# mjevans26/Satellite_ComputerVision

Hardware: AMD Instinct MI355X
Metric: tiles/sec (train) 256x256x4 U-Net (higher is better)
Workload: dtype bf16; 1 GPU; U-Net 256x256x4 bfloat16 training, batch 64 per GPU (BASELINE configs[1]); global_batch=64, parallelism=dp1, loss=weighted_categorical_crossentropy, optimizer=adam(9e-4)

## Files before the change

include/satcv.h:

```cpp
#ifndef SATCV_H
#define SATCV_H
#include <stdint.h>
#ifdef __cplusplus
extern "C" {
#endif

typedef double satcv_stat_t;

enum { SATCV_OK = 0, SATCV_ERR_INVALID = -1, SATCV_ERR_HIP = -2, SATCV_ERR_UNSUPPORTED = -3 };
enum { SATCV_F32 = 0, SATCV_BF16 = 1,
       SATCV_FP8 = 2 ,
       SATCV_FP8X = 3 ,
       SATCV_F64 = 4  };
#define SATCV_STAT_ROWS 32

const char* satcv_version(void);
const char* satcv_last_error(void);
int satcv_device_info(int32_t* out4);

int satcv_ingest_nhwc(const float* src, void* dst, int64_t npix, int32_t c, int32_t cpad,
                      int32_t dtype, void* stream);
int satcv_ingest_nhwc_scaled(const float* src, void* dst, int64_t npix, int32_t c, int32_t cpad, float mul, int32_t dtype, void* stream);
int satcv_ingest_chw(const void* src, int32_t src_kind, float scale, void* dst, int32_t n,
                     int32_t c, int32_t h, int32_t w, int32_t cpad, int32_t dtype, void* stream);
// ... 9 lines not shown
typedef struct satcv_conv_desc {
  const void* x0;
  const void* x1;
  int32_t c0, c1;
  const float* in_scale;
  const float* in_shift;
  int32_t in_relu;
  const void* w;
  const float* bias;
  void* y;
  int32_t ldy;
  satcv_stat_t* stats;
  int32_t stats_ld;
  int32_t n, h, w_;
  int32_t cout;
  int32_t cout_pad;
  int32_t kh, kw, dil;
  int32_t mode_in;
  int32_t mode_out;
  int32_t f;
  int32_t cstat;
  int32_t out_relu;
  int32_t dtype;
  int32_t accumulate;
  int32_t stride, hin, win;
  const float* out_scale;
  void* pool_y; int32_t pool_ld, pool_f;
  const void* bst_y; const void* bst_y1; int32_t bst_ld, bst_ld1, bst_split;
  const float* bst_scale; const float* bst_shift; const float* bst_mean; const float* bst_rstd; int32_t bst_relu;
  int32_t tile_policy;
} satcv_conv_desc;
int satcv_conv2d_igemm(const satcv_conv_desc* d, void* stream);
int satcv_conv2d_igemm_pipelined(const satcv_conv_desc* d);

typedef struct satcv_wgrad_desc {
  const void* x0; const void* x1; int32_t c0, c1;
  const float* in_scale; const float* in_shift; int32_t in_relu;
  const void* dy; int32_t lddy;
  float* dw;
  int32_t cin, cout;
  int32_t n, h, w_;
  int32_t kh, kw, dil;
  int32_t mode_dy;
  int32_t f;
  int32_t transposed;
  float* workspace; int64_t workspace_bytes;
  int32_t dtype;
  int32_t accumulate;
  int32_t whole_chip;
  int32_t defer_reduce;
} satcv_wgrad_desc;
int64_t satcv_conv2d_wgrad_workspace(const satcv_wgrad_desc* d);
int satcv_conv2d_wgrad(const satcv_wgrad_desc* d, void* stream);

typedef struct satcv_reduce_job {
  const float* ws; float* dw;
  int32_t nslab, taps, kpad, npad, cin, nvalid, transposed, accumulate, lanes, pad_;
} satcv_reduce_job;
int satcv_conv2d_wgrad_reduce_job(const satcv_wgrad_desc* d, satcv_reduce_job* job);
int64_t satcv_reduce_job_items(const satcv_reduce_job* job);
int satcv_reduce_slabs_batched(const satcv_reduce_job* jobs_dev, const int64_t* prefix_dev, int32_t njobs, int64_t total_items, void* stream);

typedef struct satcv_bwdf_desc {
  const void* g; const void* yraw; int32_t ldg;
  const float* bn_scale; const float* bn_shift; const float* bn_mean; const float* bn_rstd;
  const float* bn_coef;
  int32_t linear;
  const void* x0; const void* x1; int32_t c0, c1;
  const float* in_scale; const float* in_shift; int32_t in_relu;
  const void* w_dgrad;
  void* dx; int32_t lddx;
  float* dw; int32_t cin, cout;
  int32_t n, h, w_;
  int32_t kh, kw, dil;
  float* workspace; int64_t workspace_bytes;
  int32_t dtype;
  int32_t accumulate;
  satcv_stat_t* bst_sums; int32_t bst_sums_ld;
  const float* bst_mean; const float* bst_rstd;
  int32_t bst_act_form;
  const void* dpool; int32_t lddp; const void* amax;
  const float* hg_dlogits; const float* hg_w; int32_t hg_ncls;
  int32_t defer_reduce;
} satcv_bwdf_desc;
int64_t satcv_conv2d_bwd_fused_workspace(const satcv_bwdf_desc* d);
int satcv_conv2d_bwd_fused(const satcv_bwdf_desc* d, void* stream);
int satcv_conv2d_bwd_fused_reduce_job(const satcv_bwdf_desc* d, satcv_reduce_job* job);

typedef struct satcv_ctbf_desc {
  const void* g; int32_t ldg;
  const void* yup; int32_t ldy;
  const float* bn_scale; const float* bn_shift; const float* bn_mean; const float* bn_rstd;
  const float* bn_c1; const float* bn_c2; int32_t linear;
  const void* x; int32_t ldx;
  const float* in_scale; const float* in_shift; int32_t in_relu;
  const void* w_dgrad; int32_t w_npad;
  void* dx; int32_t lddx;
  float* dw; int32_t cin, cout;
  int32_t n, h, w_, f;
  float* workspace; int64_t workspace_bytes;
  int32_t dtype, accumulate, defer_reduce;
  satcv_stat_t* bst_sums; int32_t bst_sums_ld; const float* bst_mean; const float* bst_rstd;
} satcv_ctbf_desc;
int64_t satcv_convt_bwd_fused_workspace(const satcv_ctbf_desc* d);
int satcv_convt_bwd_fused(const satcv_ctbf_desc* d, void* stream);
int satcv_convt_bwd_fused_reduce_job(const satcv_ctbf_desc* d, satcv_reduce_job* job);

int satcv_bn_finalize_train(satcv_stat_t* stats, int32_t stats_ld, int32_t c, float count,
                            const float* gamma, const float* beta, float eps, float momentum,
                            int32_t updates, int32_t bessel, float* moving_mean, float* moving_var,
                            float* scale, float* shift, float* mean, float* rstd, void* stream);
int satcv_bn_affine_infer(const float* gamma, const float* beta, const float* moving_mean,
                          const float* moving_var, float eps, int32_t c, float* scale, float* shift,
                          void* stream);
typedef struct satcv_bn_affine_job {
  const float* gamma; const float* beta; const float* moving_mean; const float* moving_var;
  float* scale; float* shift; int64_t c;
  const float* conv_bias; float* bias_eff;
} satcv_bn_affine_job;
int satcv_bn_affine_infer_batched(const satcv_bn_affine_job* jobs_device, int32_t njobs, float eps, void* stream);

int satcv_bn_relu_pool(const void* yraw, const float* scale, const float* shift, void* act, int32_t act_ld,
                       void* pooled, satcv_stat_t* stats, int32_t stats_ld, int32_t n, int32_t h,
                       int32_t w_, int32_t c, int32_t f, int32_t dtype, void* stream);
int satcv_bn_relu_pool_amax(const void* yraw, const float* scale, const float* shift, void* act, int32_t act_ld,
                            void* pooled, void* amax, satcv_stat_t* stats, int32_t stats_ld, int32_t n, int32_t h,
                            int32_t w_, int32_t c, int32_t f, int32_t dtype, void* stream);

typedef struct satcv_bnbwd_desc {
  const void* da; int32_t ldda;
  const void* dpool; int32_t lddp;
  int32_t f;
  const void* yraw; int32_t ldy;
  const float* scale; const float* shift; const float* mean; const float* rstd;
  satcv_stat_t* sums; int32_t sums_ld;
  const float* coef;
  void* dy; int32_t lddy_out;
  float* dbias;
  int32_t n, h, w_, c;
  int32_t dtype;
  int32_t linear;
  const void* yraw1; int32_t ldy1;
  void* dy1; int32_t lddy1;
  int32_t c_split;
  satcv_stat_t* sk_sums; int32_t sk_sums_ld;
} satcv_bnbwd_desc;
int satcv_bn_bwd_reduce(const satcv_bnbwd_desc* d, void* stream);
int satcv_bn_bwd_finalize(satcv_stat_t* sums, int32_t sums_ld, int32_t c, float count, float* dgamma,
                          float* dbeta, float* coef, int32_t accumulate, void* stream);
int satcv_bn_bwd_apply(const satcv_bnbwd_desc* d, void* stream);
int satcv_bn_bwd_finalize2(satcv_stat_t* sums, int32_t sums_ld, satcv_stat_t* act_sums, int32_t act_sums_ld, int32_t c, float count,
                           const float* scale, const float* shift, const float* mean, const float* rstd, float* dgamma, float* dbeta,
                           float* coef, int32_t accumulate, void* stream);

int satcv_relu_bwd(const void* act, void* g, int64_t count, int32_t dtype, void* stream);
int64_t satcv_bias_grad_workspace(int64_t npix, int32_t c);
int satcv_bias_grad(const void* dy, int32_t lddy, int64_t npix, int32_t c, int32_t dtype, float* dbias, float* partials, void* stream);

int satcv_maxpool(const void* x, void* out, int32_t n, int32_t h, int32_t w_, int32_t c, int32_t k, int32_t s,
                  int32_t pad, int32_t dtype, void* stream);
int satcv_add_act(const void* y, const float* y_scale, const float* y_shift, const void* res,
                  const float* res_scale, const float* res_shift, int32_t relu, void* out, int64_t npix,
                  int32_t c, int32_t dtype, void* stream);
int satcv_affine_requant(const void* x, int32_t ldx, const float* scale, const float* shift, int32_t relu, void* out, int32_t ldo,
                         int64_t npix, int32_t c, int32_t dtype, int32_t dtype_out, void* stream);

int satcv_upsample_head(const float* logits, int32_t n, int32_t h, int32_t w_, int32_t ncls, int32_t factor,
                        int32_t activation, float thresh, float* probs, int32_t* classes, void* stream);

int satcv_dropout_mask(uint64_t seed, uint64_t offset, float rate, int64_t count, float* mask, void* stream);
int satcv_dropout_apply(const void* x, int32_t ldx, const float* scale, const float* shift, int32_t relu,
                        const float* mask, int32_t ldm, int32_t mask_mode, void* out, int32_t ldo, int32_t n,
                        int32_t hw, int32_t c, int32_t dtype, void* stream);

typedef struct satcv_head_desc {
  const void* x; int32_t ldx; int32_t cin;
  const float* in_scale; const float* in_shift;
  const float* w;
  const float* b;
  int32_t ncls; int32_t activation; float thresh;
  float* probs;
  int32_t* classes;
  const float* dlogits;
  void* dx; int32_t lddx;
  float* dw; float* db;
  const float* bnr_mean; const float* bnr_rstd; satcv_stat_t* bnr_sums; int32_t bnr_sums_ld;
  int64_t npix;
  int32_t dtype;
  float* partials;
} satcv_head_desc;
int satcv_head_fwd(const satcv_head_desc* d, void* stream);
int satcv_head_bwd(const satcv_head_desc* d, void* stream);
int64_t satcv_head_bwd_workspace(const satcv_head_desc* d);
int satcv_head_bwd_finalize(const satcv_head_desc* d, void* stream);

uint32_t satcv_crc32c(const void* data, uint64_t nbytes, uint32_t crc_in);

typedef struct {
  const void* src; int32_t src_kind;
  int32_t n, c, hin, win, h, w_;
  double rescale;
  int32_t nan_mask, replace;
  uint64_t seed;
  const double* ch_mean;
  double contra_mul, bright_mul;
  int32_t flip_v, flip_h, rot;
  float* dst; int32_t ldc, coff;
} satcv_tile_desc;
int satcv_tile_channel_mean(const satcv_tile_desc* d, double* mean_out , void* stream);
int satcv_tile_ingest(const satcv_tile_desc* d, void* stream);
int satcv_label_onehot(const void* lc, int32_t lc_kind, const int32_t* lut, const void* lu, int32_t lu_kind, const int32_t* lu_lut,
                       int32_t n, int32_t hin, int32_t win, int32_t h, int32_t w_, int32_t nclasses, int32_t flip_v, int32_t flip_h,
                       int32_t rot, float* dst, int32_t ldc, int32_t coff, void* stream);

int satcv_loss_fwd_bwd(int32_t kind, const float* probs, const float* y_true,
                       const float* weights, int32_t ncls, int32_t activation, int64_t npix,
                       float grad_scale, float* loss_out, float* dlogits, void* stream);

int satcv_loss_global_fwd_bwd(int32_t kind, const float* probs, const float* y_true,
                              const float* class_weights, int32_t ncls, int32_t activation,
                              int32_t nimg, int64_t pix_per_img, float eps, float grad_scale,
                              float* workspace, float* loss_out, float* dlogits, void* stream);

int satcv_confusion(const int32_t* classes, const float* y_true, int32_t ncls, int64_t npix,
                    int64_t* confusion, void* stream);

int satcv_adam_step(float* p, const float* g, float* m, float* v, int64_t n, float beta1,
                    float beta2, float eps, float* state, const float* lr_mul, void* stream);
int satcv_adam_step_part(float* p, const float* g, float* m, float* v, int64_t n, float beta1,
                         float beta2, float eps, float* state, const float* lr_mul, int32_t bump, void* stream);

int satcv_zero2(void* a, int64_t bytes_a, void* b, int64_t bytes_b, void* stream);

#define SATCV_COMM_ID_BYTES 128
typedef struct satcv_comm satcv_comm;
int satcv_comm_unique_id(void* id128);
// ... 57 lines not shown
```

satellite_computervision_amd/_lib.py:

```python
import ctypes as C
import os

import torch

_HERE = os.path.dirname(os.path.abspath(__file__))
LIB_PATH = os.environ.get('SATCV_LIB') or os.path.join(_HERE, 'libsatcv.so')

F32, BF16, FP8, FP8X, F64 = 0, 1, 2, 3, 4
STAT_ROWS = 32

c_i32, c_i64, c_f32, c_vp = C.c_int32, C.c_int64, C.c_float, C.c_void_p


class ConvDesc(C.Structure):
    _fields_ = [('x0', c_vp), ('x1', c_vp), ('c0', c_i32), ('c1', c_i32),
                ('in_scale', c_vp), ('in_shift', c_vp), ('in_relu', c_i32),
                ('w', c_vp), ('bias', c_vp), ('y', c_vp), ('ldy', c_i32),
                ('stats', c_vp), ('stats_ld', c_i32),
                ('n', c_i32), ('h', c_i32), ('w_', c_i32),
                ('cout', c_i32), ('cout_pad', c_i32),
                ('kh', c_i32), ('kw', c_i32), ('dil', c_i32),
                ('mode_in', c_i32), ('mode_out', c_i32), ('f', c_i32),
                ('cstat', c_i32), ('out_relu', c_i32), ('dtype', c_i32), ('accumulate', c_i32),
                ('stride', c_i32), ('hin', c_i32), ('win', c_i32), ('out_scale', c_vp), ('pool_y', c_vp), ('pool_ld', c_i32), ('pool_f', c_i32),
                ('bst_y', c_vp), ('bst_y1', c_vp), ('bst_ld', c_i32), ('bst_ld1', c_i32), ('bst_split', c_i32),
                ('bst_scale', c_vp), ('bst_shift', c_vp), ('bst_mean', c_vp), ('bst_rstd', c_vp), ('bst_relu', c_i32), ('tile_policy', c_i32)]


class PackJob(C.Structure):
    _fields_ = [('src', c_vp), ('dst', c_vp), ('mode', c_i32), ('taps', c_i32), ('cin', c_i32), ('cout', c_i32), ('kpad', c_i32), ('npad', c_i32)]


class TileDesc(C.Structure):
    _fields_ = [('src', c_vp), ('src_kind', c_i32), ('n', c_i32), ('c', c_i32), ('hin', c_i32), ('win', c_i32), ('h', c_i32), ('w_', c_i32),
                ('rescale', C.c_double), ('nan_mask', c_i32), ('replace', c_i32), ('seed', C.c_uint64), ('ch_mean', c_vp),
                ('contra_mul', C.c_double), ('bright_mul', C.c_double), ('flip_v', c_i32), ('flip_h', c_i32), ('rot', c_i32),
                ('dst', c_vp), ('ldc', c_i32), ('coff', c_i32)]


class WgradDesc(C.Structure):
    _fields_ = [('x0', c_vp), ('x1', c_vp), ('c0', c_i32), ('c1', c_i32),
                ('in_scale', c_vp), ('in_shift', c_vp), ('in_relu', c_i32),
                ('dy', c_vp), ('lddy', c_i32), ('dw', c_vp),
                ('cin', c_i32), ('cout', c_i32),
                ('n', c_i32), ('h', c_i32), ('w_', c_i32),
                ('kh', c_i32), ('kw', c_i32), ('dil', c_i32),
                ('mode_dy', c_i32), ('f', c_i32), ('transposed', c_i32),
                ('workspace', c_vp), ('workspace_bytes', c_i64), ('dtype', c_i32), ('accumulate', c_i32), ('whole_chip', c_i32), ('defer_reduce', c_i32)]


class BwdfDesc(C.Structure):
    _fields_ = [('g', c_vp), ('yraw', c_vp), ('ldg', c_i32),
                ('bn_scale', c_vp), ('bn_shift', c_vp), ('bn_mean', c_vp), ('bn_rstd', c_vp), ('bn_coef', c_vp), ('linear', c_i32),
                ('x0', c_vp), ('x1', c_vp), ('c0', c_i32), ('c1', c_i32),
                ('in_scale', c_vp), ('in_shift', c_vp), ('in_relu', c_i32),
                ('w_dgrad', c_vp), ('dx', c_vp), ('lddx', c_i32),
                ('dw', c_vp), ('cin', c_i32), ('cout', c_i32),
                ('n', c_i32), ('h', c_i32), ('w_', c_i32), ('kh', c_i32), ('kw', c_i32), ('dil', c_i32),
                ('workspace', c_vp), ('workspace_bytes', c_i64), ('dtype', c_i32), ('accumulate', c_i32),
                ('bst_sums', c_vp), ('bst_sums_ld', c_i32), ('bst_mean', c_vp), ('bst_rstd', c_vp), ('bst_act_form', c_i32),
                ('dpool', c_vp), ('lddp', c_i32), ('amax', c_vp),
                ('hg_dlogits', c_vp), ('hg_w', c_vp), ('hg_ncls', c_i32), ('defer_reduce', c_i32)]


class CtbfDesc(C.Structure):
    _fields_ = [('g', c_vp), ('ldg', c_i32), ('yup', c_vp), ('ldy', c_i32),
                ('bn_scale', c_vp), ('bn_shift', c_vp), ('bn_mean', c_vp), ('bn_rstd', c_vp), ('bn_c1', c_vp), ('bn_c2', c_vp), ('linear', c_i32),
                ('x', c_vp), ('ldx', c_i32), ('in_scale', c_vp), ('in_shift', c_vp), ('in_relu', c_i32),
                ('w_dgrad', c_vp), ('w_npad', c_i32), ('dx', c_vp), ('lddx', c_i32), ('dw', c_vp), ('cin', c_i32), ('cout', c_i32),
                ('n', c_i32), ('h', c_i32), ('w_', c_i32), ('f', c_i32), ('workspace', c_vp), ('workspace_bytes', c_i64),
                ('dtype', c_i32), ('accumulate', c_i32), ('defer_reduce', c_i32),
                ('bst_sums', c_vp), ('bst_sums_ld', c_i32), ('bst_mean', c_vp), ('bst_rstd', c_vp)]


class ReduceJob(C.Structure):
    _fields_ = [('ws', c_vp), ('dw', c_vp), ('nslab', c_i32), ('taps', c_i32), ('kpad', c_i32), ('npad', c_i32), ('cin', c_i32), ('nvalid', c_i32),
                ('transposed', c_i32), ('accumulate', c_i32), ('lanes', c_i32), ('pad_', c_i32)]


class BnBwdDesc(C.Structure):
    _fields_ = [('da', c_vp), ('ldda', c_i32), ('dpool', c_vp), ('lddp', c_i32), ('f', c_i32),
                ('yraw', c_vp), ('ldy', c_i32),
                ('scale', c_vp), ('shift', c_vp), ('mean', c_vp), ('rstd', c_vp),
                ('sums', c_vp), ('sums_ld', c_i32), ('coef', c_vp),
                ('dy', c_vp), ('lddy_out', c_i32), ('dbias', c_vp),
                ('n', c_i32), ('h', c_i32), ('w_', c_i32), ('c', c_i32), ('dtype', c_i32), ('linear', c_i32),
                ('yraw1', c_vp), ('ldy1', c_i32), ('dy1', c_vp), ('lddy1', c_i32), ('c_split', c_i32),
                ('sk_sums', c_vp), ('sk_sums_ld', c_i32)]


class HeadDesc(C.Structure):
    _fields_ = [('x', c_vp), ('ldx', c_i32), ('cin', c_i32),
                ('in_scale', c_vp), ('in_shift', c_vp), ('w', c_vp), ('b', c_vp),
                ('ncls', c_i32), ('activation', c_i32), ('thresh', c_f32),
                ('probs', c_vp), ('classes', c_vp), ('dlogits', c_vp),
                ('dx', c_vp), ('lddx', c_i32), ('dw', c_vp), ('db', c_vp),
                ('bnr_mean', c_vp), ('bnr_rstd', c_vp), ('bnr_sums', c_vp), ('bnr_sums_ld', c_i32),
                ('npix', c_i64), ('dtype', c_i32), ('partials', c_vp)]


class LstmGatesDesc(C.Structure):
    _fields_ = [('xg', c_vp), ('ldx', c_i32), ('hg', c_vp), ('ldh_g', c_i32), ('c_prev', c_vp),
                ('c_out', c_vp), ('h_out', c_vp), ('ldh', c_i32), ('gates_out', c_vp),
                ('stats', c_vp), ('stats_ld', c_i32),
                ('dh_a', c_vp), ('lddh_a', c_i32), ('dh_b', c_vp), ('lddh_b', c_i32), ('dc_next', c_vp),
                ('dz_out', c_vp), ('lddz', c_i32), ('dc_prev_out', c_vp),
                ('npix', c_i64), ('filters', c_i32), ('rec_act', c_i32), ('act', c_i32), ('dtype', c_i32)]


class DenseSrc(C.Structure):
    _fields_ = [('x', c_vp), ('ld', c_i32), ('cin', c_i32), ('dtype', c_i32),
                ('in_scale', c_vp), ('in_shift', c_vp), ('in_relu', c_i32),
                ('hs', c_i32), ('ws', c_i32),
                ('dx', c_vp), ('lddx', c_i32), ('dx_dtype', c_i32)]


class DenseDesc(C.Structure):
    _fields_ = [('src', DenseSrc * 2), ('nsrc', c_i32),
                ('w', c_vp), ('b', c_vp), ('cout', c_i32),
                ('activation', c_i32), ('max_value', c_f32),
                ('out', c_vp), ('classes', c_vp), ('z_out', c_vp),
                ('npix', c_i64), ('h', c_i32), ('w_', c_i32),
                ('dout', c_vp), ('dz_out', c_vp), ('dw', c_vp), ('db', c_vp)]


_SIGS = {
    'satcv_version': (C.c_char_p, []),
    'satcv_last_error': (C.c_char_p, []),
    'satcv_device_info': (C.c_int, [C.POINTER(c_i32)]),
    'satcv_ingest_nhwc': (C.c_int, [c_vp, c_vp, c_i64, c_i32, c_i32, c_i32, c_vp]),
    'satcv_ingest_nhwc_scaled': (C.c_int, [c_vp, c_vp, c_i64, c_i32, c_i32, c_f32, c_i32, c_vp]),
    'satcv_ingest_chw': (C.c_int, [c_vp, c_i32, c_f32, c_vp, c_i32, c_i32, c_i32, c_i32, c_i32, c_i32, c_vp]),
    'satcv_pack_weights': (C.c_int, [c_vp, c_vp, c_vp, c_i32, c_i32, c_i32, c_i32, c_i32, c_i32, c_i32, c_vp]),
    'satcv_pack_job_items': (c_i64, [C.POINTER(PackJob)]),
    'satcv_pack_weights_batched': (C.c_int, [c_vp, c_vp, c_i32, c_i64, c_i32, c_vp]),
    'satcv_conv2d_igemm': (C.c_int, [C.POINTER(ConvDesc), c_vp]),
    'satcv_conv2d_igemm_pipelined': (C.c_int, [C.POINTER(ConvDesc)]),
    'satcv_conv2d_wgrad_workspace': (c_i64, [C.POINTER(WgradDesc)]),
    'satcv_conv2d_wgrad': (C.c_int, [C.POINTER(WgradDesc), c_vp]),
    'satcv_conv2d_wgrad_reduce_job': (C.c_int, [C.POINTER(WgradDesc), C.POINTER(ReduceJob)]),
    'satcv_reduce_job_items': (c_i64, [C.POINTER(ReduceJob)]),
    'satcv_reduce_slabs_batched': (C.c_int, [c_vp, c_vp, c_i32, c_i64, c_vp]),
    'satcv_conv2d_bwd_fused_workspace': (c_i64, [C.POINTER(BwdfDesc)]),
    'satcv_conv2d_bwd_fused': (C.c_int, [C.POINTER(BwdfDesc), c_vp]),
    'satcv_conv2d_bwd_fused_reduce_job': (C.c_int, [C.POINTER(BwdfDesc), C.POINTER(ReduceJob)]),
    'satcv_convt_bwd_fused_workspace': (c_i64, [C.POINTER(CtbfDesc)]),
    'satcv_convt_bwd_fused': (C.c_int, [C.POINTER(CtbfDesc), c_vp]),
    'satcv_convt_bwd_fused_reduce_job': (C.c_int, [C.POINTER(CtbfDesc), C.POINTER(ReduceJob)]),
    'satcv_bn_finalize_train': (C.c_int, [c_vp, c_i32, c_i32, c_f32, c_vp, c_vp, c_f32, c_f32, c_i32, c_i32,
                                          c_vp, c_vp, c_vp, c_vp, c_vp, c_vp, c_vp]),
    'satcv_bn_affine_infer': (C.c_int, [c_vp, c_vp, c_vp, c_vp, c_f32, c_i32, c_vp, c_vp, c_vp]),
    'satcv_bn_affine_infer_batched': (C.c_int, [c_vp, c_i32, c_f32, c_vp]),
    'satcv_bn_relu_pool': (C.c_int, [c_vp, c_vp, c_vp, c_vp, c_i32, c_vp, c_vp, c_i32, c_i32, c_i32, c_i32, c_i32, c_i32, c_i32, c_vp]),
    'satcv_bn_relu_pool_amax': (C.c_int, [c_vp, c_vp, c_vp, c_vp, c_i32, c_vp, c_vp, c_vp, c_i32, c_i32, c_i32, c_i32, c_i32, c_i32, c_i32, c_vp]),
    'satcv_bn_bwd_reduce': (C.c_int, [C.POINTER(BnBwdDesc), c_vp]),
    'satcv_bn_bwd_finalize': (C.c_int, [c_vp, c_i32, c_i32, c_f32, c_vp, c_vp, c_vp, c_i32, c_vp]),
    'satcv_bn_bwd_apply': (C.c_int, [C.POINTER(BnBwdDesc), c_vp]),
    'satcv_bn_bwd_finalize2': (C.c_int, [c_vp, c_i32, c_vp, c_i32, c_i32, c_f32, c_vp, c_vp, c_vp, c_vp, c_vp, c_vp, c_vp, c_i32, c_vp]),
    'satcv_maxpool': (C.c_int, [c_vp, c_vp, c_i32, c_i32, c_i32, c_i32, c_i32, c_i32, c_i32, c_i32, c_vp]),
    'satcv_affine_requant': (C.c_int, [c_vp, c_i32, c_vp, c_vp, c_i32, c_vp, c_i32, c_i64, c_i32, c_i32, c_i32, c_vp]),
    'satcv_add_act': (C.c_int, [c_vp, c_vp, c_vp, c_vp, c_vp, c_vp, c_i32, c_vp, c_i64, c_i32, c_i32, c_vp]),
    'satcv_relu_bwd': (C.c_int, [c_vp, c_vp, c_i64, c_i32, c_vp]),
    'satcv_bias_grad_workspace': (c_i64, [c_i64, c_i32]),
    'satcv_bias_grad': (C.c_int, [c_vp, c_i32, c_i64, c_i32, c_i32, c_vp, c_vp, c_vp]),
    'satcv_upsample_head': (C.c_int, [c_vp, c_i32, c_i32, c_i32, c_i32, c_i32, c_i32, c_f32, c_vp, c_vp, c_vp]),
    'satcv_dropout_mask': (C.c_int, [C.c_uint64, C.c_uint64, c_f32, c_i64, c_vp, c_vp]),
    'satcv_dropout_apply': (C.c_int, [c_vp, c_i32, c_vp, c_vp, c_i32, c_vp, c_i32, c_i32, c_vp, c_i32, c_i32, c_i32, c_i32, c_i32, c_vp]),
    'satcv_tile_channel_mean': (C.c_int, [C.POINTER(TileDesc), c_vp, c_vp]),
    'satcv_tile_ingest': (C.c_int, [C.POINTER(TileDesc), c_vp]),
    'satcv_label_onehot': (C.c_int, [c_vp, c_i32, c_vp, c_vp, c_i32, c_vp, c_i32, c_i32, c_i32, c_i32, c_i32, c_i32, c_i32, c_i32, c_i32, c_vp, c_i32, c_i32, c_vp]),
    'satcv_crc32c': (C.c_uint32, [c_vp, C.c_uint64, C.c_uint32]),
    'satcv_head_fwd': (C.c_int, [C.POINTER(HeadDesc), c_vp]),
    'satcv_head_bwd': (C.c_int, [C.POINTER(HeadDesc), c_vp]),
    'satcv_head_bwd_workspace': (c_i64, [C.POINTER(HeadDesc)]),
    'satcv_head_bwd_finalize': (C.c_int, [C.POINTER(HeadDesc), c_vp]),
    'satcv_loss_fwd_bwd': (C.c_int, [c_i32, c_vp, c_vp, c_vp, c_i32, c_i32, c_i64, c_f32, c_vp, c_vp, c_vp]),
    'satcv_loss_global_fwd_bwd': (C.c_int, [c_i32, c_vp, c_vp, c_vp, c_i32, c_i32, c_i32, c_i64, c_f32, c_f32, c_vp, c_vp, c_vp, c_vp]),
    'satcv_confusion': (C.c_int, [c_vp, c_vp, c_i32, c_i64, c_vp, c_vp]),
    'satcv_adam_step': (C.c_int, [c_vp, c_vp, c_vp, c_vp, c_i64, c_f32, c_f32, c_f32, c_vp, c_vp, c_vp]),
    'satcv_adam_step_part': (C.c_int, [c_vp, c_vp, c_vp, c_vp, c_i64, c_f32, c_f32, c_f32, c_vp, c_vp, c_i32, c_vp]),
    'satcv_comm_unique_id': (C.c_int, [c_vp]),
    'satcv_comm_init': (C.c_int, [C.POINTER(c_vp), c_i32, c_i32, c_vp]),
    'satcv_comm_destroy': (C.c_int, [c_vp]),
    'satcv_comm_info': (C.c_int, [c_vp, C.POINTER(c_i32), C.POINTER(c_i32)]),
    'satcv_allreduce_grads': (C.c_int, [c_vp, c_vp, c_i64, c_i64, c_i64, c_i32, c_vp, c_vp]),
    'satcv_allreduce': (C.c_int, [c_vp, c_vp, c_i64, c_i32, c_i32, c_vp]),
    'satcv_ingest_seq': (C.c_int, [c_vp, c_vp, c_i32, c_i32, c_i32, c_i32, c_i32, c_i32, c_i32, c_vp]),
    'satcv_convlstm_gates_fwd': (C.c_int, [C.POINTER(LstmGatesDesc), c_vp]),
    'satcv_convlstm_gates_bwd': (C.c_int, [C.POINTER(LstmGatesDesc), c_vp]),
    'satcv_dense_small_fwd': (C.c_int, [C.POINTER(DenseDesc), c_vp]),
    'satcv_dense_small_bwd': (C.c_int, [C.POINTER(DenseDesc), c_vp]),
    'satcv_zero2': (C.c_int, [c_vp, c_i64, c_vp, c_i64, c_vp]),
    'satcv_graph_begin': (C.c_int, [c_vp]),
    'satcv_graph_end': (C.c_int, [c_vp, C.POINTER(c_vp)]),
    'satcv_graph_launch': (C.c_int, [c_vp, c_vp]),
    'satcv_graph_destroy': (C.c_int, [c_vp]),
    'satcv_prof_enable': (C.c_int, [c_i32]),
    'satcv_prof_collect': (C.c_int, [c_i32, C.POINTER(C.c_double), C.POINTER(c_i64), C.POINTER(C.c_double)]),
    'satcv_set_option': (C.c_int, [C.c_char_p, c_i32]),
    'satcv_get_option': (C.c_int, [C.c_char_p, C.POINTER(c_i32)]),
}

EXPORTED_SYMBOLS = tuple(_SIGS)


class SatcvError(RuntimeError):
    pass


def _load():
    if not os.path.exists(LIB_PATH):
        raise ImportError(
            f'{LIB_PATH} not found: the HIP extension is required (no CPU fallback). '
            'Build it with `python -m satellite_computervision_amd.build` or __graft_entry__.build().')
    hip = os.path.join(os.path.dirname(torch.__file__), 'lib', 'libamdhip64.so')
    if os.path.exists(hip):
        C.CDLL(hip, mode=C.RTLD_GLOBAL)
    lib = C.CDLL(LIB_PATH)
    for name, (res, args) in _SIGS.items():
        fn = getattr(lib, name)
        fn.restype = res
        fn.argtypes = args
    return lib


lib = _load()


def check(rc):
    if rc != 0:
        raise SatcvError(f'satcv error {rc}: {lib.satcv_last_error().decode()}')


def call(name, *args):
    check(getattr(lib, name)(*args))
```

satellite_computervision_amd/csrc/conv_bwd_fused.hip:

```cpp
#include "igemm_common.hpp"
#include <cstdlib>
#include <cstring>

#ifndef BWDF_ABL
#define BWDF_ABL 0
#endif
#define FABL(bit) ((BWDF_ABL & (bit)) != 0)

int wgrad_reduce_slabs(const float* ws, float* dw, int nslab, int taps, int kpad, int npad, int cin, int nvalid, int accumulate, hipStream_t st);
void reduce_job_fill(satcv_reduce_job* job, const float* ws, float* dw, int nslab, int taps, int kpad, int npad, int cin, int nvalid, int transposed, int accumulate);
void satcv_prof_begin(int kind, double flops, hipStream_t st);
void satcv_prof_end(int kind, hipStream_t st);

struct BwdfArgs {
  IgemmArgs e;
  const void* g; const void* yraw; int ldg;
  const float* bn_scale; const float* bn_shift; const float* bn_mean; const float* bn_rstd; const float* bn_coef; int bn_c, linear;
  const void* x0; const void* x1; int c0, c1;
  const float* in_scale; const float* in_shift; int in_relu;
  const void* w;
  float* ws;
  int tiles_x, tiles_y;
  satcv_stat_t* bst_sums; int bst_ld; const float* bst_mean; const float* bst_rstd;
  int bst_act_form;
  const void* dp; int lddp; const unsigned char* amax;
  const float* hg_dl; const float* hg_w;
};

__device__ __forceinline__ bf16x4 tr_read4(const bf16* p) {
  short4v v = __builtin_amdgcn_ds_read_tr16_b64_v4i16((__attribute__((address_space(3))) short4v*)(p));
  return __builtin_bit_cast(bf16x4, v);
}

template <int CIN, int COUT, int NW, int WPS, bool POOL = false, bool NODG = false, int CINS = CIN, bool HG = false>
__global__ __launch_bounds__(NW * 64, WPS) void bwd_fused_kernel(const BwdfArgs a, const int total_tiles) {
  static_assert(!HG || !POOL, "the head feeds a decoder block");
  typedef bf16 T;
  constexpr int TW = 32, TH = 8, BM = 256, RL = TH + 2, CL = TW + 2, PITCH = CL, EL = 8, NTHREADS = NW * 64;
  constexpr int SD = COUT / 8, SX = CIN / 8, SXR = CINS / 8;
  constexpr int DSTRIDE = RL * PITCH * EL;
  constexpr int XSTRIDE = BM * EL + 32;
  static_assert((DSTRIDE * 2) % 256 == 64 && (XSTRIDE * 2) % 256 == 64, "plane strides must be 64 B modulo 256 B");
  constexpr int D_ITEMS = RL * CL * SD, DI = (D_ITEMS + NTHREADS - 1) / NTHREADS;
  constexpr int X_ITEMS = BM * SXR, XI = X_ITEMS / NTHREADS;
  static_assert(X_ITEMS % NTHREADS == 0 && NTHREADS % SD == 0 && NTHREADS % SXR == 0, "item -> thread mapping");
  constexpr int XPIX_STEP = NTHREADS / SXR;
  static_assert(XPIX_STEP % 32 == 0, "x items of a thread must share a column");
  constexpr int MT = 8 / NW, NT = CIN / 32;
#ifdef BWDF_NOBAL
  constexpr int NTILE = (CIN / 32) * (COUT / 32) * 9, FULL = (NTILE + NW - 1) / NW, REM = 0, WT = FULL;
#else
  constexpr int NTILE = (CIN / 32) * (COUT / 32) * 9, FULL = NTILE / NW, REM = NTILE % NW, WT = FULL + (REM ? 1 : 0);
#endif
  constexpr bool GUARD = FULL * NW > NTILE;
  constexpr int WPP = REM ? NW / REM : 1, KPW = REM ? 16 / WPP : 0;
  static_assert(REM == 0 || (NW % REM == 0 && 16 % WPP == 0 && KPW % 2 == 0), "left-over products must split evenly along K");
  constexpr int W_ITEMS = NODG ? 0 : 9 * SD * CIN;
  constexpr size_t R0_BYTES = ((size_t)(SD * DSTRIDE + SX * XSTRIDE) * sizeof(T) + 127) / 128 * 128;
  constexpr size_t W_BYTES = (size_t)W_ITEMS * EL * sizeof(T);
  constexpr size_t O_BYTES = (size_t)BM * (CIN + 8) * sizeof(T);
  constexpr bool O_ALIAS = O_BYTES <= (size_t)SD * DSTRIDE * sizeof(T);
  constexpr size_t TAB_BYTES = (size_t)(SD * 32 + SX * 16 + (HG ? 2 * COUT : 0)) * sizeof(float);
  static_assert(!NODG || O_ALIAS || true, "");
  constexpr size_t O_OFF = O_ALIAS ? 0 : (R0_BYTES + W_BYTES + TAB_BYTES + 127) / 128 * 128;
  extern __shared__ __attribute__((aligned(16))) unsigned char smem_raw[];
  T* ldsD = reinterpret_cast<T*>(smem_raw);
  T* ldsX = ldsD + SD * DSTRIDE;
  T* ldsW = reinterpret_cast<T*>(smem_raw + R0_BYTES);
  float* tabD = reinterpret_cast<float*>(smem_raw + R0_BYTES + W_BYTES);
  float* tabX = tabD + SD * 32;
  float* tabH = tabX + SX * 16;

  const int tid = threadIdx.x, lane = tid & 63, wave = tid >> 6;
  const int r = lane & 31, hh = lane >> 5;
  const T* wp = reinterpret_cast<const T*>(a.w);

  for (int it = tid; it < W_ITEMS; it += NTHREADS) lstore8<T>(ldsW + (size_t)it * EL, gload8<T>(wp + (size_t)it * EL));
  if constexpr (SXR < SX) {
    for (int it = tid; it < (SX - SXR) * BM; it += NTHREADS) lstore8<T>(ldsX + (SXR + it / BM) * XSTRIDE + (it % BM) * EL, zero8<T>());
  }
  for (int ch = tid; ch < COUT; ch += NTHREADS) {
    const float sc = a.bn_scale[ch], sh = a.bn_shift[ch], mu = a.bn_mean[ch], rs = a.bn_rstd[ch], c1 = a.bn_coef[ch], c2 = a.bn_coef[a.bn_c + ch];
    float* t = tabD + (ch >> 3) * 32 + (ch & 7);
    t[0] = sc; t[8] = sh; t[16] = -sc * c2 * rs; t[24] = sc * (c2 * rs * mu - c1);
  }
  if constexpr (HG) {
    for (int ch = tid; ch < COUT; ch += NTHREADS) {
      float* t = tabH + (ch >> 3) * 16 + (ch & 7);
      t[0] = a.hg_w[ch * 2]; t[8] = a.hg_w[ch * 2 + 1];
    }
  }
  for (int ch = tid; ch < CINS; ch += NTHREADS) {
    float* t = tabX + (ch >> 3) * 16 + (ch & 7);
    t[0] = a.in_scale ? a.in_scale[ch] : 1.f; t[8] = a.in_scale ? a.in_shift[ch] : 0.f;
  }
  const float lin_lo = a.linear ? -INFINITY : 0.f;
  const bool xaff = a.in_scale != nullptr;
  const unsigned xrelu_lim = a.in_relu != 0 ? 0u : 0x80008000u;

  const int slot_d = tid % SD, slot_x = tid % SXR;
  constexpr int DPK = (DI + 2) / 3;
  unsigned d_pk[DPK];
#pragma unroll
  for (int k = 0; k < DPK; ++k) d_pk[k] = 0;
#pragma unroll
  for (int j = 0; j < DI; ++j) {
    const int it = tid + j * NTHREADS;
    const int p = it / SD, c = p % CL, L = p / CL;
    d_pk[j / 3] |= (unsigned)(it < D_ITEMS ? (L << 6) | c : 0x3ff) << (10 * (j % 3));
  }
  auto d_item = [&](int j) -> int { return (int)((d_pk[j / 3] >> (10 * (j % 3))) & 0x3ffu); };
  const int g_rowstride = a.e.w_ * a.ldg;
  const unsigned gy_lane = (unsigned)slot_d * EL;
  const int xch0 = slot_x * EL;
  const bool xsecond = xch0 >= a.c0;
  const T* xsrc = xsecond ? reinterpret_cast<const T*>(a.x1) + (xch0 - a.c0) : reinterpret_cast<const T*>(a.x0) + xch0;
  const int xcs = xsecond ? a.c1 : a.c0;
  const int xq0 = tid / SXR;
  const int x_l0 = slot_x * XSTRIDE + xq0 * EL;
  const int x_eoff0 = ((xq0 / TW) * a.e.w_ + (xq0 % TW)) * xcs, x_estep = (XPIX_STEP / TW) * a.e.w_ * xcs;

  int a_off[MT];
#pragma unroll
  for (int m = 0; m < MT; ++m) {
    const int q = (wave * MT + m) * 32 + r;
    a_off[m] = ((q / TW) * PITCH + (q % TW)) * EL;
  }
  const int gi = lane >> 4, i16 = lane & 15;
  const int chb = 16 * (gi & 1) + 4 * (i16 & 3);
  const int pk = 8 * (gi >> 1) + (i16 >> 2);
  const int tr_x = (chb >> 3) * XSTRIDE + pk * EL + (chb & 7);
  const int tr_d = (chb >> 3) * DSTRIDE + pk * EL + (chb & 7);

  auto tile_origin = [&](int v, int& n0, int& y0, int& x0) {
    const int tx = v % a.tiles_x; v /= a.tiles_x;
    const int ty = v % a.tiles_y;
    n0 = v / a.tiles_y; y0 = ty * TH; x0 = tx * TW;
  };
  auto next_origin = [&](int& n0, int& y0, int& x0) {
    x0 += TW;
    if (x0 >= a.e.w_) { x0 = 0; y0 += TH; if (y0 >= a.e.h) { y0 = 0; ++n0; } }
  };
  Raw8<T> rg[HG ? 1 : DI], ry[DI], rx[XI];
  float2 rdl[HG ? DI : 1];
  Raw8<T> rp[POOL ? DI : 1];
  uint2 ra[POOL ? DI : 1];
  const int hp = a.e.h >> 1, wpool = a.e.w_ >> 1;
  unsigned valid = 0;
  auto issue_loads = [&](int n0, int y0, int x0) -> unsigned {
    unsigned vm = 0;
    const int ylo = 1 - y0, yhi = a.e.h - y0 + 1, xlo = 1 - x0, xhi = a.e.w_ - x0 + 1;
    const long long pb = (long long)(n0 * a.e.h + y0 - 1) * a.e.w_ + (x0 - 1);
    const long long bp = pb * a.ldg;
    const T* gb = reinterpret_cast<const T*>(a.g) + bp;
    const T* yb = reinterpret_cast<const T*>(a.yraw) + bp;
    const unsigned centre = (unsigned)(g_rowstride + a.ldg) + gy_lane;
#pragma unroll
    for (int j = 0; j < DI; ++j) {
      const int pk_ = d_item(j), L = pk_ >> 6, c = pk_ & 63;
      const bool ok = pk_ != 0x3ff && L >= ylo && L < yhi && c >= xlo && c < xhi;
      vm |= (ok ? 1u : 0u) << j;
      unsigned off = ok ? (unsigned)(__mul24(L, g_rowstride) + __mul24(c, a.ldg)) + gy_lane : centre;
      asm volatile("" : "+v"(off));
      if constexpr (HG) {
        int poff = ok ? __mul24(L, a.e.w_) + c : a.e.w_ + 1;
        asm volatile("" : "+v"(poff));
        rdl[j] = reinterpret_cast<const float2*>(a.hg_dl)[pb + poff];
        ry[j] = gload8<T>(yb + off);
      } else if (!FABL(32)) { rg[j] = gload8<T>(gb + off); ry[j] = gload8<T>(yb + off); }
      else { rg[j] = zero8<T>(); ry[j] = zero8<T>(); rg[j].q[0].x = off; }
    }
    return vm;
  };
  auto issue_pool = [&](int n0, int y0, int x0) {
    if constexpr (POOL) {
      const int ylo = 1 - y0, yhi = a.e.h - y0 + 1, xlo = 1 - x0, xhi = a.e.w_ - x0 + 1;
      const size_t pb = (size_t)(n0 * hp + (y0 >> 1)) * wpool + (x0 >> 1);
#pragma unroll
      for (int j = 0; j < DI; ++j) {
        const int pk_ = d_item(j), L = pk_ >> 6, c = pk_ & 63;
        const bool ok = pk_ != 0x3ff && L >= ylo && L < yhi && c >= xlo && c < xhi;
        int po = ok ? __mul24((L - 1) >> 1, wpool) + ((c - 1) >> 1) : 0;
        asm volatile("" : "+v"(po));
        rp[j] = gload8<T>(reinterpret_cast<const T*>(a.dp) + (pb + po) * a.lddp + gy_lane);
        ra[j] = *reinterpret_cast<const uint2*>(a.amax + (pb + po) * COUT + gy_lane);
      }
    }
  };
  auto issue_x = [&](int n0, int y0, int x0) {
    const size_t bp = (size_t)(n0 * a.e.h + y0) * a.e.w_ + x0;
    const T* xb = xsrc + bp * xcs + x_eoff0;
#pragma unroll
    for (int j = 0; j < XI; ++j) { if (!FABL(32)) rx[j] = gload8<T>(xb + (size_t)j * x_estep); else { rx[j] = zero8<T>(); rx[j].q[0].x = (unsigned)(size_t)xb; } }
  };

  const int G = gridDim.x;
  const int xcd = blockIdx.x & 7, nx = G >> 3, remx = G & 7;
  const int bid = (xcd < remx ? xcd * (nx + 1) : remx * (nx + 1) + (xcd - remx) * nx) + (blockIdx.x >> 3);
  const int per = total_tiles / G, extra = total_tiles % G;
  const int t_lo = bid * per + (bid < extra ? bid : extra), t_hi = t_lo + per + (bid < extra ? 1 : 0);

  f32x16 wacc[WT];
  int w_xo[WT], w_do[WT];
#pragma unroll
  for (int t = 0; t < WT; ++t) {
#pragma unroll
    for (int i = 0; i < 16; ++i) wacc[t][i] = 0.f;
    const int wv = __builtin_amdgcn_readfirstlane(wave);
    const int id = t < FULL ? wv + t * NW : FULL * NW + wv / WPP;
    const int tap = id % 9, pair = id / 9;
    const int ci_t = pair % (CIN / 32), co_t = pair / (CIN / 32);
    w_xo[t] = ci_t * 4 * XSTRIDE;
    w_do[t] = co_t * 4 * DSTRIDE + ((2 - tap / 3) * PITCH + (2 - tap % 3)) * EL;
    if (t >= FULL) {
      const int k0 = (wv % WPP) * KPW;
      w_xo[t] += k0 * 16 * EL;
      w_do[t] += (k0 >> 1) * PITCH * EL;
    }
  }

  constexpr bool BST = !NODG && (WPS != 1 || POOL);
  float bs1[8], bs2[8];
#pragma unroll
  for (int e = 0; e < 8; ++e) { bs1[e] = 0.f; bs2[e] = 0.f; }
  int n0, y0, x0;
  if (t_lo < t_hi) { tile_origin(t_lo, n0, y0, x0); valid = issue_loads(n0, y0, x0); issue_x(n0, y0, x0); issue_pool(n0, y0, x0); }
  __syncthreads();
  for (int t = t_lo; t < t_hi; ++t) {
    {
      int toff = slot_d * 32;
      asm volatile("" : "+v"(toff));
      const float4* tp = reinterpret_cast<const float4*>(tabD + toff);
      float prm[32];
#pragma unroll
      for (int k = 0; k < 8; ++k) { const float4 v4 = tp[k]; prm[4 * k] = v4.x; prm[4 * k + 1] = v4.y; prm[4 * k + 2] = v4.z; prm[4 * k + 3] = v4.w; }
#pragma unroll
      for (int j = 0; j < DI; ++j) {
        float gv[8], yv[8];
        if constexpr (HG) {
          int hoff = slot_d * 16;
          asm volatile("" : "+v"(hoff));
          const float4* hp = reinterpret_cast<const float4*>(tabH + hoff);
          const float4 w00 = hp[0], w01 = hp[1], w10 = hp[2], w11 = hp[3];
          const float w0[8] = {w00.x, w00.y, w00.z, w00.w, w01.x, w01.y, w01.z, w01.w};
          const float w1[8] = {w10.x, w10.y, w10.z, w10.w, w11.x, w11.y, w11.z, w11.w};
#pragma unroll
          for (int e = 0; e < 8; ++e) gv[e] = (float)(T)fmaf(rdl[j].y, w1[e], rdl[j].x * w0[e]);
        } else {
          unpack8<T>(rg[j], gv);
        }
        unpack8<T>(ry[j], yv);
        if constexpr (POOL) {
          float pv[8];
          unpack8<T>(rp[j], pv);
          const int pk2 = d_item(j);
          const unsigned sub = ((((pk2 >> 6) + 1) & 1) << 1) | (((pk2 & 63) + 1) & 1);
#pragma unroll
          for (int e = 0; e < 8; ++e) {
            const unsigned am = ((e < 4 ? ra[j].x : ra[j].y) >> (8 * (e & 3))) & 0xffu;
            gv[e] += am == sub ? pv[e] : 0.f;
          }
        }
        Raw8<T> v;
        if constexpr (FABL(2) && !HG) { v = rg[j]; v.q[0].x ^= ry[j].q[0].x; }
        else {
          bf16x8 o;
#pragma unroll
          for (int e = 0; e < 8; ++e) {
            const float act = yv[e] * prm[e] + prm[8 + e];
            const float gm = act > lin_lo ? gv[e] : 0.f;
            o[e] = (bf16)(prm[e] * gm + (prm[16 + e] * yv[e] + prm[24 + e]));
          }
          v.q[0] = __builtin_bit_cast(uint4, o);
        }
        v = select8<T>((valid >> j) & 1u, v);
        const int pk_ = d_item(j);
        if (pk_ != 0x3ff) lstore8<T>(ldsD + slot_d * DSTRIDE + __mul24((pk_ >> 6) * CL + (pk_ & 63), EL), v);
        __builtin_amdgcn_sched_barrier(0);
      }
    }
    {
      float sc[8], sh[8];
      if (xaff) {
        int toff = slot_x * 16;
        asm volatile("" : "+v"(toff));
        const float4* tp = reinterpret_cast<const float4*>(tabX + toff);
        const float4 s0 = tp[0], s1 = tp[1], h0 = tp[2], h1 = tp[3];
        sc[0] = s0.x; sc[1] = s0.y; sc[2] = s0.z; sc[3] = s0.w; sc[4] = s1.x; sc[5] = s1.y; sc[6] = s1.z; sc[7] = s1.w;
        sh[0] = h0.x; sh[1] = h0.y; sh[2] = h0.z; sh[3] = h0.w; sh[4] = h1.x; sh[5] = h1.y; sh[6] = h1.z; sh[7] = h1.w;
      }
#pragma unroll
      for (int j = 0; j < XI; ++j) {
        Raw8<T> v = rx[j];
        if (xaff) v = affine8_lim(v, sc, sh, xrelu_lim);
        lstore8<T>(ldsX + x_l0 + j * (XPIX_STEP * EL), v);
      }
    }
    __syncthreads();
    const int tn0 = n0, ty0 = y0, tx0 = x0;
    if (t + 1 < t_hi) { next_origin(n0, y0, x0); valid = issue_loads(n0, y0, x0); }

#pragma unroll
    for (int tt = 0; tt < FULL; ++tt) {
      if (!FABL(8) && (!GUARD || tt < FULL - 1 || __builtin_amdgcn_readfirstlane(wave) + (FULL - 1) * NW < NTILE)) {
        const T* xa = ldsX + w_xo[tt] + tr_x;
        const T* da = ldsD + w_do[tt] + tr_d;
        bf16x4 fa[2][2], fb[2][2];
        auto read_k = [&](const T* xp, const T* dp, int u, int buf) {
          const int xq = u * 16 * EL, dq = ((u >> 1) * PITCH + (u & 1) * 16) * EL;
          fa[buf][0] = tr_read4(xp + xq); fa[buf][1] = tr_read4(xp + xq + 4 * EL);
          fb[buf][0] = tr_read4(dp + dq); fb[buf][1] = tr_read4(dp + dq + 4 * EL);
        };
        read_k(xa, da, 0, 0);
#pragma unroll 1
        for (int grp = 0; grp < TH / 2; ++grp) {
          const T* xp = xa + grp * (64 * EL);
          const T* dp = da + grp * (2 * PITCH * EL);
          const int wrap = grp + 1 < TH / 2 ? 1 : 1 - TH / 2;
#pragma unroll
          for (int u = 0; u < 4; ++u) {
            asm volatile("" ::: "memory");
            if (u < 3) read_k(xp, dp, u + 1, (u + 1) & 1);
            else read_k(xp + wrap * (64 * EL), dp + wrap * (2 * PITCH * EL), 0, 0);
            __builtin_amdgcn_sched_barrier(0);
            const bf16x8 afr = __builtin_shufflevector(fa[u & 1][0], fa[u & 1][1], 0, 1, 2, 3, 4, 5, 6, 7);
            const bf16x8 bfr = __builtin_shufflevector(fb[u & 1][0], fb[u & 1][1], 0, 1, 2, 3, 4, 5, 6, 7);
            if constexpr (!FABL(1)) wacc[tt] = __builtin_amdgcn_mfma_f32_32x32x16_bf16(afr, bfr, wacc[tt], 0, 0, 0);
            else asm volatile("" :: "v"(afr), "v"(bfr));
          }
        }
      }
    }
    if constexpr (REM > 0) {
      if (!FABL(8)) {
        const T* xa = ldsX + w_xo[FULL] + tr_x;
        const T* da = ldsD + w_do[FULL] + tr_d;
        bf16x4 fa[2][2], fb[2][2];
        auto read_k = [&](int u, int buf) {
          const int xq = u * 16 * EL, dq = ((u >> 1) * PITCH + (u & 1) * 16) * EL;
          fa[buf][0] = tr_read4(xa + xq); fa[buf][1] = tr_read4(xa + xq + 4 * EL);
          fb[buf][0] = tr_read4(da + dq); fb[buf][1] = tr_read4(da + dq + 4 * EL);
        };
        read_k(0, 0);
#pragma unroll
        for (int u = 0; u < KPW; ++u) {
          asm volatile("" ::: "memory");
          if (u + 1 < KPW) read_k(u + 1, (u + 1) & 1);
          __builtin_amdgcn_sched_barrier(0);
          const bf16x8 afr = __builtin_shufflevector(fa[u & 1][0], fa[u & 1][1], 0, 1, 2, 3, 4, 5, 6, 7);
          const bf16x8 bfr = __builtin_shufflevector(fb[u & 1][0], fb[u & 1][1], 0, 1, 2, 3, 4, 5, 6, 7);
          if constexpr (!FABL(1)) wacc[FULL] = __builtin_amdgcn_mfma_f32_32x32x16_bf16(afr, bfr, wacc[FULL], 0, 0, 0);
          else asm volatile("" :: "v"(afr), "v"(bfr));
        }
      }
    }
    if (t + 1 < t_hi) issue_x(n0, y0, x0);
    if (POOL && NODG && t + 1 < t_hi) issue_pool(n0, y0, x0);
    if constexpr (!NODG) {
    f32x16 acc[MT][NT];
#pragma unroll
    for (int m = 0; m < MT; ++m)
#pragma unroll
      for (int n = 0; n < NT; ++n)
#pragma unroll
        for (int i = 0; i < 16; ++i) acc[m][n][i] = 0.f;
    {
      constexpr int KS = COUT / 16, STEPS = 9 * KS;
      FragT<T> af[2][MT], bf[2][NT];
      auto read_step = [&](int st, int buf) {
        const int tap = st / KS, ks = st % KS;
        const int tap_off = ((tap / 3) * PITCH + (tap % 3)) * EL;
        const int slot = ks * 2 + hh;
#pragma unroll
        for (int m = 0; m < MT; ++m) af[buf][m] = lds_frag<T>(ldsD + slot * DSTRIDE + a_off[m] + tap_off);
#pragma unroll
        for (int n = 0; n < NT; ++n) bf[buf][n] = lds_frag<T>(ldsW + ((tap * SD + slot) * CIN + n * 32 + r) * EL);
      };
      if constexpr (!FABL(8)) {
      read_step(0, 0);
#pragma unroll
      for (int st = 0; st < STEPS; ++st) {
        asm volatile("" ::: "memory");
        if (st + 1 < STEPS) read_step(st + 1, (st + 1) & 1);
        __builtin_amdgcn_sched_barrier(0);
#pragma unroll
        for (int m = 0; m < MT; ++m)
#pragma unroll
          for (int n = 0; n < NT; ++n) {
            if constexpr (!FABL(1)) mma32<T>(acc[m][n], af[st & 1][m], bf[st & 1][n]);
            else asm volatile("" :: "v"(af[st & 1][m].v), "v"(bf[st & 1][n].v));
          }
      }
      }
    }
    if (POOL && t + 1 < t_hi) issue_pool(n0, y0, x0);
    __syncthreads();
    {
      constexpr int OPITCH = CIN + 8, VPR = CIN / 8;
      T* ldsO = reinterpret_cast<T*>(smem_raw + O_OFF);
      T* op = ldsO + ((wave * MT) * 32 + 4 * hh) * OPITCH + r;
#pragma unroll
      for (int m = 0; m < MT; ++m)
#pragma unroll
        for (int n = 0; n < NT; ++n)
#pragma unroll
          for (int i = 0; i < 16; ++i) op[(m * 32 + (i & 3) + 8 * (i >> 2)) * OPITCH + n * 32] = (T)acc[m][n][i];
      __syncthreads();
      const int vq = tid % VPR;
      T* yp = reinterpret_cast<T*>(a.e.y) + ((size_t)(tn0 * a.e.h + ty0) * a.e.w_ + tx0) * a.e.ldy + vq * 8;
      const unsigned row_pitch = (unsigned)a.e.w_ * a.e.ldy;
      const T* xact = ldsX + vq * XSTRIDE;
#pragma unroll 2
      for (int it = tid; it < BM * VPR; it += NTHREADS) {
        const int q = it / VPR;
        const uint4 dv = *reinterpret_cast<const uint4*>(ldsO + q * OPITCH + vq * 8);
        if constexpr (!FABL(4)) *reinterpret_cast<uint4*>(yp + (size_t)((q / TW) * row_pitch + (q % TW) * (unsigned)a.e.ldy)) = dv;
        else asm volatile("" :: "v"(dv.x));
        if (BST && a.bst_sums) {
          const bf16x8 d8 = __builtin_bit_cast(bf16x8, dv);
          const bf16x8 a8 = *reinterpret_cast<const bf16x8*>(xact + q * EL);
#pragma unroll
          for (int e = 0; e < 8; ++e) {
            const float df = (float)d8[e], af = (float)a8[e];
            bs1[e] += af > 0.f ? df : 0.f;
            bs2[e] += df * af;
          }
        }
      }
    }
    }
    __syncthreads();
  }
  if constexpr (REM > 0) {
    float* red = reinterpret_cast<float*>(smem_raw);
#pragma unroll
    for (int i = 0; i < 16; ++i) red[(wave * 16 + i) * 64 + lane] = wacc[FULL][i];
    __syncthreads();
    if (wave % WPP == 0) {
#pragma unroll 1
      for (int k = 1; k < WPP; ++k)
#pragma unroll
        for (int i = 0; i < 16; ++i) wacc[FULL][i] += red[((wave + k) * 16 + i) * 64 + lane];
    }
  }
#pragma unroll
  for (int tt = 0; tt < WT; ++tt) {
    const int wv = __builtin_amdgcn_readfirstlane(wave);
    const int id = tt < FULL ? wv + tt * NW : FULL * NW + wv / WPP;
    if ((tt < FULL && (!GUARD || id < NTILE)) || (tt >= FULL && wv % WPP == 0)) {
      const int tap = id % 9, pair = id / 9;
      const int ci_t = pair % (CIN / 32), co_t = pair / (CIN / 32);
      float* dst = a.ws + ((size_t)(blockIdx.x * 9 + tap) * CIN + ci_t * 32) * COUT + co_t * 32 + r;
#pragma unroll
      for (int i = 0; i < 16; ++i) dst[(size_t)((i & 3) + 8 * (i >> 2) + 4 * hh) * COUT] = wacc[tt][i];
    }
  }
  if (BST && a.bst_sums && t_lo < t_hi) {
    constexpr int VPR = CIN / 8, NPER = NTHREADS / VPR;
    float* red = reinterpret_cast<float*>(smem_raw);
    __syncthreads();
#pragma unroll
    for (int e = 0; e < 8; ++e) { red[e * NTHREADS + tid] = bs1[e]; red[(8 + e) * NTHREADS + tid] = bs2[e]; }
    __syncthreads();
    if (tid < CIN) {
      const int vq = tid >> 3, e = tid & 7;
      double t1 = 0.0, t2 = 0.0;
      for (int k = 0; k < NPER; ++k) { t1 += (double)red[e * NTHREADS + k * VPR + vq]; t2 += (double)red[(8 + e) * NTHREADS + k * VPR + vq]; }
      double s2 = t2;
      if (!a.bst_act_form) {
        const double sc = (double)a.in_scale[tid], sh = (double)a.in_shift[tid], mu = (double)a.bst_mean[tid], rs = (double)a.bst_rstd[tid];
        s2 = sc != 0.0 ? (t2 - (sh + sc * mu) * t1) * (rs / sc) : 0.0;
      }
      satcv_stat_t* rowp = a.bst_sums + (size_t)(blockIdx.x % SATCV_STAT_ROWS) * 2 * a.bst_ld;
      atomicAdd(rowp + tid, (satcv_stat_t)t1);
      atomicAdd(rowp + a.bst_ld + tid, (satcv_stat_t)s2);
    }
  }
}

template <int CIN, int COUT, int NW, bool NODG = false>
struct BwdfGeom {
  static constexpr int SD = COUT / 8, SX = CIN / 8;
  static constexpr size_t R0 = ((size_t)(SD * (10 * 34 * 8) + SX * (256 * 8 + 32)) * 2 + 127) / 128 * 128;
  static constexpr size_t O_BYTES = (size_t)256 * (CIN + 8) * 2;
  static constexpr bool O_ALIAS = O_BYTES <= (size_t)SD * (10 * 34 * 8) * 2;
  static constexpr size_t BASE = R0 + (NODG ? 0 : (size_t)9 * SD * CIN * 16) + (size_t)(SD * 32 + SX * 16 + 2 * COUT) * 4;
  static constexpr size_t LDS0 = O_ALIAS ? BASE : (BASE + 127) / 128 * 128 + O_BYTES;
  static constexpr size_t RED = (size_t)16 * NW * 64 * 4;
  static constexpr size_t LDS = LDS0 > RED ? LDS0 : RED;
};

static int g_ncu = 0;
static int bwdf_grid(size_t lds, int waves, int wps, long long total) {
  if (!g_ncu) {
    int dev = 0; hipDeviceProp_t p;
    if (hipGetDevice(&dev) != hipSuccess || hipGetDeviceProperties(&p, dev) != hipSuccess) return -1;
    g_ncu = p.multiProcessorCount;
  }
  int per_cu = (int)((160 * 1024) / lds);
  const int by_waves = 4 * wps / waves;
  if (per_cu > by_waves) per_cu = by_waves;
  if (per_cu < 1) per_cu = 1;
  long long grid = (long long)g_ncu * per_cu;
  if (grid > total) grid = total;
  return (int)grid;
}

static bool bwdf_shape_ok(const satcv_bwdf_desc* d, int& cin_s) {
  cin_s = d->c0 + d->c1;
  if (d->dtype != SATCV_BF16 || d->kh != 3 || d->kw != 3 || d->dil != 1) return false;
  if (d->x1 && d->c0 % 8 != 0) return false;
  if (d->h % 8 != 0 || d->w_ % 32 != 0) return false;
  if (d->ldg % 8 != 0 || ((uintptr_t)d->g % 16) != 0 || ((uintptr_t)d->yraw % 16) != 0) return false;
  if (d->hg_dlogits && (!d->hg_w || d->hg_ncls != 2 || d->dpool || ((uintptr_t)d->hg_dlogits % 8) != 0)) return false;
  if (d->dx && (d->lddx % 8 != 0 || ((uintptr_t)d->dx % 16) != 0)) return false;
  if ((long long)d->w_ * d->ldg >= (1 << 23)) return false;
  if (d->dpool) {
    if (!d->amax || d->lddp % 8 != 0 || ((uintptr_t)d->dpool % 16) != 0 || ((uintptr_t)d->amax % 8) != 0 || d->x1) return false;
    if (d->dx) return cin_s == 32 && d->cin == 32 && d->cout == 64;
    return cin_s == 16 && d->cin <= 16 && d->cout == 32 && !d->bst_sums;
  }
  if (!d->dx) return false;
  if (d->bst_sums && cin_s == 64 && d->cout == 64) return false;
  if (!((cin_s == 32 && d->cout == 32) || (cin_s == 64 && d->cout == 32) || (cin_s == 64 && d->cout == 64))) return false;
  if (d->cin != cin_s) return false;
  return true;
}

template <int CIN, int COUT, int NW, int WPS, bool POOL = false, bool NODG = false, int CINS = CIN, bool HG = false>
static int bwdf_launch(const satcv_bwdf_desc* d, hipStream_t st, bool query, int64_t* ws_bytes, satcv_reduce_job* job = nullptr) {
  using G = BwdfGeom<CIN, COUT, NW, NODG>;
  static_assert(G::LDS <= 160 * 1024, "tile + weights exceed the LDS");
  const long long total = (long long)d->n * (d->h / 8) * (d->w_ / 32);
  const int grid = bwdf_grid(G::LDS, NW, WPS, total);
  if (grid <= 0) { satcv_set_error("bwd_fused: device query failed"); return SATCV_ERR_HIP; }
  const size_t need = (size_t)grid * 9 * CIN * COUT * sizeof(float);
  if (job) { reduce_job_fill(job, d->workspace, d->dw, grid, 9, CIN, COUT, d->cin, COUT, 0, d->accumulate); return SATCV_OK; }
  if (query) { *ws_bytes = (int64_t)need; return SATCV_OK; }
  SATCV_CHECK((size_t)d->workspace_bytes >= need, "bwd_fused: workspace %lld < %zu", (long long)d->workspace_bytes, need);
  BwdfArgs a;
  memset(&a, 0, sizeof(a));
  a.e.y = d->dx; a.e.ldy = d->lddx; a.e.n = d->n; a.e.h = d->h; a.e.w_ = d->w_; a.e.cout = CIN; a.e.cout_pad = CIN; a.e.cstat = CIN;
  a.e.imgs = 1; a.e.rpi = 8; a.e.tiles_x = d->w_ / 32; a.e.tiles_y = d->h / 8; a.e.n_tiles = 1;
  a.g = d->g; a.yraw = d->yraw; a.ldg = d->ldg;
  a.bn_scale = d->bn_scale; a.bn_shift = d->bn_shift; a.bn_mean = d->bn_mean; a.bn_rstd = d->bn_rstd; a.bn_coef = d->bn_coef; a.bn_c = d->cout; a.linear = d->linear;
  a.x0 = d->x0; a.x1 = d->x1; a.c0 = d->c0; a.c1 = d->c1; a.in_scale = d->in_scale; a.in_shift = d->in_shift; a.in_relu = d->in_relu;
  a.w = d->w_dgrad; a.ws = d->workspace; a.tiles_x = d->w_ / 32; a.tiles_y = d->h / 8;
  a.bst_sums = d->bst_sums; a.bst_ld = d->bst_sums_ld; a.bst_mean = d->bst_mean; a.bst_rstd = d->bst_rstd; a.bst_act_form = d->bst_act_form;
  a.dp = d->dpool; a.lddp = d->lddp; a.amax = reinterpret_cast<const unsigned char*>(d->amax);
  a.hg_dl = d->hg_dlogits; a.hg_w = d->hg_w;
  auto kern = bwd_fused_kernel<CIN, COUT, NW, WPS, POOL, NODG, CINS, HG>;
  { const int rc = satcv_ensure_dynamic_lds(reinterpret_cast<const void*>(kern), G::LDS); if (rc) return rc; }
  const double flops = (NODG ? 2.0 : 4.0) * d->n * d->h * d->w_ * (double)CINS * COUT * 9;
  satcv_prof_begin(3, flops, st);
  hipLaunchKernelGGL(kern, dim3(grid), dim3(NW * 64), G::LDS, st, a, (int)total);
  satcv_prof_end(3, st);
  hipError_t e = hipGetLastError();
  if (e != hipSuccess) { satcv_set_error("bwd_fused launch: %s", hipGetErrorString(e)); return SATCV_ERR_HIP; }
  if (d->defer_reduce) return SATCV_OK;
  return wgrad_reduce_slabs(d->workspace, d->dw, grid, 9, CIN, COUT, d->cin, COUT, d->accumulate, st);
}

static int bwdf_dispatch(const satcv_bwdf_desc* d, hipStream_t st, bool query, int64_t* ws_bytes, satcv_reduce_job* job = nullptr) {
  int cin_s;
  if (!bwdf_shape_ok(d, cin_s)) return SATCV_ERR_UNSUPPORTED;
  if (d->dpool) {
    if (d->dx) return bwdf_launch<32, 64, 4, 1, true, false>(d, st, query, ws_bytes, job);
    return bwdf_launch<32, 32, 8, 2, true, true, 16>(d, st, query, ws_bytes, job);
  }
  if (cin_s == 32 && d->hg_dlogits) return bwdf_launch<32, 32, 8, 2, false, false, 32, true>(d, st, query, ws_bytes, job);
  if (d->hg_dlogits) return SATCV_ERR_UNSUPPORTED;
  if (cin_s == 32) return bwdf_launch<32, 32, 8, 2>(d, st, query, ws_bytes, job);
  if (d->cout == 32) return bwdf_launch<64, 32, 8, 2>(d, st, query, ws_bytes, job);
  return bwdf_launch<64, 64, 4, 1>(d, st, query, ws_bytes, job);
}

extern "C" int satcv_conv2d_bwd_fused_reduce_job(const satcv_bwdf_desc* d, satcv_reduce_job* job) {
  SATCV_CHECK(d && job && d->dw && d->workspace, "bwd_fused_reduce_job: null pointer");
  return bwdf_dispatch(d, nullptr, false, nullptr, job);
}

extern "C" int64_t satcv_conv2d_bwd_fused_workspace(const satcv_bwdf_desc* d) {
  int64_t nb = -1;
  if (!d || bwdf_dispatch(d, nullptr, true, &nb) != SATCV_OK) return -1;
  return nb;
}

extern "C" int satcv_conv2d_bwd_fused(const satcv_bwdf_desc* d, void* stream) {
  SATCV_CHECK(d && (d->g || d->hg_dlogits) && d->yraw && d->x0 && d->dw && d->workspace && (d->dx == nullptr || d->w_dgrad), "bwd_fused: null pointer");
  SATCV_CHECK(d->bn_scale && d->bn_shift && d->bn_mean && d->bn_rstd && d->bn_coef, "bwd_fused: BatchNorm coefficients missing");
  SATCV_CHECK((d->c1 == 0) == (d->x1 == nullptr) && d->n > 0 && d->h > 0 && d->w_ > 0, "bwd_fused: bad dims");
  SATCV_CHECK(!d->bst_sums || (d->bst_sums_ld >= d->c0 + d->c1 && (d->bst_act_form ? d->in_scale == nullptr
                               : (d->in_scale && d->in_shift && d->in_relu && d->bst_mean && d->bst_rstd))),
              "bwd_fused: the fused sums need the input's BatchNorm (in_scale / in_shift with ReLU, bst_mean / bst_rstd), or an activated input with bst_act_form");
  const int rc = bwdf_dispatch(d, reinterpret_cast<hipStream_t>(stream), false, nullptr);
  if (rc == SATCV_ERR_UNSUPPORTED) satcv_set_error("bwd_fused: shape outside the kernel's limits (ask satcv_conv2d_bwd_fused_workspace first)");
  return rc;
}
```

satellite_computervision_amd/csrc/elementwise.hip:

```cpp
#include "common.hpp"
#include <cstdlib>

#define EW_BLOCK 256
static inline int ew_grid(long long items, int cap = 0) {
  static const int dflt = [] { const char* e = getenv("SATCV_EW_PER_CU"); const int v = e ? atoi(e) : 6; return 256 * (v >= 1 ? v : 6); }();
  if (cap <= 0) cap = dflt;
  long long b = (items + EW_BLOCK - 1) / EW_BLOCK;
  if (b < 1) b = 1;
  if (b > cap) b = cap;
  return (int)b;
}
#define LAUNCH_OK(name)                                                          \
  do {                                                                           \
    hipError_t e__ = hipGetLastError();                                          \
    if (e__ != hipSuccess) {                                                     \
      satcv_set_error(name " launch: %s", hipGetErrorString(e__));               \
      return SATCV_ERR_HIP;                                                      \
    }                                                                            \
  } while (0)
#define DISPATCH_T(dtype, ...)                                                   \
  do {                                                                           \
    if ((dtype) == SATCV_BF16) { using T = bf16; __VA_ARGS__; }                  \
    else if ((dtype) == SATCV_F32) { using T = float; __VA_ARGS__; }             \
    else { satcv_set_error("bad dtype %d", (int)(dtype)); return SATCV_ERR_INVALID; } \
// ... 416 lines not shown
            float v[8];
            unpack8<T>(v4[q], v);
#pragma unroll
            for (int e = 0; e < 8; ++e) {
              const float a = round_to<T>(fmaxf(v[e] * sc[e] + sh[e], 0.f));
              if (a > mx[e]) { mx[e] = a; am[e] = q; }
            }
          }
        }
#pragma unroll
        for (int q = 0; q < 4; ++q) {
          float v[8], gr[8], o[8];
          unpack8<T>(v4[q], v);
          unpack8<T>(g4[q], gr);
#pragma unroll
          for (int e = 0; e < 8; ++e) {
            float gg = gr[e];
            if (am[e] == q) gg += gp[e];
            const float a = v[e] * sc[e] + sh[e];
            gg = (a > 0.f || d.linear) ? gg : 0.f;
            const float xh = (v[e] - mu[e]) * rs[e];
            if (APPLY) { const float t = sc[e] * (gg - c1[e] - xh * c2[e]); o[e] = round_to<T>(t); s1[e] += o[e]; }
            else { s1[e] += gg; s2[e] += gg * xh; }
          }
          if (APPLY) store8<T>(dy + pixs[q] * d.lddy_out + g * 8, o);
        }
        continue;
      }
      if (full) {
        float mx[8];
#pragma unroll
        for (int e = 0; e < 8; ++e) { mx[e] = -INFINITY; am[e] = 0; }
        for (int i = 0; i < f; ++i) for (int j = 0; j < f; ++j) {
          float v[8];
          load8<T>(yr + ((size_t)(img * h + py * f + i) * w + px * f + j) * d.ldy + g * 8, v);
#pragma unroll
          for (int e = 0; e < 8; ++e) {
            const float a = round_to<T>(fmaxf(v[e] * sc[e] + sh[e], 0.f));
            if (a > mx[e]) { mx[e] = a; am[e] = i * f + j; }
          }
        }
        load8<T>(dp + ((size_t)(img * hp + py) * wp + px) * d.lddp + g * 8, gp);
      }
      for (int i = 0; i < f; ++i) {
        const int y = py * f + i; if (y >= h) break;
        for (int j = 0; j < f; ++j) {
          const int x = px * f + j; if (x >= w) break;
          const size_t pix = (size_t)(img * h + y) * w + x;
          float v[8], gr[8];
          load8<T>(yr + pix * d.ldy + g * 8, v);
          if (da) load8<T>(da + pix * d.ldda + g * 8, gr);
          else {
#pragma unroll
            for (int e = 0; e < 8; ++e) gr[e] = 0.f;
          }
          float o[8];
#pragma unroll
          for (int e = 0; e < 8; ++e) {
            float gg = gr[e];
            if (full && am[e] == i * f + j) gg += gp[e];
            const float a = v[e] * sc[e] + sh[e];
            gg = (a > 0.f || d.linear) ? gg : 0.f;
            const float xh = (v[e] - mu[e]) * rs[e];
            if (APPLY) { const float t = sc[e] * (gg - c1[e] - xh * c2[e]); o[e] = round_to<T>(t); s1[e] += o[e]; }
            else { s1[e] += gg; s2[e] += gg * xh; }
          }
          if (APPLY) store8<T>(dy + pix * d.lddy_out + g * 8, o);
        }
      }
    }
  }
  if (!APPLY) block_channel_reduce(lds, s1, s2, g, active, c, d.sums, d.sums_ld);
  else if (d.dbias) {
    for (int i = threadIdx.x; i < c; i += blockDim.x) lds[i] = 0.f;
    __syncthreads();
    if (active) {
#pragma unroll
      for (int e = 0; e < 8; ++e) atomicAdd(&lds[g * 8 + e], s1[e]);
    }
    __syncthreads();
    for (int i = threadIdx.x; i < c; i += blockDim.x) atomicAdd(d.dbias + i, lds[i]);
  }
}
template <typename T, bool APPLY>
__global__ __launch_bounds__(EW_BLOCK) void bn_bwd_dense_kernel(const satcv_bnbwd_desc d, const int rev, const int cld) {
  extern __shared__ float lds[];
  const int c = d.c, G = c / 8;
  const unsigned npix = (unsigned)d.n * d.h * d.w_;
  const unsigned nthreads = gridDim.x * blockDim.x;
  const unsigned per = nthreads / G;
  const unsigned gid = blockIdx.x * blockDim.x + threadIdx.x;
  const bool active = gid < per * G;
  const int g = gid % G;
  const bool second = d.c_split > 0 && g * 8 >= d.c_split;
  const T* da = (const T*)d.da + g * 8;
  const T* yr = second ? (const T*)d.yraw1 + (g * 8 - d.c_split) : (const T*)d.yraw + g * 8;
  T* dy = second ? (T*)d.dy1 + (g * 8 - d.c_split) : (T*)d.dy + g * 8;
  const int ldy = second ? d.ldy1 : d.ldy, lddy = second ? d.lddy1 : d.lddy_out;
  const bool sk = APPLY && d.sk_sums != nullptr && !second;
  float sc[8], sh[8], mu[8], rs[8], c1[8], c2[8], s1[8], s2[8];
#pragma unroll
  for (int e = 0; e < 8; ++e) {
    const int ch = g * 8 + e;
    sc[e] = d.scale[ch]; sh[e] = d.shift[ch]; mu[e] = d.mean[ch]; rs[e] = d.rstd[ch];
    c1[e] = APPLY ? d.coef[ch] : 0.f; c2[e] = APPLY ? d.coef[cld + ch] : 0.f;
    s1[e] = 0.f; s2[e] = 0.f;
  }
  if (active) {
    const unsigned pfirst = gid / G;
    const long long step = rev ? -(long long)per : (long long)per;
    const long long pstart = rev ? (long long)npix - 1 - pfirst : (long long)pfirst;
    const T* yq = yr + pstart * ldy;
    const T* dq = da + pstart * d.ldda;
    T* oq = dy + pstart * lddy;
    const long long ystep = step * ldy, dstep = step * d.ldda, ostep = step * lddy;
    const float lin_lo = d.linear ? -INFINITY : 0.f;
#pragma unroll 4
    for (unsigned p0 = pfirst; p0 < npix; p0 += per) {
      float v[8], gr[8], o[8];
      load8<T>(yq, v);
      load8<T>(dq, gr);
#pragma unroll
      for (int e = 0; e < 8; ++e) {
        const float a = v[e] * sc[e] + sh[e];
        const float gg = (a > lin_lo) ? gr[e] : 0.f;
        const float xh = (v[e] - mu[e]) * rs[e];
        if (APPLY) {
          const float t = sc[e] * (gg - c1[e] - xh * c2[e]); o[e] = round_to<T>(t);
          if (sk) { s1[e] += v[e] > 0.f ? o[e] : 0.f; s2[e] += o[e] * v[e]; }
          else s1[e] += o[e];
        }
        else { s1[e] += gg; s2[e] += gg * xh; }
      }
      if (APPLY) store8<T>(oq, o);
      yq += ystep; dq += dstep; oq += ostep;
    }
  }
  if (!APPLY) block_channel_reduce(lds, s1, s2, g, active, c, d.sums, d.sums_ld);
  else if (d.sk_sums) block_channel_reduce(lds, s1, s2, g, active && !second, c, d.sk_sums, d.sk_sums_ld, d.c_split > 0 ? d.c_split : -1);
  else if (d.dbias) {
    for (int i = threadIdx.x; i < c; i += blockDim.x) lds[i] = 0.f;
    __syncthreads();
    if (active) {
#pragma unroll
      for (int e = 0; e < 8; ++e) atomicAdd(&lds[g * 8 + e], s1[e]);
    }
    __syncthreads();
    for (int i = threadIdx.x; i < c; i += blockDim.x) atomicAdd(d.dbias + i, lds[i]);
  }
}

template <typename T, bool SK, bool DB, int U>
__global__ __launch_bounds__(EW_BLOCK) void bn_bwd_apply_dense_kernel(const satcv_bnbwd_desc d, const int rev, const int cld) {
  extern __shared__ float lds[];
  const int c = d.c, G = c / 8;
  const unsigned npix = (unsigned)d.n * d.h * d.w_;
  const unsigned nthreads = gridDim.x * blockDim.x;
  const unsigned per = nthreads / G;
  const unsigned gid = blockIdx.x * blockDim.x + threadIdx.x;
  const bool active = gid < per * G;
  const int g = gid % G;
  const bool second = d.c_split > 0 && g * 8 >= d.c_split;
  const T* da = (const T*)d.da + g * 8;
  const T* yr = second ? (const T*)d.yraw1 + (g * 8 - d.c_split) : (const T*)d.yraw + g * 8;
  T* dy = second ? (T*)d.dy1 + (g * 8 - d.c_split) : (T*)d.dy + g * 8;
  const int ldy = second ? d.ldy1 : d.ldy, lddy = second ? d.lddy1 : d.lddy_out;
  float sc[8], sh[8], mu[8], k1[8], k2[8], s1[8], s2[8];
#pragma unroll
  for (int e = 0; e < 8; ++e) {
    const int ch = g * 8 + e;
    sc[e] = d.scale[ch]; sh[e] = d.shift[ch]; mu[e] = d.mean[ch];
    k1[e] = sc[e] * d.coef[ch]; k2[e] = sc[e] * d.rstd[ch] * d.coef[cld + ch];
    s1[e] = 0.f; s2[e] = 0.f;
  }
  const float lin_lo = d.linear ? -INFINITY : 0.f;
  const unsigned pfirst = gid / G;
  const unsigned nit = (npix + per - 1) / per;
  auto body = [&](unsigned i0, auto FULLC) __attribute__((always_inline)) {
    constexpr bool FULL = decltype(FULLC)::value;
    Raw8<T> rv[U], rg[U];
    unsigned pp[U];
    bool ok[U];
#pragma unroll
    for (int u = 0; u < U; ++u) {
      const unsigned long long q = (unsigned long long)pfirst + (unsigned long long)(i0 + u) * per;
      ok[u] = FULL ? active : (active && q < npix);
      const unsigned pq = (FULL || q < npix) ? (unsigned)q : npix - 1;
      pp[u] = rev ? npix - 1 - pq : pq;
      rv[u] = gload8<T>(yr + (size_t)pp[u] * ldy);
      rg[u] = gload8<T>(da + (size_t)pp[u] * d.ldda);
    }
#pragma unroll
    for (int u = 0; u < U; ++u) {
      float v[8], gr[8], o[8];
      unpack8<T>(rv[u], v);
      unpack8<T>(rg[u], gr);
#pragma unroll
      for (int e = 0; e < 8; ++e) {
        const float gm = (fmaf(v[e], sc[e], sh[e]) > lin_lo) ? gr[e] : 0.f;
        const float t = fmaf(-k2[e], v[e] - mu[e], fmaf(sc[e], gm, -k1[e]));
        if constexpr (SK || DB) {
          o[e] = round_to<T>(t);
          const float om = (FULL || ok[u]) ? o[e] : 0.f;
          if constexpr (SK) { s1[e] += v[e] > 0.f ? om : 0.f; s2[e] = fmaf(om, v[e], s2[e]); }
          else s1[e] += om;
        } else {
          o[e] = t;
        }
      }
      if (ok[u]) store8<T>(dy + (size_t)pp[u] * lddy, o);
    }
  };
  unsigned i0 = 0;
  for (; (unsigned long long)(i0 + U) * per < npix; i0 += U) body(i0, std::true_type{});
  for (; i0 < nit; i0 += U) body(i0, std::false_type{});
  if constexpr (SK) block_channel_reduce(lds, s1, s2, g, active && !second, c, d.sk_sums, d.sk_sums_ld, d.c_split > 0 ? d.c_split : -1);
  else if constexpr (DB) {
    for (int i = threadIdx.x; i < c; i += blockDim.x) lds[i] = 0.f;
    __syncthreads();
    if (active) {
#pragma unroll
      for (int e = 0; e < 8; ++e) atomicAdd(&lds[g * 8 + e], s1[e]);
    }
    __syncthreads();
    for (int i = threadIdx.x; i < c; i += blockDim.x) atomicAdd(d.dbias + i, lds[i]);
  }
}
template <typename T>
static void bn_bwd_apply_dense_launch(const satcv_bnbwd_desc& e, long long items, size_t lds_bytes, int rev, int cld, hipStream_t st) {
  static const int mode = getenv("SATCV_BN_APPLY") ? atoi(getenv("SATCV_BN_APPLY")) : 1;
  const dim3 grid(ew_grid(items)), block(EW_BLOCK);
  if (mode == 0) { hipLaunchKernelGGL((bn_bwd_dense_kernel<T, true>), grid, block, lds_bytes, st, e, rev, cld); return; }
  if (e.sk_sums) hipLaunchKernelGGL((bn_bwd_apply_dense_kernel<T, true, false, 4>), grid, block, lds_bytes, st, e, rev, cld);
  else if (e.dbias) hipLaunchKernelGGL((bn_bwd_apply_dense_kernel<T, false, true, 4>), grid, block, lds_bytes, st, e, rev, cld);
  else hipLaunchKernelGGL((bn_bwd_apply_dense_kernel<T, false, false, 4>), grid, block, lds_bytes, st, e, rev, cld);
}
static int bnbwd_check(const satcv_bnbwd_desc* d, bool apply) {
  SATCV_CHECK(d && d->yraw && d->scale && d->shift && d->mean && d->rstd, "bn_bwd: null pointer");
  SATCV_CHECK(d->da || d->dpool, "bn_bwd: no incoming gradient");
  SATCV_CHECK(d->c > 0 && d->c % 8 == 0 && d->c <= 2048 && d->n > 0 && d->h > 0 && d->w_ > 0, "bn_bwd: bad dims");
  SATCV_CHECK(!d->dpool || d->f >= 1, "bn_bwd: pool factor");
  SATCV_CHECK(!apply || !d->sk_sums || (d->c_split > 0 && !d->dbias && d->sk_sums_ld >= d->c_split), "bn_bwd_apply: sk_sums needs the two-source form");
  if (apply) SATCV_CHECK(d->coef && d->dy, "bn_bwd_apply: coef/dy missing");
  else SATCV_CHECK(d->sums && d->sums_ld >= d->c, "bn_bwd_reduce: sums missing");
  if (d->c_split > 0) {
    SATCV_CHECK(d->c_split % 8 == 0 && d->c_split < d->c && d->yraw1 && d->ldy1 >= d->c - d->c_split && !d->dpool && d->da && !d->dbias &&
                (long long)d->n * d->h * d->w_ < 0x7fffffffLL, "bn_bwd: second source needs the dense form (da, no dpool / dbias), c_split %% 8 == 0");
    if (apply) SATCV_CHECK(!d->dy1 || d->lddy1 >= d->c - d->c_split, "bn_bwd_apply: dy1 channel stride");
  }
  return SATCV_OK;
}
extern "C" int satcv_bn_bwd_reduce(const satcv_bnbwd_desc* d, void* stream) {
  int rc = bnbwd_check(d, false); if (rc) return rc;
  const int f = d->dpool ? d->f : 1;
  const long long items = (long long)d->n * cdiv(d->h, f) * cdiv(d->w_, f) * (d->c / 8);
  const int grid = ew_grid((items + 7) / 8);
  if (!d->dpool && d->da && (long long)d->n * d->h * d->w_ < 0x7fffffffLL) {
    DISPATCH_T(d->dtype, hipLaunchKernelGGL((bn_bwd_dense_kernel<T, false>), dim3(grid), dim3(EW_BLOCK), (EW_BLOCK + 8) * 16 * sizeof(float), (hipStream_t)stream, *d, 0, d->c));
  } else {
    DISPATCH_T(d->dtype, hipLaunchKernelGGL((bn_bwd_kernel<T, false>), dim3(grid), dim3(EW_BLOCK), (EW_BLOCK + 8) * 16 * sizeof(float), (hipStream_t)stream, *d));
  }
  LAUNCH_OK("bn_bwd_reduce");
  return SATCV_OK;
}
extern "C" int satcv_bn_bwd_apply(const satcv_bnbwd_desc* d, void* stream) {
  static const int rev = getenv("SATCV_BN_REV") ? atoi(getenv("SATCV_BN_REV")) : 1;
  int rc = bnbwd_check(d, true); if (rc) return rc;
  const int f = d->dpool ? d->f : 1;
  if (d->c_split > 0 && !d->dy1) {
    satcv_bnbwd_desc e = *d;
    e.c = d->c_split; e.c_split = 0; e.yraw1 = nullptr;
    const long long it1 = (long long)d->n * d->h * d->w_ * (e.c / 8);
    const size_t lds_1 = d->sk_sums ? (EW_BLOCK + 8) * 16 * sizeof(float) : e.c * sizeof(float);
    DISPATCH_T(d->dtype, bn_bwd_apply_dense_launch<T>(e, it1, lds_1, rev, d->c, (hipStream_t)stream));
    LAUNCH_OK("bn_bwd_apply");
    return SATCV_OK;
  }
  const long long items = (long long)d->n * cdiv(d->h, f) * cdiv(d->w_, f) * (d->c / 8);
  if (!d->dpool && d->da && (long long)d->n * d->h * d->w_ < 0x7fffffffLL) {
    const size_t lds_b = d->sk_sums ? (EW_BLOCK + 8) * 16 * sizeof(float) : d->c * sizeof(float);
    DISPATCH_T(d->dtype, bn_bwd_apply_dense_launch<T>(*d, items, lds_b, rev, d->c, (hipStream_t)stream));
  } else {
    DISPATCH_T(d->dtype, hipLaunchKernelGGL((bn_bwd_kernel<T, true>), dim3(ew_grid(items)), dim3(EW_BLOCK), d->c * sizeof(float), (hipStream_t)stream, *d));
  }
  LAUNCH_OK("bn_bwd_apply");
  return SATCV_OK;
}
__global__ void bn_bwd_finalize_kernel(satcv_stat_t* sums, int ld, int c, float count, float* dgamma, float* dbeta, float* coef, int accumulate) {
  const int ch = blockIdx.x * (blockDim.x / 32) + threadIdx.x / 32, r = threadIdx.x & 31;
  double d1 = 0.0, d2 = 0.0;
  if (ch < c) {
    satcv_stat_t* row = sums + (size_t)r * 2 * ld;
    d1 = row[ch]; d2 = row[ld + ch];
    row[ch] = 0.0; row[ld + ch] = 0.0;
  }
#pragma unroll
  for (int o = 16; o > 0; o >>= 1) { d1 += __shfl_xor(d1, o, 64); d2 += __shfl_xor(d2, o, 64); }
  if (ch >= c || r != 0) return;
  const float s1 = (float)d1, s2 = (float)d2;
  if (dbeta) dbeta[ch] = accumulate ? dbeta[ch] + s1 : s1;
  if (dgamma) dgamma[ch] = accumulate ? dgamma[ch] + s2 : s2;
  coef[ch] = s1 / count; coef[c + ch] = s2 / count;
}
__global__ void bn_bwd_finalize2_kernel(satcv_stat_t* sums, int ld, satcv_stat_t* asums, int ald, int c, float count, const float* scale, const float* shift,
                                        const float* mean, const float* rstd, float* dgamma, float* dbeta, float* coef, int accumulate) {
  const int ch = blockIdx.x * (blockDim.x / 32) + threadIdx.x / 32, r = threadIdx.x & 31;
  double d1 = 0.0, d2 = 0.0, a1 = 0.0, a2 = 0.0;
  if (ch < c) {
    if (sums) { satcv_stat_t* row = sums + (size_t)r * 2 * ld; d1 = row[ch]; d2 = row[ld + ch]; row[ch] = 0.0; row[ld + ch] = 0.0; }
    satcv_stat_t* arow = asums + (size_t)r * 2 * ald;
    a1 = arow[ch]; a2 = arow[ald + ch]; arow[ch] = 0.0; arow[ald + ch] = 0.0;
  }
#pragma unroll
  for (int o = 16; o > 0; o >>= 1) {
    d1 += __shfl_xor(d1, o, 64); d2 += __shfl_xor(d2, o, 64); a1 += __shfl_xor(a1, o, 64); a2 += __shfl_xor(a2, o, 64);
  }
  if (ch >= c || r != 0) return;
  const double sc = (double)scale[ch], sh = (double)shift[ch], mu = (double)mean[ch], rs = (double)rstd[ch];
  const double a2x = sc != 0.0 ? (a2 - (sh + sc * mu) * a1) * (rs / sc) : 0.0;
  const float s1 = (float)(d1 + a1), s2 = (float)(d2 + a2x);
  if (dbeta) dbeta[ch] = accumulate ? dbeta[ch] + s1 : s1;
  if (dgamma) dgamma[ch] = accumulate ? dgamma[ch] + s2 : s2;
  coef[ch] = s1 / count; coef[c + ch] = s2 / count;
}
extern "C" int satcv_bn_bwd_finalize2(satcv_stat_t* sums, int32_t sums_ld, satcv_stat_t* act_sums, int32_t act_sums_ld, int32_t c, float count,
                                      const float* scale, const float* shift, const float* mean, const float* rstd, float* dgamma, float* dbeta,
                                      float* coef, int32_t accumulate, void* stream) {
  SATCV_CHECK(act_sums && coef && scale && shift && mean && rstd && c > 0 && act_sums_ld >= c && (!sums || sums_ld >= c) && count > 0, "bn_bwd_finalize2: bad args");
  hipLaunchKernelGGL(bn_bwd_finalize2_kernel, dim3(cdiv(c, 8)), dim3(256), 0, (hipStream_t)stream, sums, sums_ld, act_sums, act_sums_ld, c, count, scale, shift,
                     mean, rstd, dgamma, dbeta, coef, accumulate);
  LAUNCH_OK("bn_bwd_finalize2");
  return SATCV_OK;
}
extern "C" int satcv_bn_bwd_finalize(satcv_stat_t* sums, int32_t sums_ld, int32_t c, float count, float* dgamma, float* dbeta, float* coef, int32_t accumulate,
                                     void* stream) {
  SATCV_CHECK(sums && coef && c > 0 && sums_ld >= c && count > 0, "bn_bwd_finalize: bad args");
  hipLaunchKernelGGL(bn_bwd_finalize_kernel, dim3(cdiv(c, 8)), dim3(256), 0, (hipStream_t)stream, sums, sums_ld, c, count, dgamma, dbeta, coef, accumulate);
  LAUNCH_OK("bn_bwd_finalize");
  return SATCV_OK;
}

#define HEAD_NCMAX 8
template <typename T>
__global__ void head_fwd_kernel(const satcv_head_desc d) {
  extern __shared__ float lds[];
  const int cin = d.cin, nc = d.ncls;
  float* lw = lds; float* lb = lw + cin * nc; float* lsc = lb + nc; float* lsh = lsc + cin;
  for (int i = threadIdx.x; i < cin * nc; i += blockDim.x) lw[i] = d.w[i];
  for (int i = threadIdx.x; i < nc; i += blockDim.x) lb[i] = d.b[i];
  for (int i = threadIdx.x; i < cin; i += blockDim.x) { lsc[i] = d.in_scale ? d.in_scale[i] : 1.f; lsh[i] = d.in_shift ? d.in_shift[i] : 0.f; }
  __syncthreads();
  const T* x = (const T*)d.x;
  const bool tr = d.in_scale != nullptr;
  for (long long p = blockIdx.x * (long long)blockDim.x + threadIdx.x; p < d.npix; p += (long long)gridDim.x * blockDim.x) {
    float z[HEAD_NCMAX];
#pragma unroll
    for (int k = 0; k < HEAD_NCMAX; ++k) z[k] = k < nc ? lb[k] : -INFINITY;
    for (int g = 0; g < cin / 8; ++g) {
      float v[8];
      load8<T>(x + p * d.ldx + g * 8, v);
#pragma unroll
      for (int e = 0; e < 8; ++e) {
        const int ch = g * 8 + e;
        const float a = tr ? fmaxf(v[e] * lsc[ch] + lsh[ch], 0.f) : v[e];
#pragma unroll
        for (int k = 0; k < HEAD_NCMAX; ++k) if (k < nc) z[k] += a * lw[ch * nc + k];
      }
    }
    if (d.activation == 2) {
#pragma unroll
      for (int k = 0; k < HEAD_NCMAX; ++k) if (k < nc) d.probs[p * nc + k] = z[k];
    } else if (d.activation == 0) {
      float mx = z[0]; int am = 0;
#pragma unroll
      for (int k = 1; k < HEAD_NCMAX; ++k) if (k < nc && z[k] > mx) { mx = z[k]; }
      float s = 0.f, ex[HEAD_NCMAX];
#pragma unroll
      for (int k = 0; k < HEAD_NCMAX; ++k) { ex[k] = k < nc ? expf(z[k] - mx) : 0.f; s += ex[k]; }
      const float inv = 1.f / s;
      float best = -1.f;
#pragma unroll
      for (int k = 0; k < HEAD_NCMAX; ++k) if (k < nc) {
        const float pr = ex[k] * inv;
        d.probs[p * nc + k] = pr;
        if (pr > best) { best = pr; am = k; }
      }
      if (d.classes) d.classes[p] = am;
    } else {
#pragma unroll
      for (int k = 0; k < HEAD_NCMAX; ++k) if (k < nc) {
        const float pr = 1.f / (1.f + expf(-z[k]));
        d.probs[p * nc + k] = pr;
        if (d.classes) d.classes[p * nc + k] = pr > d.thresh ? 1 : 0;
      }
    }
  }
}

template <typename T, int NC, int CIN>
__global__ __launch_bounds__(EW_BLOCK) void head_fwd_fast_kernel(const satcv_head_desc d) {
  float w[CIN][NC], b[NC], sc[CIN], sh[CIN];
  const bool tr = d.in_scale != nullptr;
#pragma unroll
  for (int c = 0; c < CIN; ++c) {
    sc[c] = tr ? d.in_scale[c] : 1.f; sh[c] = tr ? d.in_shift[c] : 0.f;
#pragma unroll
    for (int k = 0; k < NC; ++k) w[c][k] = d.w[c * NC + k];
  }
#pragma unroll
  for (int k = 0; k < NC; ++k) b[k] = d.b[k];
  const T* x = (const T*)d.x;
  for (long long p = blockIdx.x * (long long)blockDim.x + threadIdx.x; p < d.npix; p += (long long)gridDim.x * blockDim.x) {
    float z[NC];
#pragma unroll
// ... 846 lines not shown
```

satellite_computervision_amd/engine.py:

```python
import ctypes as C
import os
import itertools
from collections import defaultdict
from fractions import Fraction

import numpy as np
import torch

from . import ops, parallel
from ._lib import lib, check, F32, BF16, STAT_ROWS

_M16_DEFAULT = int(os.environ.get('SATCV_M16', '1'))

BN_EPS = 1e-3
BN_MOMENTUM = 0.99


class KTensor:
    _ids = itertools.count()

    def __init__(self, node, channels, down=Fraction(1), name=None):
        self.id = next(KTensor._ids)
        self.node, self.channels, self.down, self.name = node, channels, down, name

    @property
    def shape(self):
        return (None, None, None, self.channels)


class Node:
    def __init__(self, op, inputs, layer=None, **attrs):
        self.op, self.inputs, self.layer, self.attrs = op, list(inputs), layer, attrs
        self.outputs = []

    def out(self, channels, down, name=None):
        t = KTensor(self, channels, down, name)
        self.outputs.append(t)
        return t


class ParamSpec:
    def __init__(self, name, shape, kind, init):
        self.name, self.shape, self.kind, self.init = name, tuple(shape), kind, init

    @property
    def size(self):
        return int(np.prod(self.shape))


BIAS_NOISE = os.environ.get('SATCV_BN_BIAS_NOISE', '0') == '1'
WGRAD_LATE = os.environ.get('SATCV_WGRAD_LATE', '0') == '1'
CTBF = os.environ.get('SATCV_CTBF', '1') != '0'
CTBF_COUTS = tuple(int(v) for v in os.environ.get('SATCV_CTBF_COUTS', '32,64').split(',') if v)
FUSE_RESIDUAL = os.environ.get('SATCV_FUSE_RESIDUAL', '1') == '1'
EARLY_OPT = os.environ.get('SATCV_EARLY_OPT', '0') == '1'
EARLY_OPT_FRAC = 0.05
FUSE_DGRAD_ALL = os.environ.get('SATCV_FUSE_DGRAD_BN_BWD', '1') == '2'


def rup(a, b):
    return (a + b - 1) // b * b


def topo_nodes(outputs):
    seen, order = set(), []

    def visit(node):
        if id(node) in seen:
            return
        seen.add(id(node))
        for t in node.inputs:
            visit(t.node)
        order.append(node)
    for t in outputs:
        visit(t.node)
    return order


class TRef:

    def __init__(self, srcs, n, h, w, affine=None, relu=False):
        self.srcs, self.n, self.h, self.w = srcs, n, h, w
        self.affine, self.relu = affine, relu

    @property
    def c(self):
        return sum(c for _, c in self.srcs)


def _fp(t, off=0):
    return None if t is None else t.data_ptr() + t.element_size() * off


class Runtime:

    def __init__(self, model, dtype):
        if not torch.cuda.is_available():
            raise RuntimeError('satellite_computervision_amd needs a ROCm GPU (no CPU fallback)')
        self.model, self.dtype = model, dtype
        self.tdtype = ops.TORCH_DTYPE[dtype]
        self.esize = 2 if dtype == BF16 else 4
        self.dev = torch.device('cuda', torch.cuda.current_device())
        self.offsets = {}
        off = 0
        for p in model.param_specs:
            if p.kind in ('moving_mean', 'moving_var'):
                continue
            self.offsets[p.name] = off
            off += rup(p.size, 4)
        self.n_train = off
        soff = 0
        self.soffsets = {}
        for p in model.param_specs:
            if p.kind in ('moving_mean', 'moving_var'):
                self.soffsets[p.name] = soff
                soff += rup(p.size, 4)
        self.pflat = torch.zeros(max(off, 4), dtype=torch.float32, device=self.dev)
        self.gflat = torch.zeros_like(self.pflat)
        self.sflat = torch.zeros(max(soff, 4), dtype=torch.float32, device=self.dev)
        self.adam_m = self.adam_v = None
        self.adam_state = torch.tensor([1e-3, 0.0, 1.0, 0.0], dtype=torch.float32, device=self.dev)
        self.lr_mul = None
        self.dropout_seed = 0x5A7C0FFEE
        host = np.zeros(self.pflat.numel(), np.float32)
        hs = np.zeros(self.sflat.numel(), np.float32)
        self.zero_gamma = set()
        for p in model.param_specs:
            v = np.asarray(p.init(), np.float32).reshape(-1)
            self._note_gamma(p.name, v)
            if p.name in self.offsets:
                host[self.offsets[p.name]:self.offsets[p.name] + p.size] = v
            else:
                hs[self.soffsets[p.name]:self.soffsets[p.name] + p.size] = v
        self.pflat.copy_(torch.from_numpy(host))
        self.sflat.copy_(torch.from_numpy(hs))
        self.specs = {p.name: p for p in model.param_specs}
        self.packed = {}
        for node in model.nodes:
            if node.op in ('cba', 'convT'):
                lay = node.layer
# ... 481 lines not shown
                spatial = node.attrs['spatial']
                hw = r.h * r.w
                mask = self._z(*((n, ctot) if spatial else (n * hw, ctot)), dtype=torch.float32)
                out = self._z(n, r.h, r.w, ctot)
                rate = float(node.attrs['rate'])
                slot = len(self.dropouts)
                self.dropouts.append(dict(mask=mask, node=node))
                cnt = mask.numel()

                def gen(st, mask=mask, rate=rate, cnt=cnt, slot=slot):
                    check(lib.satcv_dropout_mask(self.rt.dropout_seed, (self.step_count << 8) + slot, rate, cnt, mask.data_ptr(), st))
                self.fwd.append(gen)
                off = 0
                mode = 0 if spatial else 1
                for (src, cs) in r.srcs:
                    a = r.affine
                    self.fwd.append(lambda st, src=src, cs=cs, off=off, a=a, rl=1 if r.relu else 0, mask=mask, ctot=ctot, mode=mode, out=out,
                                    hw=hw: check(lib.satcv_dropout_apply(
                        src.data_ptr(), cs, _fp(a['scale'], off) if a else None, _fp(a['shift'], off) if a else None, rl,
                        _fp(mask, off), ctot, mode, out.data_ptr() + off * es, ctot, n, hw, cs, dt, st)))
                    off += cs
                vals[tout.id] = TRef([(out, ctot)], n, r.h, r.w)
                ctx[id(node)] = dict(mask=mask, spatial=spatial, ctot=ctot, hw=hw, r=r)
            elif op == 'head':
                tin, tout = node.inputs[0], node.outputs[0]
                r = vals[tin.id]
                if len(r.srcs) != 1:
                    raise NotImplementedError('head on concatenated input')
                lay = node.layer
                ncls = tout.channels
                act = {'softmax': 0, 'sigmoid': 1, 'linear': 2}[node.attrs['activation']]
                (y, c) = r.srcs[0]
                npix = n * r.h * r.w
                probs = self._z(n, r.h, r.w, ncls, dtype=torch.float32)
                classes = self._z(*((n, r.h, r.w) if act != 1 else (n, r.h, r.w, ncls)), dtype=torch.int32)
                hd = ops.make_head_desc(x=y.data_ptr(), ldx=c, cin=c, w=rt.pptr(lay.name + '/kernel'), b=rt.pptr(lay.name + '/bias'),
                                        ncls=ncls, activation=act, npix=npix, dtype=dt,
                                        in_scale=_fp(r.affine['scale']) if r.affine else None,
                                        in_shift=_fp(r.affine['shift']) if r.affine else None,
                                        thresh=node.attrs.get('thresh', 0.5), probs=probs.data_ptr(), classes=classes.data_ptr())
                self.keep.append(hd)
                self.fwd.append(lambda st, hd=hd: check(lib.satcv_head_fwd(C.byref(hd), st)))
                self.outputs[tout.id] = probs
                ctx[id(node)] = dict(r=r, probs=probs, classes=classes, act=act, ncls=ncls)
                self.head = ctx[id(node)]
                self.head_node = node
            elif op == 'classes':
                hctx = ctx[id(node.inputs[0].node)]
                if 'thresh' in node.attrs:
                    node.inputs[0].node.attrs['thresh'] = node.attrs['thresh']
                self.outputs[node.outputs[0].id] = hctx['classes']
            else:
                raise NotImplementedError(f'op {op}')
        self.vals = vals
        self.node_ctx = ctx
        if training:
            self._build_backward(consumers, vals, acts, ctx, cat_stats)

    def _build_backward(self, consumers, vals, acts, ctx, cat_stats):
        rt, m, n = self.rt, self.rt.model, self.n
        dt, es = rt.dtype, rt.esize
        gact, gpool, gpool_f, graw = {}, {}, {}, {}
        self.dbg = {}
        _cnt = defaultdict(int)
        for nd in m.nodes:
            if nd.layer is not None:
                _cnt[nd.layer.name] += 1
        shared_layers = {k for k, v in _cnt.items() if v > 1}
        ws_need = 0
        wdescs = []
        DEFER = int(os.environ.get('SATCV_DEFER_REDUCE', '0')) != 0
        RED3 = (not DEFER) and self.side is not None and os.environ.get('SATCV_REDUCE_STREAM', '0') == '1'
        self.rstream = torch.cuda.Stream() if RED3 else None
        self._last_red_ev = None
        rpending = []
        rgroups = []
        fused_ws_need = 0
        fdescs = []
        h = self.head
        self.dlogits = self._z(n * h['r'].h * h['r'].w, h['ncls'], dtype=torch.float32)
        self.loss_buf = self._z(1, dtype=torch.float32)

        def bn_bwd_steps(da, ldda, dp, lddp, f, yraw, ldy, aff, aoff, sums, sums_off, sums_ld, c, hh, ww, dy, lddy, dbias,
                         dgamma, dbeta, accum=0, linear=0, frozen=False, second=None, act=None):
            coef = self._z(2, c, dtype=torch.float32)
            common = dict(yraw=yraw, ldy=ldy, scale=_fp(aff['scale'], aoff), shift=_fp(aff['shift'], aoff),
                          mean=_fp(aff['mean'], aoff), rstd=_fp(aff['rstd'], aoff), n=n, h=hh, w_=ww, c=c, dtype=dt,
                          f=f, sums=_fp(sums, sums_off), sums_ld=sums_ld, coef=_fp(coef), dy=dy, lddy_out=lddy, dbias=dbias, linear=linear)
            d = ops.make_bnbwd_desc(da=da, ldda=ldda, dpool=dp, lddp=lddp, **common, **(second or {}))
            self.keep.append(d)
            parts = act['parts'] if (act and not frozen) else set()
            need_da, need_dp = da is not None and 'skip' not in parts, dp is not None and 'pool' not in parts
            dr = d
            if parts and (need_da or need_dp):
                dr = ops.make_bnbwd_desc(da=da if need_da else None, ldda=ldda if need_da else 0, dpool=dp if need_dp else None,
                                         lddp=lddp if need_dp else 0, **common)
                self.keep.append(dr)
            cnt = float(n * hh * ww)
            red = lambda st: check(lib.satcv_bn_bwd_reduce(C.byref(dr), st))
            red.label = f"bn_bwd_reduce n{n} {hh}x{ww} c{c} f{f}{' (part)' if dr is not d else ''}"
            red.work = dict(kind='bn_bwd_reduce', px=n * hh * ww, c=c, esize=es)
            if parts and not (need_da or need_dp):
                red = None
            if parts:
                abuf = act['buf']
                fin0 = lambda st: check(lib.satcv_bn_bwd_finalize2(_fp(sums, sums_off) if red is not None else None, sums_ld, _fp(abuf), c, c, cnt,
                                                                   _fp(aff['scale'], aoff), _fp(aff['shift'], aoff), _fp(aff['mean'], aoff),
                                                                   _fp(aff['rstd'], aoff), dgamma, dbeta, _fp(coef), accum, st))
            else:
                fin0 = lambda st: check(lib.satcv_bn_bwd_finalize(_fp(sums, sums_off), sums_ld, c, cnt, dgamma, dbeta, _fp(coef), accum, st))
            if self.sync_bn:
                def fin(st):
                    parallel.allreduce_mean_(sums)
                    if parts:
                        parallel.allreduce_mean_(act['buf'])
                    fin0(st)
            else:
                fin = fin0
            app = lambda st: check(lib.satcv_bn_bwd_apply(C.byref(d), st))
            app.label = f"bn_bwd_apply n{n} {hh}x{ww} c{c} f{f}"
            app.work = dict(kind='bn_bwd_apply', px=n * hh * ww, c=c, esize=es)
            app.coef = coef
            if frozen:
                def fin_frozen(st):
                    sums.zero_()
                    coef.zero_()
                    if act:
                        act['buf'].zero_()
                return None, fin_frozen, app
            return red, fin, app

        act_sums = {}
        POOL_SUMS = getattr(rt.model, 'fuse_pool_bn_sums', True) and dt == ops.BF16
        ident = {}

        def ident_vecs(c):
            if c not in ident:
                ident[c] = (torch.ones(c, dtype=torch.float32, device=rt.dev), torch.zeros(c, dtype=torch.float32, device=rt.dev))
                self.keep.append(ident[c])
            return ident[c]

        def act_sums_for(t):
            if not POOL_SUMS or t.node.op != 'cba' or not t.node.attrs.get('bn', True) or not t.node.attrs.get('relu', True):
                return None
            if t.node.layer.bn_name in self.frozen or t.node.layer.bn_name in self.raw_bn or t.node.layer.name in shared_layers:
                return None
            if t.id not in act_sums:
                act_sums[t.id] = dict(buf=self._z(STAT_ROWS, 2, t.channels, dtype=torch.float64), parts=set())
            return act_sums[t.id]

        seen_layers = set()
        fused = {}
        HEAD_FAST = {(1, 16), (2, 16), (1, 32), (2, 32), (3, 32), (4, 32), (1, 64), (2, 64)}

        def fuse_target(t):
            if not rt.model.fuse_head_bn_bwd or t.id in gact or len(consumers[t.id]) != 1:
                return None
            P, pc = t.node, ctx.get(id(t.node))
            if P.op != 'cba' or pc['yoff'] != 0 or pc['ldy'] != pc['cout']:
                return None
            c, aff = pc['cout'], pc['aff']
            sums = self._z(STAT_ROWS, 2, c, dtype=torch.float64)
            return dict(mean=_fp(aff['mean']), rstd=_fp(aff['rstd']), sums=_fp(sums), sums_ld=c), sums

        def bst_target(t):
            if not getattr(rt.model, 'fuse_dgrad_bn_bwd', True) or dt != ops.BF16 or t.id in gact or t.id in gpool or len(consumers[t.id]) != 1:
                return None
            P, pc = t.node, ctx.get(id(t.node))
            if P.op == 'cba' and P.attrs.get('bn', True) and P.layer.bn_name not in self.frozen:
                c, aff, aoff = pc['cout'], pc['aff'], pc['aoff']
                b = dict(y=pc['y'].data_ptr() + pc['yoff'] * es, ld=pc['ldy'], relu=1 if P.attrs.get('relu', True) else 0)
            elif P.op == 'concat_bn_relu' and P.layer.name not in self.frozen:
                ra, rb, aff, ca, cb = pc['ra'], pc['rb'], pc['aff'], pc['ca'], pc['cb']
                if (P.inputs[1].node.op == 'convT' and BIAS_NOISE) or ca % 8:
                    return None
                c, aoff = ca + cb, 0
                b = dict(y=ra.srcs[0][0].data_ptr(), ld=ca, y1=rb.srcs[0][0].data_ptr(), ld1=cb, split=ca, relu=1)
            else:
                return None
            b.update(scale=_fp(aff['scale'], aoff), shift=_fp(aff['shift'], aoff), mean=_fp(aff['mean'], aoff), rstd=_fp(aff['rstd'], aoff))
            return b, c

        def act_form_unfit(t):
            P = t.node
            return (P.op == 'cba' and P.layer.bn_name in self.raw_bn) or (P.op == 'concat_bn_relu' and P.layer.name in self.raw_bn)

        def dgrad_step(t, **kw):
            kw.setdefault('tile_policy', self.tile_policy)
            if (POOL_SUMS and not kw.get('accumulate') and t.node.op == 'pool' and len(consumers[t.id]) == 1 and t.id not in gact
                    and len(vals[t.id].srcs) == 1 and vals[t.id].affine is None):
                ent = act_sums_for(t.node.inputs[0])
                if ent is not None and vals[t.id].srcs[0][1] == kw['cout'] == t.node.inputs[0].channels:
                    one, zero = ident_vecs(kw['cout'])
                    kwp = dict(kw, bst=dict(y=vals[t.id].srcs[0][0].data_ptr(), ld=kw['cout'], scale=_fp(one), shift=_fp(zero), mean=_fp(zero),
                                            rstd=_fp(one), relu=1), stats=_fp(ent['buf']), stats_ld=kw['cout'])
                    probe = ops.make_conv_desc(**kwp)
                    if lib.satcv_conv2d_igemm_pipelined(C.byref(probe)) == 1:
                        ent['parts'].add('pool')
                        fn = self._conv_step(role='dgrad', **kwp)
                        fn.label += ' +poolsums'
                        return fn
            bt = None if kw.get('accumulate') else bst_target(t)
            kdepth = kw.get('kh', 1) * kw.get('kw', 1) * (kw.get('c0', 0) + (kw.get('c1', 0) or 0))
            pays = FUSE_DGRAD_ALL or kdepth >= 2304 or (kdepth >= 1152 and kw['cout'] <= kw.get('c0', 0)) or kw.get('kh', 1) == 1
            if bt is not None and bt[1] == kw['cout'] and pays:
                sums = self._z(STAT_ROWS, 2, bt[1], dtype=torch.float64)
                kw2 = dict(kw, bst=bt[0], stats=_fp(sums), stats_ld=bt[1])
                probe = ops.make_conv_desc(**kw2)
                if lib.satcv_conv2d_igemm_pipelined(C.byref(probe)) == 1:
                    fused[t.id] = sums
                    fn = self._conv_step(role='dgrad', **kw2)
                    fn.label += ' +bnred'
                    return fn
            return self._conv_step(role='dgrad', **kw)

        def wgrad_step(r, dy, lddy, lay, cin_real, cout, hh, ww, k, dil, f=0, accum=0, last=False):
            nonlocal ws_need
            sa = self._src_args(r)
            if sa['x1'] is not None and sa['c0'] % 8:
                raise NotImplementedError(f'{lay.name}: training a convolution over a concatenation needs a first part of a multiple of 8 channels '
                                          f'(got {sa["c0"]}); inference has no such limit')
            d = ops.make_wgrad_desc(dy=dy, lddy=lddy, dw=rt.gptr(lay.name + '/kernel'), cin=cin_real, cout=cout, n=n, h=hh, w_=ww,
                                    dtype=dt, kh=k, kw=k, dil=dil, mode_dy=1 if f else 0, f=f if f else 1, transposed=1 if f else 0, accumulate=accum,
                                    whole_chip=1 if last else 0, **sa)
            nb = lib.satcv_conv2d_wgrad_workspace(C.byref(d))
            if nb < 0:
                raise RuntimeError(lib.satcv_last_error().decode())
            nvalid = (f * f if f else 1) * cout
            grp = None
            if DEFER and not accum and lay.name not in shared_layers and nvalid % 4 == 0 and not (k == 3 and dil > 1):
                d.defer_reduce = 1
                d._own_ws = nb
# ... 120 lines not shown
                dx = self._z(n, r.h, r.w, c)
                lay = node.layer
                hb = None
                ft = fuse_target(node.inputs[0]) if (cx['ncls'], c) in HEAD_FAST and r.affine else None
                if ft is not None:
                    hb = dict(mean=ft[0]['mean'], rstd=ft[0]['rstd'], sums=ft[0]['sums'], sums_ld=ft[0]['sums_ld'])
                    fused[node.inputs[0].id] = ft[1]
                hd = ops.make_head_desc(x=y.data_ptr(), ldx=c, cin=c, w=rt.pptr(lay.name + '/kernel'), b=rt.pptr(lay.name + '/bias'),
                                        ncls=cx['ncls'], activation=cx['act'], npix=n * r.h * r.w, dtype=dt,
                                        in_scale=_fp(r.affine['scale']) if r.affine else None,
                                        in_shift=_fp(r.affine['shift']) if r.affine else None,
                                        dlogits=self.dlogits.data_ptr(), dx=dx.data_ptr(), lddx=c,
                                        dw=rt.gptr(lay.name + '/kernel'), db=rt.gptr(lay.name + '/bias'), bnr=hb)
                self.keep.append(hd)
                self.bwd.append(lambda st, hd=hd: check(lib.satcv_head_bwd(C.byref(hd), st)))
                nb = lib.satcv_head_bwd_workspace(C.byref(hd))
                if nb > 0:
                    part = self._z(nb // 4, dtype=torch.float32)
                    hd.partials = part.data_ptr()
                    self.bwd.append(lambda st, hd=hd: check(lib.satcv_head_bwd_finalize(C.byref(hd), st)))
                gact[node.inputs[0].id] = (dx, 0, c)
                head_feed[node.inputs[0].id] = dict(hd=hd, ncls=cx['ncls'], c=c, w=rt.pptr(lay.name + '/kernel'), wname=lay.name + '/kernel',
                                                    fused_reduce=ft is not None)
            elif op == 'add_relu':
                ty, tsc = node.inputs
                g = gact.get(node.outputs[0].id)
                if g is None or cx is None:
                    continue
                c, hh, ww, out = cx['c'], cx['h'], cx['w'], cx['out']
                if g[1] != 0 or g[2] != c:
                    raise NotImplementedError('residual-join gradient in a channel slice')
                gb, cnt = g[0], n * hh * ww * c
                self.bwd.append(lambda st, out=out, gb=gb, cnt=cnt: check(lib.satcv_relu_bwd(out.data_ptr(), gb.data_ptr(), cnt, dt, st)))
                for t in (ty, tsc):
                    prev = gact.get(t.id)
                    if prev is None:
                        gact[t.id] = (gb, 0, c)
                    else:
                        if prev[1] != 0 or prev[2] != c:
                            raise NotImplementedError('gradient fan-in into a channel slice')
                        self.bwd.append(lambda st, pb=prev[0], gb=gb, npx=n * hh * ww, c=c: check(lib.satcv_add_act(
                            pb.data_ptr(), None, None, gb.data_ptr(), None, None, 0, pb.data_ptr(), npx, c, dt, st)))
            elif op == 'cba' and not node.attrs.get('bn', True):
                tin, tout = node.inputs[0], node.outputs[0]
                da = gact.get(tout.id)
                if da is None:
                    continue
                lay, r, cout = node.layer, cx['r'], cx['cout']
                if da[1] != 0 or da[2] != cout:
                    raise NotImplementedError('plain-convolution gradient in a channel slice')
                hh, ww, dyb = r.h, r.w, da[0]
                accum = 1 if lay.name in seen_layers else 0
                seen_layers.add(lay.name)
                bpart = self._z(max(lib.satcv_bias_grad_workspace(n * hh * ww, cout) // 4, 1), dtype=torch.float32)
                self.bwd.append(lambda st, dyb=dyb, cout=cout, npx=n * hh * ww, db=rt.gptr(lay.name + '/bias'), bpart=bpart: check(lib.satcv_bias_grad(
                    dyb.data_ptr(), cout, npx, cout, dt, db, bpart.data_ptr(), st)))
                pk = rt.packed[lay.name]
                self.bwd.append(wgrad_step(r, dyb.data_ptr(), cout, lay, pk['cin'], cout, hh, ww, cx['k'], cx['dil'], accum=accum))
                if tin.node.op != 'input':
                    cinp = r.c
                    prev = gact.get(tin.id)
                    if prev is not None and (prev[1] != 0 or prev[2] != cinp):
                        raise NotImplementedError('gradient fan-in into a channel slice')
                    gin = prev[0] if prev is not None else self._z(n, hh, ww, cinp)
                    self.bwd.append(dgrad_step(tin, x0=dyb.data_ptr(), c0=cout, w=pk['dgrad'].data_ptr(), y=gin.data_ptr(), ldy=cinp,
                                               n=n, h=hh, w_=ww, cout=cinp, cout_pad=rup(cinp, 32), kh=cx['k'], kw=cx['k'],
                                               dil=cx['dil'], dtype=dt, accumulate=1 if prev is not None else 0))
                    gact[tin.id] = (gin, 0, cinp)
            elif op == 'cba':
                tin, tout = node.inputs[0], node.outputs[0]
                da, dp = gact.get(tout.id), gpool.get(tout.id)
                graws = [gact[cn.outputs[0].id] for cn in consumers.get(tout.id, []) if cn.op == 'raw' and cn.outputs[0].id in gact]
                if da is None and dp is None:
                    if graws:
                        raise NotImplementedError('a convolution consumed only through its un-normalised output')
                    continue
                lay, r, y, aff, cout = node.layer, cx['r'], cx['y'], cx['aff'], cx['cout']
                yoff, ldy, aoff = cx['yoff'], cx['ldy'], cx['aoff']
                hh, ww = r.h, r.w
                pre = fused.get(tout.id)
                sums = pre if pre is not None else self._z(STAT_ROWS, 2, cout, dtype=torch.float64)
                accum = 1 if lay.name in seen_layers else 0
                seen_layers.add(lay.name)
                da_ptr = da[0].data_ptr() + da[1] * es if da is not None else None
                fz = None
                if (getattr(rt.model, 'fuse_thin_bwd', True) and dt == ops.BF16 and da is not None and dp is None and not graws and not BIAS_NOISE
                        and tin.node.op != 'input' and gact.get(tin.id) is None and cx['k'] == 3 and cx['dil'] == 1 and da[2] == ldy
                        and lay.name not in shared_layers):
                    pk = rt.packed[lay.name]
                    cinp = r.c
                    sa = self._src_args(r)
                    coef = self._z(2, cout, dtype=torch.float32)
                    gin = self._z(n, hh, ww, cinp)
                    fz = ops.make_bwdf_desc(g=da_ptr, yraw=y.data_ptr() + yoff * es, ldg=ldy, bn_scale=_fp(aff['scale'], aoff), bn_shift=_fp(aff['shift'], aoff),
                                            bn_mean=_fp(aff['mean'], aoff), bn_rstd=_fp(aff['rstd'], aoff), bn_coef=_fp(coef),
                                            linear=0 if node.attrs.get('relu', True) else 1, w_dgrad=pk['dgrad'].data_ptr(), dx=gin.data_ptr(), lddx=cinp,
                                            dw=rt.gptr(lay.name + '/kernel'), cin=pk['cin'], cout=cout, n=n, h=hh, w_=ww, dtype=dt, accumulate=accum, **sa)
                    bt = bst_target(tin) if (sa['in_relu'] and sa['in_scale'] is not None and not act_form_unfit(tin)) else None
                    sums_below = None
                    if bt is not None and bt[1] == cinp and bt[0].get('relu', 0) == 1:
                        sums_below = self._z(STAT_ROWS, 2, cinp, dtype=torch.float64)
                        fz.bst_sums, fz.bst_sums_ld, fz.bst_mean, fz.bst_rstd = _fp(sums_below), cinp, bt[0]['mean'], bt[0]['rstd']
                    hf = head_feed.get(tout.id)
                    if (hf is not None and getattr(rt.model, 'fuse_head_grad', True) and hf['ncls'] == 2 and hf['c'] == cout == 32 and cinp == 32
                            and hf['fused_reduce'] and pre is not None and len(consumers.get(tout.id, [])) == 1):
                        fz.hg_dlogits, fz.hg_w, fz.hg_ncls = self.dlogits.data_ptr(), hf['w'], 2
                        if lib.satcv_conv2d_bwd_fused_workspace(C.byref(fz)) < 0:
                            fz.hg_dlogits, fz.hg_w, fz.hg_ncls = None, None, 0
                        else:
                            hf['hd'].dx = None
                    nbf = lib.satcv_conv2d_bwd_fused_workspace(C.byref(fz))
                    if nbf < 0 and sums_below is not None:
                        fz.bst_sums, fz.bst_sums_ld, fz.bst_mean, fz.bst_rstd = None, 0, None, None
                        sums_below = None
                        nbf = lib.satcv_conv2d_bwd_fused_workspace(C.byref(fz))
                    if nbf < 0:
                        fz = None
                    elif sums_below is not None:
                        fused[tin.id] = sums_below
                if fz is not None:
                    if DEFER and not accum and lay.name not in shared_layers:
                        fz.defer_reduce = 1
                        fz._own_ws = nbf
                        rpending.append((fz, 'f', 4 * 9 * pk['cin'] * cout))
                    else:
                        fused_ws_need = max(fused_ws_need, nbf)
                    fdescs.append(fz)
                    self.keep.append(fz)
                    cnt = float(n * hh * ww)
                    frozen_bn = lay.bn_name in self.frozen
                    dg_, db_ = rt.gptr(lay.bn_name + '/gamma'), rt.gptr(lay.bn_name + '/beta')
                    bd = ops.make_bnbwd_desc(yraw=y.data_ptr() + yoff * es, ldy=ldy, scale=_fp(aff['scale'], aoff), shift=_fp(aff['shift'], aoff),
                                             mean=_fp(aff['mean'], aoff), rstd=_fp(aff['rstd'], aoff), n=n, h=hh, w_=ww, c=cout, dtype=dt,
                                             da=da_ptr, ldda=da[2], sums=_fp(sums), sums_ld=cout, coef=_fp(coef), linear=fz.linear)
                    self.keep.append(bd)
                    if frozen_bn:
                        def fin(st, sums=sums, coef=coef):
                            sums.zero_(); coef.zero_()
                    else:
                        if pre is None:
                            red = lambda st, bd=bd: check(lib.satcv_bn_bwd_reduce(C.byref(bd), st))
                            red.label = f"bn_bwd_reduce n{n} {hh}x{ww} c{cout} f1"
                            red.work = dict(kind='bn_bwd_reduce', px=n * hh * ww, c=cout, esize=es)
                            self.bwd.append(red)
                        fin0 = lambda st, sums=sums, coef=coef, cnt=cnt, dg_=dg_, db_=db_, accum=accum, c_=cout: check(lib.satcv_bn_bwd_finalize(
                            _fp(sums), c_, c_, cnt, dg_, db_, _fp(coef), accum, st))
                        if self.sync_bn:
                            def fin(st, fin0=fin0, sums=sums):
                                parallel.allreduce_mean_(sums)
                                fin0(st)
                        else:
                            fin = fin0
                    self.bwd.append(fin)
                    fstep = lambda st, fz=fz: check(lib.satcv_conv2d_bwd_fused(C.byref(fz), st))
                    fstep.label = f"bwd_fused k3 n{n} {hh}x{ww} {sa['c0']}+{sa['c1']}->{cout}{' +bnred' if fz.bst_sums else ''}{' +headgrad' if fz.hg_dlogits else ''}"
                    fstep.work = dict(kind='bwd_fused', taps=9, px=n * hh * ww, cin=pk['cin'], cout=cout, esize=es)
                    self.bwd.append(fstep)
                    gact[tin.id] = (gin, 0, cinp)
                    self.dbg['dx:' + lay.name] = gin
                    self.dbg['dyparts:' + lay.name] = dict(g=da, y=y, yoff=yoff, ldy=ldy, aff=aff, aoff=aoff, cout=cout, coef=coef, linear=fz.linear)
                    if fz.hg_dlogits:
                        self.dbg['dyparts:' + lay.name]['head'] = (self.dlogits, head_feed[tout.id]['wname'])
                    self.dbg['_ctx:' + lay.name] = dict(da=da, dp=dp, y=y, yoff=yoff, ldy=ldy, aff=aff, aoff=aoff, cout=cout)
                    continue
                dy = self._z(n, hh, ww, cout)
                red, fin, app = bn_bwd_steps(da_ptr, da[2] if da is not None else 0, dp[0].data_ptr() if dp is not None else None,
                                             cout, gpool_f.get(tout.id, 1), y.data_ptr() + yoff * es, ldy, aff, aoff, sums, 0, cout, cout, hh, ww,
                                             dy.data_ptr(), cout, rt.gptr(lay.name + '/bias') if BIAS_NOISE else None,
                                             rt.gptr(lay.bn_name + '/gamma'), rt.gptr(lay.bn_name + '/beta'), accum,
                                             linear=0 if node.attrs.get('relu', True) else 1, frozen=lay.bn_name in self.frozen,
                                             act=act_sums.get(tout.id) if (act_sums.get(tout.id) or {}).get('parts') else None)
                fzp = None
                amax = self.amax_of.get(tout.id)
                if (amax is not None and getattr(rt.model, 'fuse_pool_bwd', True) and dt == ops.BF16 and da is not None and dp is not None
                        and gpool_f.get(tout.id, 1) == 2 and not graws and not BIAS_NOISE and cx['k'] == 3 and cx['dil'] == 1 and da[2] == ldy
                        and dp[1] == 0 and lay.bn_name not in self.frozen and gact.get(tin.id) is None and lay.name not in shared_layers):
                    pkp = rt.packed[lay.name]
                    sa = self._src_args(r)
                    want_dx = tin.node.op != 'input'
                    cinp = r.c
                    ginp = self._z(n, hh, ww, cinp) if want_dx else None
                    fzp = ops.make_bwdf_desc(g=da_ptr, yraw=y.data_ptr() + yoff * es, ldg=ldy, bn_scale=_fp(aff['scale'], aoff), bn_shift=_fp(aff['shift'], aoff),
                                             bn_mean=_fp(aff['mean'], aoff), bn_rstd=_fp(aff['rstd'], aoff), bn_coef=_fp(app.coef), linear=0,
                                             w_dgrad=pkp['dgrad'].data_ptr() if want_dx else None, dx=ginp.data_ptr() if want_dx else None,
                                             lddx=cinp if want_dx else 0, dw=rt.gptr(lay.name + '/kernel'), cin=pkp['cin'], cout=cout, n=n, h=hh, w_=ww,
                                             dtype=dt, accumulate=accum, dpool=dp[0].data_ptr(), lddp=dp[2], amax=amax.data_ptr(), **sa)
                    ent = None
                    if (want_dx and POOL_SUMS and tin.node.op == 'pool' and len(consumers[tin.id]) == 1 and sa['in_scale'] is None
                            and len(vals[tin.id].srcs) == 1 and tin.node.inputs[0].channels == cinp):
                        ent = act_sums_for(tin.node.inputs[0])
                    if ent is not None:
                        fzp.bst_sums, fzp.bst_sums_ld, fzp.bst_act_form = _fp(ent['buf']), cinp, 1
                    nbp = lib.satcv_conv2d_bwd_fused_workspace(C.byref(fzp))
                    if nbp < 0:
                        fzp = None
                    elif ent is not None:
                        ent['parts'].add('pool')
                if fzp is not None:
                    if DEFER and not accum and lay.name not in shared_layers:
                        fzp.defer_reduce = 1
                        fzp._own_ws = nbp
                        rpending.append((fzp, 'f', 4 * 9 * pkp['cin'] * cout))
                    else:
                        fused_ws_need = max(fused_ws_need, nbp)
                    fdescs.append(fzp)
                    self.keep.append(fzp)
                    self.bwd += [fin] if (pre is not None or red is None) else [red, fin]
                    fstep = lambda st, fzp=fzp: check(lib.satcv_conv2d_bwd_fused(C.byref(fzp), st))
                    fstep.label = f"bwd_fused k3 n{n} {hh}x{ww} {sa['c0']}+{sa['c1']}->{cout} pooled{'' if want_dx else ' nodx'}{' +poolsums' if fzp.bst_sums else ''}"
                    fstep.work = dict(kind='bwd_fused', taps=9, px=n * hh * ww, cin=pkp['cin'], cout=cout, esize=es, nodx=not want_dx, pooled=True)
                    self.bwd.append(fstep)
                    if want_dx:
                        gact[tin.id] = (ginp, 0, cinp)
                        self.dbg['dx:' + lay.name] = ginp
                    self.dbg['dyparts:' + lay.name] = dict(g=da, y=y, yoff=yoff, ldy=ldy, aff=aff, aoff=aoff, cout=cout, coef=app.coef, linear=0,
                                                           dp=dp, amax=amax)
                    self.dbg['_ctx:' + lay.name] = dict(da=da, dp=dp, y=y, yoff=yoff, ldy=ldy, aff=aff, aoff=aoff, cout=cout)
                    continue
                self.bwd += [fin, app] if (pre is not None or red is None) else [red, fin, app]
                for gr in graws:
                    if gr[1] != 0 or gr[2] != cout:
                        raise NotImplementedError('raw-output gradient in a channel slice')
                    bpart = self._z(max(lib.satcv_bias_grad_workspace(n * hh * ww, cout) // 4, 1), dtype=torch.float32)
                    self.bwd.append(lambda st, dy=dy, gb=gr[0], npx=n * hh * ww, cout=cout, db=rt.gptr(lay.name + '/bias'), bpart=bpart: (
                        check(lib.satcv_bias_grad(gb.data_ptr(), cout, npx, cout, dt, db, bpart.data_ptr(), st)),
                        check(lib.satcv_add_act(dy.data_ptr(), None, None, gb.data_ptr(), None, None, 0, dy.data_ptr(), npx, cout, dt, st))))
                self.dbg['dy:' + lay.name] = dy
                self.dbg['_ctx:' + lay.name] = dict(da=da, dp=dp, y=y, yoff=yoff, ldy=ldy, aff=aff, aoff=aoff, cout=cout)
                pk = rt.packed[lay.name]
                wstep = wgrad_step(r, dy.data_ptr(), cout, lay, pk['cin'], cout, hh, ww, cx['k'], cx['dil'], accum=accum,
                                   last=tin.node.op == 'input' and len(m.inputs) == 1 and os.environ.get('SATCV_WGRAD_LAST_FULL', '1') != '0')
                if not WGRAD_LATE:
                    self.bwd.append(wstep)
                if tin.node.op != 'input':
                    cinp = r.c
                    prev = gact.get(tin.id)
                    if prev is not None and (prev[1] != 0 or prev[2] != cinp):
                        raise NotImplementedError('gradient fan-in into a channel slice')
                    gin = prev[0] if prev is not None else self._z(n, hh, ww, cinp)
                    self.bwd.append(dgrad_step(tin, x0=dy.data_ptr(), c0=cout, w=pk['dgrad'].data_ptr(), y=gin.data_ptr(), ldy=cinp,
                                               n=n, h=hh, w_=ww, cout=cinp, cout_pad=rup(cinp, 32), kh=cx['k'], kw=cx['k'],
                                               dil=cx['dil'], dtype=dt, accumulate=1 if prev is not None else 0))
                    gact[tin.id] = (gin, 0, cinp)
                    self.dbg['dx:' + lay.name] = gin
                if WGRAD_LATE:
                    self.bwd.append(wstep)
            elif op == 'dropout':
                tin, tout = node.inputs[0], node.outputs[0]
                g = gact.get(tout.id)
                if g is None or cx is None:
                    continue
                if g[1] != 0 or g[2] != cx['ctot']:
                    raise NotImplementedError('dropout gradient in a channel slice')
                gt, mask, ctot, hw = g[0], cx['mask'], cx['ctot'], cx['hw']
                mode = 0 if cx['spatial'] else 1
                self.bwd.append(lambda st, gt=gt, mask=mask, ctot=ctot, hw=hw, mode=mode: check(lib.satcv_dropout_apply(
                    gt.data_ptr(), ctot, None, None, 0, _fp(mask), ctot, mode, gt.data_ptr(), ctot, n, hw, ctot, dt, st)))
                gact[tin.id] = (gt, 0, ctot)
            elif op == 'concat':
                g = gact.get(node.outputs[0].id)
                if g is None:
                    continue
                off = 0
                for t in node.inputs:
                    gact[t.id] = (g[0], g[1] + off, g[2])
                    off += t.channels
            elif op == 'pool':
                tin, tout = node.inputs[0], node.outputs[0]
                if tout.id in gact:
                    if gact[tout.id][1] != 0:
                        raise NotImplementedError('pooled gradient in a channel slice')
                    gpool[tin.id] = gact[tout.id]
                    gpool_f[tin.id] = cx['f']
            elif op == 'concat_bn_relu':
                ta, tb = node.inputs
                tout = node.outputs[0]
                g = gact.get(tout.id)
                if g is None:
                    continue
                ra, rb, aff, ca, cb = cx['ra'], cx['rb'], cx['aff'], cx['ca'], cx['cb']
                ctot = ca + cb
                hh, ww = ra.h, ra.w
                pre = fused.get(tout.id)
                sums = pre if pre is not None else self._z(STAT_ROWS, 2, ctot, dtype=torch.float64)
                dskip = self._z(n, hh, ww, ca)
                du = self._z(n, hh, ww, cb)
                bn = node.layer.name
                upl = tb.node.layer
                if g[2] != ctot:
                    raise NotImplementedError('decoder concat gradient in a channel slice')
                gptr_ = g[0].data_ptr() + g[1] * es
                if not (tb.node.op == 'convT' and BIAS_NOISE) and ca % 8 == 0:
                    sec = dict(yraw1=rb.srcs[0][0].data_ptr(), ldy1=cb, dy1=du.data_ptr(), lddy1=cb, c_split=ca)
                    ctbf = None
                    cxt = ctx.get(id(tb.node)) if tb.node.op == 'convT' else None
                    if (CTBF and dt == ops.BF16 and cxt is not None and bn not in self.frozen and upl.name not in shared_layers and cxt['f'] == 2
                            and cb in CTBF_COUTS and len(consumers.get(tb.id, [])) == 1):
                        rT = cxt['r']
                        saT = self._src_args(rT)
                        probe = ops.make_ctbf_desc(g=gptr_ + ca * es, ldg=ctot, yup=rb.srcs[0][0].data_ptr(), ldy=cb, bn_scale=None, bn_shift=None, bn_mean=None,
                                                   bn_rstd=None, bn_c1=None, bn_c2=None, x=saT['x0'], ldx=saT['c0'], w_dgrad=rt.packed[upl.name]['dgrad'].data_ptr(),
                                                   w_npad=rup(rT.c, 32), dx=saT['x0'], lddx=rT.c, dw=rt.gptr(upl.name + '/kernel'), cin=rT.c, cout=cb, n=n,
                                                   h=rT.h, w_=rT.w, dtype=dt)
                        if saT['x1'] is None and saT['c0'] == rT.c == rt.packed[upl.name]['cin'] and lib.satcv_convt_bwd_fused_workspace(C.byref(probe)) > 0:
                            ctbf = dict(g=gptr_ + ca * es, ldg=ctot, yup=rb.srcs[0][0].data_ptr(), ldy=cb, aff=aff, aoff=ca, ctot=ctot)
                            sec['dy1'] = None
                    ent = None
                    if (bn not in self.frozen and ta.id not in gact and any(cn.op == 'pool' for cn in consumers[ta.id])
                            and len([cn for cn in consumers[ta.id] if cn.op != 'pool']) == 1 and ta.channels == ca):
                        ent = act_sums_for(ta)
                    if ent is not None:
                        sec.update(sk_sums=_fp(ent['buf']), sk_sums_ld=ca)
                        ent['parts'].add('skip')
                    r_, f_, a_ = bn_bwd_steps(gptr_, ctot, None, 0, 1, ra.srcs[0][0].data_ptr(), ca, aff, 0, sums, 0, ctot, ctot, hh, ww,
                                              dskip.data_ptr(), ca, None, rt.gptr(bn + '/gamma'), rt.gptr(bn + '/beta'), frozen=bn in self.frozen,
                                              second=sec)
                    if ent is not None:
                        a_.label += ' +skipsums'
                    if ctbf is not None:
                        a_.label += ' (skip half)'
                        a_.work = dict(kind='bn_bwd_apply', px=n * hh * ww, c=ca, esize=es)
                        ctbf['coef'] = a_.coef
                    self.bwd += [f_, a_] if (pre is not None or r_ is None) else [r_, f_, a_]
                    gact[ta.id] = (dskip, 0, ca)
                    self.dbg['dskip:' + bn] = dskip
                    self.dbg['du:' + bn] = du
                    graw[tb.id] = ctbf if ctbf is not None else du
                    continue
                ra_, fa_, aa_ = bn_bwd_steps(gptr_, ctot, None, 0, 1, ra.srcs[0][0].data_ptr(), ca, aff, 0, sums, 0, ctot, ca, hh, ww,
                                             dskip.data_ptr(), ca, None, rt.gptr(bn + '/gamma'), rt.gptr(bn + '/beta'), frozen=bn in self.frozen)
                rb_, fb_, ab_ = bn_bwd_steps(gptr_ + ca * es, ctot, None, 0, 1, rb.srcs[0][0].data_ptr(), cb, aff, ca, sums, ca, ctot, cb,
                                             hh, ww, du.data_ptr(), cb, rt.gptr(upl.name + '/bias') if (tb.node.op == 'convT' and BIAS_NOISE) else None,
                                             rt.gptr(bn + '/gamma') + 4 * ca, rt.gptr(bn + '/beta') + 4 * ca, frozen=bn in self.frozen)
                self.bwd += [fa_, fb_, aa_, ab_] if (pre is not None or ra_ is None) else [ra_, rb_, fa_, fb_, aa_, ab_]
                gact[ta.id] = (dskip, 0, ca)
                self.dbg['dskip:' + bn] = dskip
                self.dbg['du:' + bn] = du
                graw[tb.id] = du
            elif op == 'convT':
                tin, tout = node.inputs[0], node.outputs[0]
                du = graw.get(tout.id)
                if du is None:
                    continue
                lay, r, cout, f = node.layer, cx['r'], cx['cout'], cx['f']
                pk = rt.packed[lay.name]
                if isinstance(du, dict):
                    cb_, sa = du, self._src_args(r)
                    cinp = r.c
                    gin = self._z(n, r.h, r.w, cinp)
                    af_, ao_, ct_ = cb_['aff'], cb_['aoff'], cb_['ctot']
                    fz = ops.make_ctbf_desc(g=cb_['g'], ldg=cb_['ldg'], yup=cb_['yup'], ldy=cb_['ldy'], bn_scale=_fp(af_['scale'], ao_), bn_shift=_fp(af_['shift'], ao_),
                                            bn_mean=_fp(af_['mean'], ao_), bn_rstd=_fp(af_['rstd'], ao_), bn_c1=_fp(cb_['coef'], ao_), bn_c2=_fp(cb_['coef'], ct_ + ao_),
                                            x=sa['x0'], ldx=sa['c0'], in_scale=sa['in_scale'], in_shift=sa['in_shift'], in_relu=sa['in_relu'],
                                            w_dgrad=pk['dgrad'].data_ptr(), w_npad=rup(cinp, 32), dx=gin.data_ptr(), lddx=cinp, dw=rt.gptr(lay.name + '/kernel'),
                                            cin=cinp, cout=cout, n=n, h=r.h, w_=r.w, dtype=dt)
                    bt = bst_target(tin) if (sa['in_relu'] and sa['in_scale'] is not None and not act_form_unfit(tin)) else None
                    if bt is not None and bt[1] == cinp and bt[0].get('relu', 0) == 1:
                        sums_below = self._z(STAT_ROWS, 2, cinp, dtype=torch.float64)
                        fz.bst_sums, fz.bst_sums_ld, fz.bst_mean, fz.bst_rstd = _fp(sums_below), cinp, bt[0]['mean'], bt[0]['rstd']
                        fused[tin.id] = sums_below
                    nbc = lib.satcv_convt_bwd_fused_workspace(C.byref(fz))
                    if nbc <= 0:
                        raise RuntimeError('convt_bwd_fused: the probe accepted this shape, the final descriptor did not')
                    wsc = self._z(max(nbc // 4, 1), dtype=torch.float32)
                    fz.workspace, fz.workspace_bytes = wsc.data_ptr(), nbc
                    self.keep.append(fz)
                    cstep = lambda st, fz=fz: check(lib.satcv_convt_bwd_fused(C.byref(fz), st))
                    cstep.label = f"convt_bwd_fused n{n} {r.h}x{r.w} {cinp}<-4x{cout}{' +bnred' if fz.bst_sums else ''}"
                    cstep.work = dict(kind='convt_bwd_fused', px=n * r.h * r.w, cin=cinp, cout=cout, esize=es)
                    self.bwd.append(cstep)
                    gact[tin.id] = (gin, 0, cinp)
                    self.dbg['dx:' + lay.name] = gin
                    continue
                wstep = wgrad_step(r, du.data_ptr(), cout, lay, pk['cin'], cout, r.h, r.w, 1, 1, f=f)
                if not WGRAD_LATE:
                    self.bwd.append(wstep)
                cinp = r.c
                gin = self._z(n, r.h, r.w, cinp)
                self.bwd.append(dgrad_step(tin, x0=du.data_ptr(), c0=cout, w=pk['dgrad'].data_ptr(), y=gin.data_ptr(), ldy=cinp, n=n, h=r.h,
                                           w_=r.w, cout=cinp, cout_pad=rup(cinp, 32), kh=1, kw=1, dil=1, mode_in=1, f=f, dtype=dt))
                if WGRAD_LATE:
                    self.bwd.append(wstep)
                gact[tin.id] = (gin, 0, cinp)
                self.dbg['dx:' + lay.name] = gin
        if prev_node is not None:
            grads_ready(prev_node)
        if ws_need:
            ws = self._z(max(ws_need // 4, 1), dtype=torch.float32)
            for d in wdescs:
                if not d.defer_reduce:
                    d.workspace, d.workspace_bytes = ws.data_ptr(), ws_need
        if fused_ws_need:
            wsf = self._z(max(fused_ws_need // 4, 1), dtype=torch.float32)
            for d in fdescs:
                if not d.defer_reduce:
                    d.workspace, d.workspace_bytes = wsf.data_ptr(), fused_ws_need
        flush_reduces(force=True)
        if rgroups:
            from ._lib import ReduceJob
            own = [d for g in rgroups for d, _ in g['items']]
            arena = self._z(max(sum((d._own_ws + 255) // 256 * 256 for d in own) // 4, 1), dtype=torch.float32)
            off = 0
            for d in own:
                d.workspace, d.workspace_bytes = arena.data_ptr() + off, d._own_ws
                off += (d._own_ws + 255) // 256 * 256
            for g in rgroups:
                jobs, prefix, tot = [], [], 0
                for d, kind in g['items']:
                    j = ReduceJob()
                    check((lib.satcv_conv2d_wgrad_reduce_job if kind == 'w' else lib.satcv_conv2d_bwd_fused_reduce_job)(C.byref(d), C.byref(j)))
                    prefix.append(tot)
# ... 29 lines not shown
```

satellite_computervision_amd/ops.py:

```python
import ctypes as C
import torch

from . import _lib
from ._lib import lib, check, ConvDesc, WgradDesc, BnBwdDesc, HeadDesc, F32, BF16, FP8, FP8X, STAT_ROWS

TORCH_DTYPE = {F32: torch.float32, BF16: torch.bfloat16, FP8: torch.float8_e4m3fn, FP8X: torch.float8_e4m3fn}
DTYPE_CODE = {torch.float32: F32, torch.bfloat16: BF16, torch.float8_e4m3fn: FP8}


def rup(a, b):
    return (a + b - 1) // b * b


def stream_ptr():
    return C.c_void_p(torch.cuda.current_stream().cuda_stream)


def ptr(t):
    if t is None:
        return None
    assert t.is_cuda, 'satcv ops need device tensors (no CPU fallback)'
    return C.c_void_p(t.data_ptr())


# ... 160 lines not shown
def conv_bwd_fused(g, yraw, scale, shift, mean, rstd, coef, x, w_dgrad, cin, cout, *, x1=None, in_scale=None, in_shift=None, in_relu=False,
                   linear=False, accumulate_into=None, bst=None, dpool=None, amax=None, want_dx=True, head=None):
    n, h, w_, c0 = x.shape
    c1 = x1.shape[-1] if x1 is not None else 0
    dx = torch.empty(n, h, w_, c0 + c1, dtype=x.dtype, device=x.device) if want_dx else None
    dw = accumulate_into if accumulate_into is not None else torch.empty(3, 3, cin, cout, dtype=torch.float32, device=x.device)
    d = make_bwdf_desc(g=_p(g), yraw=_p(yraw), ldg=g.shape[-1] if g is not None else yraw.shape[-1], bn_scale=_p(scale), bn_shift=_p(shift), bn_mean=_p(mean), bn_rstd=_p(rstd),
                       bn_coef=_p(coef), x0=_p(x), c0=c0, x1=_p(x1), c1=c1, in_scale=_p(in_scale), in_shift=_p(in_shift), in_relu=in_relu,
                       w_dgrad=_p(w_dgrad), dx=_p(dx), lddx=c0 + c1, dw=_p(dw), cin=cin, cout=cout, n=n, h=h, w_=w_, dtype=DTYPE_CODE[x.dtype],
                       linear=linear, accumulate=accumulate_into is not None, dpool=_p(dpool), lddp=dpool.shape[-1] if dpool is not None else 0,
                       amax=_p(amax), **(dict(hg_dlogits=_p(head[0]), hg_w=_p(head[1]), hg_ncls=head[0].shape[-1]) if head else {}),
                       **(dict(bst_sums=_p(bst['sums']), bst_sums_ld=bst['sums'].shape[-1], bst_mean=_p(bst.get('mean')), bst_rstd=_p(bst.get('rstd')),
                               bst_act_form=bst.get('act_form', 0)) if bst else {}))
    nb = lib.satcv_conv2d_bwd_fused_workspace(C.byref(d))
    if nb < 0:
        return None
    ws = torch.empty(max(nb // 4, 1), dtype=torch.float32, device=x.device)
    d.workspace, d.workspace_bytes = ws.data_ptr(), nb
    check(lib.satcv_conv2d_bwd_fused(C.byref(d), stream_ptr()))
    return dx, dw


def conv2d_wgrad(x, dy, cin, cout, *, kh=3, kw=3, dil=1, x1=None, in_scale=None, in_shift=None, in_relu=False,
                 transposed_f=0, dw=None):
    n, h, w_, c0 = x.shape
    dtype = DTYPE_CODE[x.dtype]
    c1 = x1.shape[-1] if x1 is not None else 0
    f = transposed_f
    if dw is None:
        shape = (f, f, cout, cin) if f else (kh, kw, cin, cout)
        dw = torch.empty(shape, dtype=torch.float32, device=x.device)
    d = make_wgrad_desc(x0=_p(x), c0=c0, x1=_p(x1), c1=c1, dy=_p(dy), lddy=dy.shape[-1], dw=_p(dw), cin=cin, cout=cout,
                        n=n, h=h, w_=w_, dtype=dtype, in_scale=_p(in_scale), in_shift=_p(in_shift), in_relu=in_relu,
                        kh=1 if f else kh, kw=1 if f else kw, dil=dil, mode_dy=1 if f else 0, f=f if f else 1,
                        transposed=1 if f else 0)
    nbytes = lib.satcv_conv2d_wgrad_workspace(C.byref(d))
    if nbytes < 0:
        raise _lib.SatcvError(lib.satcv_last_error().decode())
    ws = torch.empty(max(nbytes // 4, 1), dtype=torch.float32, device=x.device)
    d.workspace, d.workspace_bytes = ws.data_ptr(), nbytes
    check(lib.satcv_conv2d_wgrad(C.byref(d), stream_ptr()))
    return dw


def bn_finalize_train(stats, count, gamma, beta, moving_mean, moving_var, eps=1e-3, momentum=0.99, updates=1, bessel=False):
    c = gamma.numel()
    dev = gamma.device
    scale, shift, mean, rstd = (torch.empty(c, dtype=torch.float32, device=dev) for _ in range(4))
    check(lib.satcv_bn_finalize_train(ptr(stats), stats.shape[-1], c, float(count), ptr(gamma), ptr(beta), eps, momentum,
                                      updates, int(bessel), ptr(moving_mean), ptr(moving_var), ptr(scale), ptr(shift),
                                      ptr(mean), ptr(rstd), stream_ptr()))
    return scale, shift, mean, rstd


def bn_affine_infer(gamma, beta, moving_mean, moving_var, eps=1e-3):
    c = gamma.numel()
    scale = torch.empty(c, dtype=torch.float32, device=gamma.device)
    shift = torch.empty_like(scale)
    check(lib.satcv_bn_affine_infer(ptr(gamma), ptr(beta), ptr(moving_mean), ptr(moving_var), eps, c, ptr(scale), ptr(shift), stream_ptr()))
    return scale, shift


def bn_relu_pool(yraw, scale, shift, f, want_act=True, want_pool=True, stats=None):
    n, h, w_, c = yraw.shape
    act = torch.empty_like(yraw) if want_act else None
    pooled = torch.empty(n, h // f, w_ // f, c, dtype=yraw.dtype, device=yraw.device) if want_pool else None
    check(lib.satcv_bn_relu_pool(ptr(yraw), ptr(scale), ptr(shift), ptr(act), 0, ptr(pooled), ptr(stats),
                                 stats.shape[-1] if stats is not None else 0, n, h, w_, c, f, DTYPE_CODE[yraw.dtype], stream_ptr()))
    return act, pooled


def bn_relu_pool_amax(yraw, scale, shift, f):
    n, h, w_, c = yraw.shape
    act = torch.empty_like(yraw)
    pooled = torch.empty(n, h // f, w_ // f, c, dtype=yraw.dtype, device=yraw.device)
    amax = torch.empty(n, h // f, w_ // f, c, dtype=torch.uint8, device=yraw.device)
    check(lib.satcv_bn_relu_pool_amax(ptr(yraw), ptr(scale), ptr(shift), ptr(act), 0, ptr(pooled), ptr(amax), None, 0, n, h, w_, c, f,
                                      DTYPE_CODE[yraw.dtype], stream_ptr()))
    return act, pooled, amax


def make_bnbwd_desc(*, yraw, ldy, scale, shift, mean, rstd, n, h, w_, c, dtype, da=None, ldda=0, dpool=None, lddp=0, f=1,
                    sums=None, sums_ld=0, coef=None, dy=None, lddy_out=0, dbias=None, linear=0, yraw1=None, ldy1=0, dy1=None, lddy1=0,
                    c_split=0, sk_sums=None, sk_sums_ld=0):
    d = BnBwdDesc()
    d.sk_sums, d.sk_sums_ld = sk_sums, sk_sums_ld
    d.linear = linear
    d.yraw1, d.ldy1, d.dy1, d.lddy1, d.c_split = yraw1, ldy1, dy1, lddy1, c_split
    d.da, d.ldda, d.dpool, d.lddp, d.f = da, ldda, dpool, lddp, f
    d.yraw, d.ldy = yraw, ldy
    d.scale, d.shift, d.mean, d.rstd = scale, shift, mean, rstd
    d.sums, d.sums_ld, d.coef = sums, sums_ld, coef
    d.dy, d.lddy_out, d.dbias = dy, lddy_out, dbias
    d.n, d.h, d.w_, d.c, d.dtype = n, h, w_, c, dtype
    return d


def bn_relu_bwd(yraw, scale, shift, mean, rstd, da=None, dpool=None, f=1, want_dbias=False):
    n, h, w_, c = yraw.shape
    dev, dtype = yraw.device, DTYPE_CODE[yraw.dtype]
    sums = new_stats(c, dev)
    coef = torch.empty(2, c, dtype=torch.float32, device=dev)
    dgamma = torch.empty(c, dtype=torch.float32, device=dev)
    dbeta = torch.empty_like(dgamma)
    dy = torch.empty_like(yraw)
    dbias = torch.zeros(c, dtype=torch.float32, device=dev) if want_dbias else None
    d = make_bnbwd_desc(yraw=_p(yraw), ldy=c, scale=_p(scale), shift=_p(shift), mean=_p(mean), rstd=_p(rstd), n=n, h=h, w_=w_,
                        c=c, dtype=dtype, da=_p(da), ldda=da.shape[-1] if da is not None else 0, dpool=_p(dpool),
                        lddp=dpool.shape[-1] if dpool is not None else 0, f=f, sums=_p(sums), sums_ld=c, coef=_p(coef),
                        dy=_p(dy), lddy_out=c, dbias=_p(dbias))
    check(lib.satcv_bn_bwd_reduce(C.byref(d), stream_ptr()))
    check(lib.satcv_bn_bwd_finalize(ptr(sums), c, c, float(n * h * w_), ptr(dgamma), ptr(dbeta), ptr(coef), 0, stream_ptr()))
    check(lib.satcv_bn_bwd_apply(C.byref(d), stream_ptr()))
    return dy, dgamma, dbeta, dbias


def bn_relu_bwd_concat(y0, y1, scale, shift, mean, rstd, da):
    n, h, w_, c0 = y0.shape
    c1 = y1.shape[-1]
    c = c0 + c1
    dev, dtype = y0.device, DTYPE_CODE[y0.dtype]
    sums = new_stats(c, dev)
    coef = torch.empty(2, c, dtype=torch.float32, device=dev)
    dgamma = torch.empty(c, dtype=torch.float32, device=dev)
    dbeta = torch.empty_like(dgamma)
    dy0, dy1 = torch.empty_like(y0), torch.empty_like(y1)
    d = make_bnbwd_desc(yraw=_p(y0), ldy=c0, scale=_p(scale), shift=_p(shift), mean=_p(mean), rstd=_p(rstd), n=n, h=h, w_=w_, c=c, dtype=dtype,
                        da=_p(da), ldda=c, sums=_p(sums), sums_ld=c, coef=_p(coef), dy=_p(dy0), lddy_out=c0,
                        yraw1=_p(y1), ldy1=c1, dy1=_p(dy1), lddy1=c1, c_split=c0)
    check(lib.satcv_bn_bwd_reduce(C.byref(d), stream_ptr()))
    check(lib.satcv_bn_bwd_finalize(ptr(sums), c, c, float(n * h * w_), ptr(dgamma), ptr(dbeta), ptr(coef), 0, stream_ptr()))
    check(lib.satcv_bn_bwd_apply(C.byref(d), stream_ptr()))
    return dy0, dy1, dgamma, dbeta


def make_head_desc(*, x, ldx, cin, w, b, ncls, activation, npix, dtype, in_scale=None, in_shift=None, thresh=0.5,
                   probs=None, classes=None, dlogits=None, dx=None, lddx=0, dw=None, db=None, bnr=None, partials=None):
    d = HeadDesc()
    d.partials = partials
    d.x, d.ldx, d.cin = x, ldx, cin
    d.in_scale, d.in_shift, d.w, d.b = in_scale, in_shift, w, b
    d.ncls, d.activation, d.thresh = ncls, activation, thresh
    d.probs, d.classes, d.dlogits = probs, classes, dlogits
    d.dx, d.lddx, d.dw, d.db = dx, lddx, dw, db
    d.npix, d.dtype = npix, dtype
    if bnr:
        for k, v in bnr.items():
            setattr(d, 'bnr_' + k, v)
    return d


def head_fwd(x, w, b, activation='softmax', in_scale=None, in_shift=None, thresh=0.5):
    n, h, w_, c = x.shape
    cin, ncls = w.shape
    act = 0 if activation == 'softmax' else 1
    probs = torch.empty(n, h, w_, ncls, dtype=torch.float32, device=x.device)
    classes = torch.empty((n, h, w_) if act == 0 else (n, h, w_, ncls), dtype=torch.int32, device=x.device)
    d = make_head_desc(x=_p(x), ldx=c, cin=cin, w=_p(w), b=_p(b), ncls=ncls, activation=act, npix=n * h * w_,
                       dtype=DTYPE_CODE[x.dtype], in_scale=_p(in_scale), in_shift=_p(in_shift), thresh=thresh,
                       probs=_p(probs), classes=_p(classes))
    check(lib.satcv_head_fwd(C.byref(d), stream_ptr()))
    return probs, classes


def head_bwd(x, w, dlogits, in_scale=None, in_shift=None):
    n, h, w_, c = x.shape
    cin, ncls = w.shape
    dx = torch.empty(n, h, w_, c, dtype=x.dtype, device=x.device)
    if c > cin:
# ... 81 lines not shown
```

Measured before the change: 8387 tiles/s.

## Fold decoder concat skip-branch BN backward into pooled encoder fused backward

```diff
diff --git a/include/satcv.h b/include/satcv.h
--- a/include/satcv.h
+++ b/include/satcv.h
@@ -115,6 +115,9 @@
   const void* dpool; int32_t lddp; const void* amax;
   const float* hg_dlogits; const float* hg_w; int32_t hg_ncls;
   int32_t defer_reduce;
+  const void* cat_g; int32_t cat_ld;
+  const float* cat_scale; const float* cat_shift; const float* cat_mean; const float* cat_rstd; const float* cat_coef; int32_t cat_c;
+  satcv_stat_t* fold_sums; int32_t fold_sums_ld;
 } satcv_bwdf_desc;
 int64_t satcv_conv2d_bwd_fused_workspace(const satcv_bwdf_desc* d);
 int satcv_conv2d_bwd_fused(const satcv_bwdf_desc* d, void* stream);
@@ -177,6 +180,7 @@
   void* dy1; int32_t lddy1;
   int32_t c_split;
   satcv_stat_t* sk_sums; int32_t sk_sums_ld;
+  satcv_stat_t* fold_sums; int32_t fold_sums_ld;
 } satcv_bnbwd_desc;
 int satcv_bn_bwd_reduce(const satcv_bnbwd_desc* d, void* stream);
 int satcv_bn_bwd_finalize(satcv_stat_t* sums, int32_t sums_ld, int32_t c, float count, float* dgamma,
@@ -185,6 +189,10 @@
 int satcv_bn_bwd_finalize2(satcv_stat_t* sums, int32_t sums_ld, satcv_stat_t* act_sums, int32_t act_sums_ld, int32_t c, float count,
                            const float* scale, const float* shift, const float* mean, const float* rstd, float* dgamma, float* dbeta,
                            float* coef, int32_t accumulate, void* stream);
+int satcv_bn_bwd_finalize2_fold(satcv_stat_t* sums, int32_t sums_ld, satcv_stat_t* act_sums, int32_t act_sums_ld, satcv_stat_t* fold_sums,
+                                int32_t fold_sums_ld, int32_t c, float count, const float* scale, const float* shift, const float* mean,
+                                const float* rstd, const float* cat_scale, const float* cat_mean, const float* cat_rstd, const float* cat_coef,
+                                int32_t cat_c, float cat_eps, float* dgamma, float* dbeta, float* coef, int32_t accumulate, void* stream);
 
 int satcv_relu_bwd(const void* act, void* g, int64_t count, int32_t dtype, void* stream);
 int64_t satcv_bias_grad_workspace(int64_t npix, int32_t c);
diff --git a/satellite_computervision_amd/_lib.py b/satellite_computervision_amd/_lib.py
--- a/satellite_computervision_amd/_lib.py
+++ b/satellite_computervision_amd/_lib.py
@@ -60,7 +60,9 @@
                 ('workspace', c_vp), ('workspace_bytes', c_i64), ('dtype', c_i32), ('accumulate', c_i32),
                 ('bst_sums', c_vp), ('bst_sums_ld', c_i32), ('bst_mean', c_vp), ('bst_rstd', c_vp), ('bst_act_form', c_i32),
                 ('dpool', c_vp), ('lddp', c_i32), ('amax', c_vp),
-                ('hg_dlogits', c_vp), ('hg_w', c_vp), ('hg_ncls', c_i32), ('defer_reduce', c_i32)]
+                ('hg_dlogits', c_vp), ('hg_w', c_vp), ('hg_ncls', c_i32), ('defer_reduce', c_i32),
+                ('cat_g', c_vp), ('cat_ld', c_i32), ('cat_scale', c_vp), ('cat_shift', c_vp), ('cat_mean', c_vp), ('cat_rstd', c_vp),
+                ('cat_coef', c_vp), ('cat_c', c_i32), ('fold_sums', c_vp), ('fold_sums_ld', c_i32)]
 
 
 class CtbfDesc(C.Structure):
@@ -86,7 +88,7 @@
                 ('dy', c_vp), ('lddy_out', c_i32), ('dbias', c_vp),
                 ('n', c_i32), ('h', c_i32), ('w_', c_i32), ('c', c_i32), ('dtype', c_i32), ('linear', c_i32),
                 ('yraw1', c_vp), ('ldy1', c_i32), ('dy1', c_vp), ('lddy1', c_i32), ('c_split', c_i32),
-                ('sk_sums', c_vp), ('sk_sums_ld', c_i32)]
+                ('sk_sums', c_vp), ('sk_sums_ld', c_i32), ('fold_sums', c_vp), ('fold_sums_ld', c_i32)]
 
 
 class HeadDesc(C.Structure):
@@ -157,6 +159,8 @@
     'satcv_bn_bwd_finalize': (C.c_int, [c_vp, c_i32, c_i32, c_f32, c_vp, c_vp, c_vp, c_i32, c_vp]),
     'satcv_bn_bwd_apply': (C.c_int, [C.POINTER(BnBwdDesc), c_vp]),
     'satcv_bn_bwd_finalize2': (C.c_int, [c_vp, c_i32, c_vp, c_i32, c_i32, c_f32, c_vp, c_vp, c_vp, c_vp, c_vp, c_vp, c_vp, c_i32, c_vp]),
+    'satcv_bn_bwd_finalize2_fold': (C.c_int, [c_vp, c_i32, c_vp, c_i32, c_vp, c_i32, c_i32, c_f32, c_vp, c_vp, c_vp, c_vp,
+                                              c_vp, c_vp, c_vp, c_vp, c_i32, c_f32, c_vp, c_vp, c_vp, c_i32, c_vp]),
     'satcv_maxpool': (C.c_int, [c_vp, c_vp, c_i32, c_i32, c_i32, c_i32, c_i32, c_i32, c_i32, c_i32, c_vp]),
     'satcv_affine_requant': (C.c_int, [c_vp, c_i32, c_vp, c_vp, c_i32, c_vp, c_i32, c_i64, c_i32, c_i32, c_i32, c_vp]),
     'satcv_add_act': (C.c_int, [c_vp, c_vp, c_vp, c_vp, c_vp, c_vp, c_i32, c_vp, c_i64, c_i32, c_i32, c_vp]),
diff --git a/satellite_computervision_amd/csrc/conv_bwd_fused.hip b/satellite_computervision_amd/csrc/conv_bwd_fused.hip
--- a/satellite_computervision_amd/csrc/conv_bwd_fused.hip
+++ b/satellite_computervision_amd/csrc/conv_bwd_fused.hip
@@ -25,6 +25,9 @@
   int bst_act_form;
   const void* dp; int lddp; const unsigned char* amax;
   const float* hg_dl; const float* hg_w;
+  const void* cg; int ldc;
+  const float* c_scale; const float* c_shift; const float* c_mean; const float* c_rstd; const float* c_coef; int c_c;
+  satcv_stat_t* fold_sums; int fold_ld;
 };
 
 __device__ __forceinline__ bf16x4 tr_read4(const bf16* p) {
@@ -32,9 +35,10 @@
   return __builtin_bit_cast(bf16x4, v);
 }
 
-template <int CIN, int COUT, int NW, int WPS, bool POOL = false, bool NODG = false, int CINS = CIN, bool HG = false>
+template <int CIN, int COUT, int NW, int WPS, bool POOL = false, bool NODG = false, int CINS = CIN, bool HG = false, bool CAT = false, int FOLDG = 0>
 __global__ __launch_bounds__(NW * 64, WPS) void bwd_fused_kernel(const BwdfArgs a, const int total_tiles) {
   static_assert(!HG || !POOL, "the head feeds a decoder block");
+  static_assert(!CAT || POOL, "the concatenation's skip gradient feeds a pooled encoder block");
   typedef bf16 T;
   constexpr int TW = 32, TH = 8, BM = 256, RL = TH + 2, CL = TW + 2, PITCH = CL, EL = 8, NTHREADS = NW * 64;
   constexpr int SD = COUT / 8, SX = CIN / 8, SXR = CINS / 8;
@@ -60,7 +64,7 @@
   constexpr size_t W_BYTES = (size_t)W_ITEMS * EL * sizeof(T);
   constexpr size_t O_BYTES = (size_t)BM * (CIN + 8) * sizeof(T);
   constexpr bool O_ALIAS = O_BYTES <= (size_t)SD * DSTRIDE * sizeof(T);
-  constexpr size_t TAB_BYTES = (size_t)(SD * 32 + SX * 16 + (HG ? 2 * COUT : 0)) * sizeof(float);
+  constexpr size_t TAB_BYTES = (size_t)(SD * 32 + SX * 16 + (HG ? 2 * COUT : 0) + (CAT ? SD * 40 : 0)) * sizeof(float);
   static_assert(!NODG || O_ALIAS || true, "");
   constexpr size_t O_OFF = O_ALIAS ? 0 : (R0_BYTES + W_BYTES + TAB_BYTES + 127) / 128 * 128;
   extern __shared__ __attribute__((aligned(16))) unsigned char smem_raw[];
@@ -70,6 +74,11 @@
   float* tabD = reinterpret_cast<float*>(smem_raw + R0_BYTES + W_BYTES);
   float* tabX = tabD + SD * 32;
   float* tabH = tabX + SX * 16;
+  float* tabC = tabH + (HG ? 2 * COUT : 0);
+  constexpr int VPR_ = CIN / 8, NFT = FOLDG ? NTHREADS / VPR_ * FOLDG : 1;
+  constexpr size_t F_OFF = ((O_ALIAS ? R0_BYTES + W_BYTES + TAB_BYTES : O_OFF + O_BYTES) + 127) / 128 * 128;
+  T* ldsR = reinterpret_cast<T*>(smem_raw + F_OFF);
+  float* facc = reinterpret_cast<float*>(smem_raw + F_OFF + (size_t)FOLDG * XSTRIDE * sizeof(T));
 
   const int tid = threadIdx.x, lane = tid & 63, wave = tid >> 6;
   const int r = lane & 31, hh = lane >> 5;
@@ -90,6 +99,16 @@
       t[0] = a.hg_w[ch * 2]; t[8] = a.hg_w[ch * 2 + 1];
     }
   }
+  if constexpr (CAT) {
+    for (int ch = tid; ch < COUT; ch += NTHREADS) {
+      const float sc = a.c_scale[ch];
+      float* t = tabC + (ch >> 3) * 40 + (ch & 7);
+      t[0] = sc; t[8] = a.c_shift[ch]; t[16] = a.c_mean[ch]; t[24] = sc * a.c_coef[ch]; t[32] = sc * a.c_rstd[ch] * a.c_coef[a.c_c + ch];
+    }
+  }
+  if constexpr (FOLDG > 0) {
+    for (int i = tid; i < 16 * NFT; i += NTHREADS) facc[i] = 0.f;
+  }
   for (int ch = tid; ch < CINS; ch += NTHREADS) {
     float* t = tabX + (ch >> 3) * 16 + (ch & 7);
     t[0] = a.in_scale ? a.in_scale[ch] : 1.f; t[8] = a.in_scale ? a.in_shift[ch] : 0.f;
@@ -111,6 +130,7 @@
   }
   auto d_item = [&](int j) -> int { return (int)((d_pk[j / 3] >> (10 * (j % 3))) & 0x3ffu); };
   const int g_rowstride = a.e.w_ * a.ldg;
+  const int c_rowstride = a.e.w_ * a.ldc;
   const unsigned gy_lane = (unsigned)slot_d * EL;
   const int xch0 = slot_x * EL;
   const bool xsecond = xch0 >= a.c0;
@@ -167,6 +187,10 @@
         asm volatile("" : "+v"(poff));
         rdl[j] = reinterpret_cast<const float2*>(a.hg_dl)[pb + poff];
         ry[j] = gload8<T>(yb + off);
+      } else if constexpr (CAT) {
+        unsigned offc = ok ? (unsigned)(__mul24(L, c_rowstride) + __mul24(c, a.ldc)) + gy_lane : (unsigned)(c_rowstride + a.ldc) + gy_lane;
+        asm volatile("" : "+v"(offc));
+        rg[j] = gload8<T>(reinterpret_cast<const T*>(a.cg) + pb * a.ldc + offc); ry[j] = gload8<T>(yb + off);
       } else if (!FABL(32)) { rg[j] = gload8<T>(gb + off); ry[j] = gload8<T>(yb + off); }
       else { rg[j] = zero8<T>(); ry[j] = zero8<T>(); rg[j].q[0].x = off; }
     }
@@ -250,6 +274,17 @@
           unpack8<T>(rg[j], gv);
         }
         unpack8<T>(ry[j], yv);
+        if constexpr (CAT) {
+          int coff = slot_d * 40;
+          asm volatile("" : "+v"(coff));
+          const float* cp = tabC + coff;
+#pragma unroll
+          for (int e = 0; e < 8; ++e) {
+            const float av = round_to<T>(fmaxf(yv[e] * prm[e] + prm[8 + e], 0.f));
+            const float gmc = fmaf(av, cp[e], cp[8 + e]) > 0.f ? gv[e] : 0.f;
+            gv[e] = round_to<T>(fmaf(-cp[32 + e], av - cp[16 + e], fmaf(cp[e], gmc, -cp[24 + e])));
+          }
+        }
         if constexpr (POOL) {
           float pv[8];
           unpack8<T>(rp[j], pv);
@@ -292,6 +327,7 @@
 #pragma unroll
       for (int j = 0; j < XI; ++j) {
         Raw8<T> v = rx[j];
+        if constexpr (FOLDG > 0) { if (slot_x < FOLDG) lstore8<T>(ldsR + x_l0 + j * (XPIX_STEP * EL), v); }
         if (xaff) v = affine8_lim(v, sc, sh, xrelu_lim);
         lstore8<T>(ldsX + x_l0 + j * (XPIX_STEP * EL), v);
       }
@@ -410,6 +446,9 @@
       T* yp = reinterpret_cast<T*>(a.e.y) + ((size_t)(tn0 * a.e.h + ty0) * a.e.w_ + tx0) * a.e.ldy + vq * 8;
       const unsigned row_pitch = (unsigned)a.e.w_ * a.e.ldy;
       const T* xact = ldsX + vq * XSTRIDE;
+      float fz[FOLDG ? 8 : 1], fg[FOLDG ? 8 : 1];
+#pragma unroll
+      for (int e = 0; e < (FOLDG ? 8 : 1); ++e) { fz[e] = 0.f; fg[e] = 0.f; }
 #pragma unroll 2
       for (int it = tid; it < BM * VPR; it += NTHREADS) {
         const int q = it / VPR;
@@ -425,6 +464,24 @@
             bs1[e] += af > 0.f ? df : 0.f;
             bs2[e] += df * af;
           }
+          if constexpr (FOLDG > 0) {
+            if (vq < FOLDG) {
+              const bf16x8 r8 = *reinterpret_cast<const bf16x8*>(ldsR + vq * XSTRIDE + q * EL);
+#pragma unroll
+              for (int e = 0; e < 8; ++e) {
+                const bool z = (float)r8[e] == 0.f;
+                fz[e] += z ? 1.f : 0.f;
+                fg[e] += (z && (float)a8[e] > 0.f) ? (float)d8[e] : 0.f;
+              }
+            }
+          }
+        }
+      }
+      if constexpr (FOLDG > 0) {
+        if (BST && a.bst_sums && vq < FOLDG) {
+          const int k = (tid / VPR) * FOLDG + vq;
+#pragma unroll
+          for (int e = 0; e < 8; ++e) { facc[e * NFT + k] += fg[e]; facc[(8 + e) * NFT + k] += fz[e]; }
         }
       }
     }
@@ -475,17 +532,28 @@
       atomicAdd(rowp + tid, (satcv_stat_t)t1);
       atomicAdd(rowp + a.bst_ld + tid, (satcv_stat_t)s2);
     }
-  }
-}
-
-template <int CIN, int COUT, int NW, bool NODG = false>
+    if constexpr (FOLDG > 0) {
+      if (tid < FOLDG * 8) {
+        const int vq = tid >> 3, e = tid & 7;
+        double g1 = 0.0, z1 = 0.0;
+        for (int k = 0; k < NTHREADS / VPR; ++k) { g1 += (double)facc[e * NFT + k * FOLDG + vq]; z1 += (double)facc[(8 + e) * NFT + k * FOLDG + vq]; }
+        satcv_stat_t* rowf = a.fold_sums + (size_t)(blockIdx.x % SATCV_STAT_ROWS) * 2 * a.fold_ld;
+        atomicAdd(rowf + tid, (satcv_stat_t)g1);
+        atomicAdd(rowf + a.fold_ld + tid, (satcv_stat_t)z1);
+      }
+    }
+  }
+}
+
+template <int CIN, int COUT, int NW, bool NODG = false, bool CAT = false, int FOLDG = 0>
 struct BwdfGeom {
   static constexpr int SD = COUT / 8, SX = CIN / 8;
   static constexpr size_t R0 = ((size_t)(SD * (10 * 34 * 8) + SX * (256 * 8 + 32)) * 2 + 127) / 128 * 128;
   static constexpr size_t O_BYTES = (size_t)256 * (CIN + 8) * 2;
   static constexpr bool O_ALIAS = O_BYTES <= (size_t)SD * (10 * 34 * 8) * 2;
-  static constexpr size_t BASE = R0 + (NODG ? 0 : (size_t)9 * SD * CIN * 16) + (size_t)(SD * 32 + SX * 16 + 2 * COUT) * 4;
-  static constexpr size_t LDS0 = O_ALIAS ? BASE : (BASE + 127) / 128 * 128 + O_BYTES;
+  static constexpr size_t BASE = R0 + (NODG ? 0 : (size_t)9 * SD * CIN * 16) + (size_t)(SD * 32 + SX * 16 + 2 * COUT + (CAT ? SD * 40 : 0)) * 4;
+  static constexpr size_t LDS00 = O_ALIAS ? BASE : (BASE + 127) / 128 * 128 + O_BYTES;
+  static constexpr size_t LDS0 = FOLDG ? (LDS00 + 127) / 128 * 128 + (size_t)FOLDG * (256 * 8 + 32) * 2 + (size_t)16 * (NW * 64 / (CIN / 8) * FOLDG) * 4 : LDS00;
   static constexpr size_t RED = (size_t)16 * NW * 64 * 4;
   static constexpr size_t LDS = LDS0 > RED ? LDS0 : RED;
 };
@@ -513,6 +581,13 @@
   if (d->h % 8 != 0 || d->w_ % 32 != 0) return false;
   if (d->ldg % 8 != 0 || ((uintptr_t)d->g % 16) != 0 || ((uintptr_t)d->yraw % 16) != 0) return false;
   if (d->hg_dlogits && (!d->hg_w || d->hg_ncls != 2 || d->dpool || ((uintptr_t)d->hg_dlogits % 8) != 0)) return false;
+  if (d->cat_g) {
+    if (!d->dpool || d->cat_ld % 8 != 0 || d->cat_ld < d->cout || ((uintptr_t)d->cat_g % 16) != 0 || (long long)d->w_ * d->cat_ld >= (1 << 23)) return false;
+    if (!d->cat_scale || !d->cat_shift || !d->cat_mean || !d->cat_rstd || !d->cat_coef || d->cat_c < d->cout || d->linear) return false;
+  }
+  if (d->fold_sums) {
+    if (d->dpool || d->hg_dlogits || !d->bst_sums || d->bst_act_form || d->c0 != 32 || d->c1 != 32 || d->cout != 32 || d->fold_sums_ld < 32) return false;
+  }
   if (d->dx && (d->lddx % 8 != 0 || ((uintptr_t)d->dx % 16) != 0)) return false;
   if ((long long)d->w_ * d->ldg >= (1 << 23)) return false;
   if (d->dpool) {
@@ -527,9 +602,9 @@
   return true;
 }
 
-template <int CIN, int COUT, int NW, int WPS, bool POOL = false, bool NODG = false, int CINS = CIN, bool HG = false>
+template <int CIN, int COUT, int NW, int WPS, bool POOL = false, bool NODG = false, int CINS = CIN, bool HG = false, bool CAT = false, int FOLDG = 0>
 static int bwdf_launch(const satcv_bwdf_desc* d, hipStream_t st, bool query, int64_t* ws_bytes, satcv_reduce_job* job = nullptr) {
-  using G = BwdfGeom<CIN, COUT, NW, NODG>;
+  using G = BwdfGeom<CIN, COUT, NW, NODG, CAT, FOLDG>;
   static_assert(G::LDS <= 160 * 1024, "tile + weights exceed the LDS");
   const long long total = (long long)d->n * (d->h / 8) * (d->w_ / 32);
   const int grid = bwdf_grid(G::LDS, NW, WPS, total);
@@ -549,7 +624,9 @@
   a.bst_sums = d->bst_sums; a.bst_ld = d->bst_sums_ld; a.bst_mean = d->bst_mean; a.bst_rstd = d->bst_rstd; a.bst_act_form = d->bst_act_form;
   a.dp = d->dpool; a.lddp = d->lddp; a.amax = reinterpret_cast<const unsigned char*>(d->amax);
   a.hg_dl = d->hg_dlogits; a.hg_w = d->hg_w;
-  auto kern = bwd_fused_kernel<CIN, COUT, NW, WPS, POOL, NODG, CINS, HG>;
+  a.cg = d->cat_g; a.ldc = d->cat_ld; a.c_scale = d->cat_scale; a.c_shift = d->cat_shift; a.c_mean = d->cat_mean; a.c_rstd = d->cat_rstd;
+  a.c_coef = d->cat_coef; a.c_c = d->cat_c; a.fold_sums = d->fold_sums; a.fold_ld = d->fold_sums_ld;
+  auto kern = bwd_fused_kernel<CIN, COUT, NW, WPS, POOL, NODG, CINS, HG, CAT, FOLDG>;
   { const int rc = satcv_ensure_dynamic_lds(reinterpret_cast<const void*>(kern), G::LDS); if (rc) return rc; }
   const double flops = (NODG ? 2.0 : 4.0) * d->n * d->h * d->w_ * (double)CINS * COUT * 9;
   satcv_prof_begin(3, flops, st);
@@ -565,9 +642,14 @@
   int cin_s;
   if (!bwdf_shape_ok(d, cin_s)) return SATCV_ERR_UNSUPPORTED;
   if (d->dpool) {
+    if (d->cat_g) {
+      if (d->dx) return bwdf_launch<32, 64, 4, 1, true, false, 32, false, true>(d, st, query, ws_bytes, job);
+      return bwdf_launch<32, 32, 8, 2, true, true, 16, false, true>(d, st, query, ws_bytes, job);
+    }
     if (d->dx) return bwdf_launch<32, 64, 4, 1, true, false>(d, st, query, ws_bytes, job);
     return bwdf_launch<32, 32, 8, 2, true, true, 16>(d, st, query, ws_bytes, job);
   }
+  if (d->fold_sums) return bwdf_launch<64, 32, 8, 2, false, false, 64, false, false, 4>(d, st, query, ws_bytes, job);
   if (cin_s == 32 && d->hg_dlogits) return bwdf_launch<32, 32, 8, 2, false, false, 32, true>(d, st, query, ws_bytes, job);
   if (d->hg_dlogits) return SATCV_ERR_UNSUPPORTED;
   if (cin_s == 32) return bwdf_launch<32, 32, 8, 2>(d, st, query, ws_bytes, job);
@@ -587,7 +669,7 @@
 }
 
 extern "C" int satcv_conv2d_bwd_fused(const satcv_bwdf_desc* d, void* stream) {
-  SATCV_CHECK(d && (d->g || d->hg_dlogits) && d->yraw && d->x0 && d->dw && d->workspace && (d->dx == nullptr || d->w_dgrad), "bwd_fused: null pointer");
+  SATCV_CHECK(d && (d->g || d->hg_dlogits || d->cat_g) && d->yraw && d->x0 && d->dw && d->workspace && (d->dx == nullptr || d->w_dgrad), "bwd_fused: null pointer");
   SATCV_CHECK(d->bn_scale && d->bn_shift && d->bn_mean && d->bn_rstd && d->bn_coef, "bwd_fused: BatchNorm coefficients missing");
   SATCV_CHECK((d->c1 == 0) == (d->x1 == nullptr) && d->n > 0 && d->h > 0 && d->w_ > 0, "bwd_fused: bad dims");
   SATCV_CHECK(!d->bst_sums || (d->bst_sums_ld >= d->c0 + d->c1 && (d->bst_act_form ? d->in_scale == nullptr
diff --git a/satellite_computervision_amd/csrc/elementwise.hip b/satellite_computervision_amd/csrc/elementwise.hip
--- a/satellite_computervision_amd/csrc/elementwise.hip
+++ b/satellite_computervision_amd/csrc/elementwise.hip
@@ -522,7 +522,7 @@
     for (int i = threadIdx.x; i < c; i += blockDim.x) atomicAdd(d.dbias + i, lds[i]);
   }
 }
-template <typename T, bool APPLY>
+template <typename T, bool APPLY, bool FD = false>
 __global__ __launch_bounds__(EW_BLOCK) void bn_bwd_dense_kernel(const satcv_bnbwd_desc d, const int rev, const int cld) {
   extern __shared__ float lds[];
   const int c = d.c, G = c / 8;
@@ -538,13 +538,13 @@
   T* dy = second ? (T*)d.dy1 + (g * 8 - d.c_split) : (T*)d.dy + g * 8;
   const int ldy = second ? d.ldy1 : d.ldy, lddy = second ? d.lddy1 : d.lddy_out;
   const bool sk = APPLY && d.sk_sums != nullptr && !second;
-  float sc[8], sh[8], mu[8], rs[8], c1[8], c2[8], s1[8], s2[8];
+  float sc[8], sh[8], mu[8], rs[8], c1[8], c2[8], s1[8], s2[8], f1[8], f2[8];
 #pragma unroll
   for (int e = 0; e < 8; ++e) {
     const int ch = g * 8 + e;
     sc[e] = d.scale[ch]; sh[e] = d.shift[ch]; mu[e] = d.mean[ch]; rs[e] = d.rstd[ch];
     c1[e] = APPLY ? d.coef[ch] : 0.f; c2[e] = APPLY ? d.coef[cld + ch] : 0.f;
-    s1[e] = 0.f; s2[e] = 0.f;
+    s1[e] = 0.f; s2[e] = 0.f; f1[e] = 0.f; f2[e] = 0.f;
   }
   if (active) {
     const unsigned pfirst = gid / G;
@@ -570,13 +570,22 @@
           if (sk) { s1[e] += v[e] > 0.f ? o[e] : 0.f; s2[e] += o[e] * v[e]; }
           else s1[e] += o[e];
         }
-        else { s1[e] += gg; s2[e] += gg * xh; }
+        else {
+          s1[e] += gg; s2[e] += gg * xh;
+          if constexpr (FD) { if (v[e] == 0.f) { f1[e] += gg; f2[e] += 1.f; } }
+        }
       }
       if (APPLY) store8<T>(oq, o);
       yq += ystep; dq += dstep; oq += ostep;
     }
   }
-  if (!APPLY) block_channel_reduce(lds, s1, s2, g, active, c, d.sums, d.sums_ld);
+  if (!APPLY) {
+    block_channel_reduce(lds, s1, s2, g, active, c, d.sums, d.sums_ld);
+    if constexpr (FD) {
+      __syncthreads();
+      block_channel_reduce(lds, f1, f2, g, active && !second, c, d.fold_sums, d.fold_sums_ld, d.c_split);
+    }
+  }
   else if (d.sk_sums) block_channel_reduce(lds, s1, s2, g, active && !second, c, d.sk_sums, d.sk_sums_ld, d.c_split > 0 ? d.c_split : -1);
   else if (d.dbias) {
     for (int i = threadIdx.x; i < c; i += blockDim.x) lds[i] = 0.f;
@@ -695,7 +704,10 @@
   const int f = d->dpool ? d->f : 1;
   const long long items = (long long)d->n * cdiv(d->h, f) * cdiv(d->w_, f) * (d->c / 8);
   const int grid = ew_grid((items + 7) / 8);
-  if (!d->dpool && d->da && (long long)d->n * d->h * d->w_ < 0x7fffffffLL) {
+  SATCV_CHECK(!d->fold_sums || (d->c_split > 0 && d->fold_sums_ld >= d->c_split), "bn_bwd_reduce: fold_sums needs the two-source form");
+  if (d->fold_sums) {
+    DISPATCH_T(d->dtype, hipLaunchKernelGGL((bn_bwd_dense_kernel<T, false, true>), dim3(grid), dim3(EW_BLOCK), (EW_BLOCK + 8) * 16 * sizeof(float), (hipStream_t)stream, *d, 0, d->c));
+  } else if (!d->dpool && d->da && (long long)d->n * d->h * d->w_ < 0x7fffffffLL) {
     DISPATCH_T(d->dtype, hipLaunchKernelGGL((bn_bwd_dense_kernel<T, false>), dim3(grid), dim3(EW_BLOCK), (EW_BLOCK + 8) * 16 * sizeof(float), (hipStream_t)stream, *d, 0, d->c));
   } else {
     DISPATCH_T(d->dtype, hipLaunchKernelGGL((bn_bwd_kernel<T, false>), dim3(grid), dim3(EW_BLOCK), (EW_BLOCK + 8) * 16 * sizeof(float), (hipStream_t)stream, *d));
@@ -742,20 +754,33 @@
   if (dgamma) dgamma[ch] = accumulate ? dgamma[ch] + s2 : s2;
   coef[ch] = s1 / count; coef[c + ch] = s2 / count;
 }
+struct FoldArgs {
+  satcv_stat_t* sums; int ld;
+  const float* sc; const float* mean; const float* rstd; const float* coef; int cc; float eps;
+};
 __global__ void bn_bwd_finalize2_kernel(satcv_stat_t* sums, int ld, satcv_stat_t* asums, int ald, int c, float count, const float* scale, const float* shift,
-                                        const float* mean, const float* rstd, float* dgamma, float* dbeta, float* coef, int accumulate) {
+                                        const float* mean, const float* rstd, float* dgamma, float* dbeta, float* coef, int accumulate,
+                                        const FoldArgs fa) {
   const int ch = blockIdx.x * (blockDim.x / 32) + threadIdx.x / 32, r = threadIdx.x & 31;
-  double d1 = 0.0, d2 = 0.0, a1 = 0.0, a2 = 0.0;
+  double d1 = 0.0, d2 = 0.0, a1 = 0.0, a2 = 0.0, fg = 0.0, fz = 0.0;
   if (ch < c) {
     if (sums) { satcv_stat_t* row = sums + (size_t)r * 2 * ld; d1 = row[ch]; d2 = row[ld + ch]; row[ch] = 0.0; row[ld + ch] = 0.0; }
     satcv_stat_t* arow = asums + (size_t)r * 2 * ald;
     a1 = arow[ch]; a2 = arow[ald + ch]; arow[ch] = 0.0; arow[ald + ch] = 0.0;
+    if (fa.sums) { satcv_stat_t* frow = fa.sums + (size_t)r * 2 * fa.ld; fg = frow[ch]; fz = frow[fa.ld + ch]; frow[ch] = 0.0; frow[fa.ld + ch] = 0.0; }
   }
 #pragma unroll
   for (int o = 16; o > 0; o >>= 1) {
     d1 += __shfl_xor(d1, o, 64); d2 += __shfl_xor(d2, o, 64); a1 += __shfl_xor(a1, o, 64); a2 += __shfl_xor(a2, o, 64);
+    fg += __shfl_xor(fg, o, 64); fz += __shfl_xor(fz, o, 64);
   }
   if (ch >= c || r != 0) return;
+  if (fa.sums) {
+    const double csc = (double)fa.sc[ch], cmu = (double)fa.mean[ch], crs = (double)fa.rstd[ch];
+    const double c1 = (double)fa.coef[ch], c2 = (double)fa.coef[fa.cc + ch];
+    a1 += -csc * fg + fz * (csc * c1 - csc * crs * c2 * cmu);
+    a2 += (double)count * csc * crs * (double)fa.eps * c2;
+  }
   const double sc = (double)scale[ch], sh = (double)shift[ch], mu = (double)mean[ch], rs = (double)rstd[ch];
   const double a2x = sc != 0.0 ? (a2 - (sh + sc * mu) * a1) * (rs / sc) : 0.0;
   const float s1 = (float)(d1 + a1), s2 = (float)(d2 + a2x);
@@ -767,9 +792,22 @@
                                       const float* scale, const float* shift, const float* mean, const float* rstd, float* dgamma, float* dbeta,
                                       float* coef, int32_t accumulate, void* stream) {
   SATCV_CHECK(act_sums && coef && scale && shift && mean && rstd && c > 0 && act_sums_ld >= c && (!sums || sums_ld >= c) && count > 0, "bn_bwd_finalize2: bad args");
+  const FoldArgs fa{nullptr, 0, nullptr, nullptr, nullptr, nullptr, 0, 0.f};
   hipLaunchKernelGGL(bn_bwd_finalize2_kernel, dim3(cdiv(c, 8)), dim3(256), 0, (hipStream_t)stream, sums, sums_ld, act_sums, act_sums_ld, c, count, scale, shift,
-                     mean, rstd, dgamma, dbeta, coef, accumulate);
+                     mean, rstd, dgamma, dbeta, coef, accumulate, fa);
   LAUNCH_OK("bn_bwd_finalize2");
+  return SATCV_OK;
+}
+extern "C" int satcv_bn_bwd_finalize2_fold(satcv_stat_t* sums, int32_t sums_ld, satcv_stat_t* act_sums, int32_t act_sums_ld, satcv_stat_t* fold_sums,
+                                           int32_t fold_sums_ld, int32_t c, float count, const float* scale, const float* shift, const float* mean,
+                                           const float* rstd, const float* cat_scale, const float* cat_mean, const float* cat_rstd, const float* cat_coef,
+                                           int32_t cat_c, float cat_eps, float* dgamma, float* dbeta, float* coef, int32_t accumulate, void* stream) {
+  SATCV_CHECK(act_sums && coef && scale && shift && mean && rstd && c > 0 && act_sums_ld >= c && (!sums || sums_ld >= c) && count > 0, "bn_bwd_finalize2_fold: bad args");
+  SATCV_CHECK(fold_sums && fold_sums_ld >= c && cat_scale && cat_mean && cat_rstd && cat_coef && cat_c >= c, "bn_bwd_finalize2_fold: fold terms missing");
+  const FoldArgs fa{fold_sums, fold_sums_ld, cat_scale, cat_mean, cat_rstd, cat_coef, cat_c, cat_eps};
+  hipLaunchKernelGGL(bn_bwd_finalize2_kernel, dim3(cdiv(c, 8)), dim3(256), 0, (hipStream_t)stream, sums, sums_ld, act_sums, act_sums_ld, c, count, scale, shift,
+                     mean, rstd, dgamma, dbeta, coef, accumulate, fa);
+  LAUNCH_OK("bn_bwd_finalize2_fold");
   return SATCV_OK;
 }
 extern "C" int satcv_bn_bwd_finalize(satcv_stat_t* sums, int32_t sums_ld, int32_t c, float count, float* dgamma, float* dbeta, float* coef, int32_t accumulate,
diff --git a/satellite_computervision_amd/engine.py b/satellite_computervision_amd/engine.py
--- a/satellite_computervision_amd/engine.py
+++ b/satellite_computervision_amd/engine.py
@@ -56,6 +56,24 @@
 EARLY_OPT = os.environ.get('SATCV_EARLY_OPT', '0') == '1'
 EARLY_OPT_FRAC = 0.05
 FUSE_DGRAD_ALL = os.environ.get('SATCV_FUSE_DGRAD_BN_BWD', '1') == '2'
+SKIP_FOLD = os.environ.get('SATCV_SKIP_BN_FOLD', '0') == '1'
+
+
+class _FoldedSkipGrad:
+
+    def __init__(self, g, a, aff, coef, ca, ctot):
+        self.g, self.a, self.aff, self.coef, self.ca, self.ctot = g, a, aff, coef, ca, ctot
+
+    def double(self):
+        import torch
+        ca = self.ca
+        g = self.g.float().reshape(-1, self.ctot)[:, :ca]
+        a = self.a.float().reshape(-1, ca)
+        sc, sh, mu, rs = (self.aff[k][:ca].float() for k in ('scale', 'shift', 'mean', 'rstd'))
+        c1, c2 = self.coef[0][:ca].float(), self.coef[1][:ca].float()
+        gm = torch.where(a * sc + sh > 0, g, torch.zeros_like(g))
+        da = sc * gm - sc * c1 - (sc * rs * c2) * (a - mu)
+        return da.to(self.g.dtype).double()
 
 
 def rup(a, b):
@@ -703,7 +721,7 @@
         self.loss_buf = self._z(1, dtype=torch.float32)
 
         def bn_bwd_steps(da, ldda, dp, lddp, f, yraw, ldy, aff, aoff, sums, sums_off, sums_ld, c, hh, ww, dy, lddy, dbias,
-                         dgamma, dbeta, accum=0, linear=0, frozen=False, second=None, act=None):
+                         dgamma, dbeta, accum=0, linear=0, frozen=False, second=None, act=None, fold=None):
             coef = self._z(2, c, dtype=torch.float32)
             common = dict(yraw=yraw, ldy=ldy, scale=_fp(aff['scale'], aoff), shift=_fp(aff['shift'], aoff),
                           mean=_fp(aff['mean'], aoff), rstd=_fp(aff['rstd'], aoff), n=n, h=hh, w_=ww, c=c, dtype=dt,
@@ -723,7 +741,13 @@
             red.work = dict(kind='bn_bwd_reduce', px=n * hh * ww, c=c, esize=es)
             if parts and not (need_da or need_dp):
                 red = None
-            if parts:
+            if parts and fold is not None:
+                abuf, fa, fo = act['buf'], fold['aff'], fold['coef']
+                fin0 = lambda st: check(lib.satcv_bn_bwd_finalize2_fold(
+                    _fp(sums, sums_off) if red is not None else None, sums_ld, _fp(abuf), c, _fp(fold['buf']), c, c, cnt,
+                    _fp(aff['scale'], aoff), _fp(aff['shift'], aoff), _fp(aff['mean'], aoff), _fp(aff['rstd'], aoff),
+                    _fp(fa['scale']), _fp(fa['mean']), _fp(fa['rstd']), _fp(fo), fold['ctot'], BN_EPS, dgamma, dbeta, _fp(coef), accum, st))
+            elif parts:
                 abuf = act['buf']
                 fin0 = lambda st: check(lib.satcv_bn_bwd_finalize2(_fp(sums, sums_off) if red is not None else None, sums_ld, _fp(abuf), c, c, cnt,
                                                                    _fp(aff['scale'], aoff), _fp(aff['shift'], aoff), _fp(aff['mean'], aoff),
@@ -735,6 +759,8 @@
                     parallel.allreduce_mean_(sums)
                     if parts:
                         parallel.allreduce_mean_(act['buf'])
+                    if fold is not None:
+                        parallel.allreduce_mean_(fold['buf'])
                     fin0(st)
             else:
                 fin = fin0
@@ -769,6 +795,23 @@
             if t.id not in act_sums:
                 act_sums[t.id] = dict(buf=self._z(STAT_ROWS, 2, t.channels, dtype=torch.float64), parts=set())
             return act_sums[t.id]
+
+        fold_src = {}
+        skip_fold = {}
+
+        def skip_fold_ok(cn):
+            if not SKIP_FOLD or dt != ops.BF16 or BIAS_NOISE or not getattr(rt.model, 'fuse_pool_bwd', True):
+                return False
+            if cn.layer.name in self.frozen or cn.layer.name in self.raw_bn:
+                return False
+            ta = cn.inputs[0]
+            if act_sums_for(ta) is None or self.amax_of.get(ta.id) is None or ta.channels not in (32, 64):
+                return False
+            cs = consumers[ta.id]
+            if len([c_ for c_ in cs if c_.op != 'pool']) != 1 or not any(c_.op == 'pool' for c_ in cs):
+                return False
+            ex = ctx.get(id(ta.node))
+            return ex is not None and ex['k'] == 3 and ex['dil'] == 1
 
         seen_layers = set()
         fused = {}
@@ -1055,9 +1098,10 @@
                 sums = pre if pre is not None else self._z(STAT_ROWS, 2, cout, dtype=torch.float64)
                 accum = 1 if lay.name in seen_layers else 0
                 seen_layers.add(lay.name)
-                da_ptr = da[0].data_ptr() + da[1] * es if da is not None else None
+                da_ptr = da[0].data_ptr() + da[1] * es if (da is not None and da[0] is not None) else None
+                sf = skip_fold.get(tout.id)
                 fz = None
-                if (getattr(rt.model, 'fuse_thin_bwd', True) and dt == ops.BF16 and da is not None and dp is None and not graws and not BIAS_NOISE
+                if (getattr(rt.model, 'fuse_thin_bwd', True) and dt == ops.BF16 and da_ptr is not None and dp is None and not graws and not BIAS_NOISE
                         and tin.node.op != 'input' and gact.get(tin.id) is None and cx['k'] == 3 and cx['dil'] == 1 and da[2] == ldy
                         and lay.name not in shared_layers):
                     pk = rt.packed[lay.name]
@@ -1071,9 +1115,15 @@
                                             dw=rt.gptr(lay.name + '/kernel'), cin=pk['cin'], cout=cout, n=n, h=hh, w_=ww, dtype=dt, accumulate=accum, **sa)
                     bt = bst_target(tin) if (sa['in_relu'] and sa['in_scale'] is not None and not act_form_unfit(tin)) else None
                     sums_below = None
+                    fold_buf = None
                     if bt is not None and bt[1] == cinp and bt[0].get('relu', 0) == 1:
                         sums_below = self._z(STAT_ROWS, 2, cinp, dtype=torch.float64)
                         fz.bst_sums, fz.bst_sums_ld, fz.bst_mean, fz.bst_rstd = _fp(sums_below), cinp, bt[0]['mean'], bt[0]['rstd']
+                        if tin.node.op == 'concat_bn_relu' and skip_fold_ok(tin.node) and tin.node.inputs[0].channels == sa['c0']:
+                            fold_buf = self._z(STAT_ROWS, 2, sa['c0'], dtype=torch.float64)
+                            fz.fold_sums, fz.fold_sums_ld = _fp(fold_buf), sa['c0']
+                            if lib.satcv_conv2d_bwd_fused_workspace(C.byref(fz)) < 0:
+                                fz.fold_sums, fz.fold_sums_ld, fold_buf = None, 0, None
                     hf = head_feed.get(tout.id)
                     if (hf is not None and getattr(rt.model, 'fuse_head_grad', True) and hf['ncls'] == 2 and hf['c'] == cout == 32 and cinp == 32
                             and hf['fused_reduce'] and pre is not None and len(consumers.get(tout.id, [])) == 1):
@@ -1085,12 +1135,15 @@
                     nbf = lib.satcv_conv2d_bwd_fused_workspace(C.byref(fz))
                     if nbf < 0 and sums_below is not None:
                         fz.bst_sums, fz.bst_sums_ld, fz.bst_mean, fz.bst_rstd = None, 0, None, None
+                        fz.fold_sums, fz.fold_sums_ld, fold_buf = None, 0, None
                         sums_below = None
                         nbf = lib.satcv_conv2d_bwd_fused_workspace(C.byref(fz))
                     if nbf < 0:
                         fz = None
                     elif sums_below is not None:
                         fused[tin.id] = sums_below
+                        if fold_buf is not None:
+                            fold_src[tin.id] = fold_buf
                 if fz is not None:
                     if DEFER and not accum and lay.name not in shared_layers:
                         fz.defer_reduce = 1
@@ -1126,7 +1179,7 @@
                             fin = fin0
                     self.bwd.append(fin)
                     fstep = lambda st, fz=fz: check(lib.satcv_conv2d_bwd_fused(C.byref(fz), st))
-                    fstep.label = f"bwd_fused k3 n{n} {hh}x{ww} {sa['c0']}+{sa['c1']}->{cout}{' +bnred' if fz.bst_sums else ''}{' +headgrad' if fz.hg_dlogits else ''}"
+                    fstep.label = f"bwd_fused k3 n{n} {hh}x{ww} {sa['c0']}+{sa['c1']}->{cout}{' +bnred' if fz.bst_sums else ''}{' +foldsums' if fz.fold_sums else ''}{' +headgrad' if fz.hg_dlogits else ''}"
                     fstep.work = dict(kind='bwd_fused', taps=9, px=n * hh * ww, cin=pk['cin'], cout=cout, esize=es)
                     self.bwd.append(fstep)
                     gact[tin.id] = (gin, 0, cinp)
@@ -1142,7 +1195,7 @@
                                              dy.data_ptr(), cout, rt.gptr(lay.name + '/bias') if BIAS_NOISE else None,
                                              rt.gptr(lay.bn_name + '/gamma'), rt.gptr(lay.bn_name + '/beta'), accum,
                                              linear=0 if node.attrs.get('relu', True) else 1, frozen=lay.bn_name in self.frozen,
-                                             act=act_sums.get(tout.id) if (act_sums.get(tout.id) or {}).get('parts') else None)
+                                             act=act_sums.get(tout.id) if (act_sums.get(tout.id) or {}).get('parts') else None, fold=sf)
                 fzp = None
                 amax = self.amax_of.get(tout.id)
                 if (amax is not None and getattr(rt.model, 'fuse_pool_bwd', True) and dt == ops.BF16 and da is not None and dp is not None
@@ -1153,11 +1206,15 @@
                     want_dx = tin.node.op != 'input'
                     cinp = r.c
                     ginp = self._z(n, hh, ww, cinp) if want_dx else None
-                    fzp = ops.make_bwdf_desc(g=da_ptr, yraw=y.data_ptr() + yoff * es, ldg=ldy, bn_scale=_fp(aff['scale'], aoff), bn_shift=_fp(aff['shift'], aoff),
+                    fzp = ops.make_bwdf_desc(g=None if sf is not None else da_ptr, yraw=y.data_ptr() + yoff * es, ldg=ldy, bn_scale=_fp(aff['scale'], aoff), bn_shift=_fp(aff['shift'], aoff),
                                              bn_mean=_fp(aff['mean'], aoff), bn_rstd=_fp(aff['rstd'], aoff), bn_coef=_fp(app.coef), linear=0,
                                              w_dgrad=pkp['dgrad'].data_ptr() if want_dx else None, dx=ginp.data_ptr() if want_dx else None,
                                              lddx=cinp if want_dx else 0, dw=rt.gptr(lay.name + '/kernel'), cin=pkp['cin'], cout=cout, n=n, h=hh, w_=ww,
                                              dtype=dt, accumulate=accum, dpool=dp[0].data_ptr(), lddp=dp[2], amax=amax.data_ptr(), **sa)
+                    if sf is not None:
+                        fa_ = sf['aff']
+                        fzp.cat_g, fzp.cat_ld, fzp.cat_c, fzp.cat_coef = sf['g'], sf['ctot'], sf['ctot'], _fp(sf['coef'])
+                        fzp.cat_scale, fzp.cat_shift, fzp.cat_mean, fzp.cat_rstd = _fp(fa_['scale']), _fp(fa_['shift']), _fp(fa_['mean']), _fp(fa_['rstd'])
                     ent = None
                     if (want_dx and POOL_SUMS and tin.node.op == 'pool' and len(consumers[tin.id]) == 1 and sa['in_scale'] is None
                             and len(vals[tin.id].srcs) == 1 and tin.node.inputs[0].channels == cinp):
@@ -1167,8 +1224,12 @@
                     nbp = lib.satcv_conv2d_bwd_fused_workspace(C.byref(fzp))
                     if nbp < 0:
                         fzp = None
+                        if sf is not None:
+                            raise RuntimeError(f'{lay.name}: the folded skip gradient needs the pooled fused backward, which refused the shape')
                     elif ent is not None:
                         ent['parts'].add('pool')
+                if fzp is None and sf is not None:
+                    raise RuntimeError(f'{lay.name}: the folded skip gradient needs the pooled fused backward')
                 if fzp is not None:
                     if DEFER and not accum and lay.name not in shared_layers:
                         fzp.defer_reduce = 1
@@ -1180,14 +1241,14 @@
                     self.keep.append(fzp)
                     self.bwd += [fin] if (pre is not None or red is None) else [red, fin]
                     fstep = lambda st, fzp=fzp: check(lib.satcv_conv2d_bwd_fused(C.byref(fzp), st))
-                    fstep.label = f"bwd_fused k3 n{n} {hh}x{ww} {sa['c0']}+{sa['c1']}->{cout} pooled{'' if want_dx else ' nodx'}{' +poolsums' if fzp.bst_sums else ''}"
+                    fstep.label = f"bwd_fused k3 n{n} {hh}x{ww} {sa['c0']}+{sa['c1']}->{cout} pooled{'' if want_dx else ' nodx'}{' +poolsums' if fzp.bst_sums else ''}{' +skipbn' if fzp.cat_g else ''}"
                     fstep.work = dict(kind='bwd_fused', taps=9, px=n * hh * ww, cin=pkp['cin'], cout=cout, esize=es, nodx=not want_dx, pooled=True)
                     self.bwd.append(fstep)
                     if want_dx:
                         gact[tin.id] = (ginp, 0, cinp)
                         self.dbg['dx:' + lay.name] = ginp
-                    self.dbg['dyparts:' + lay.name] = dict(g=da, y=y, yoff=yoff, ldy=ldy, aff=aff, aoff=aoff, cout=cout, coef=app.coef, linear=0,
-                                                           dp=dp, amax=amax)
+                    self.dbg['dyparts:' + lay.name] = dict(g=(sf['view'], 0, cout) if sf is not None else da, y=y, yoff=yoff, ldy=ldy, aff=aff, aoff=aoff,
+                                                           cout=cout, coef=app.coef, linear=0, dp=dp, amax=amax)
                     self.dbg['_ctx:' + lay.name] = dict(da=da, dp=dp, y=y, yoff=yoff, ldy=ldy, aff=aff, aoff=aoff, cout=cout)
                     continue
                 self.bwd += [fin, app] if (pre is not None or red is None) else [red, fin, app]
@@ -1256,7 +1317,6 @@
                 hh, ww = ra.h, ra.w
                 pre = fused.get(tout.id)
                 sums = pre if pre is not None else self._z(STAT_ROWS, 2, ctot, dtype=torch.float64)
-                dskip = self._z(n, hh, ww, ca)
                 du = self._z(n, hh, ww, cb)
                 bn = node.layer.name
                 upl = tb.node.layer
@@ -1282,6 +1342,26 @@
                     if (bn not in self.frozen and ta.id not in gact and any(cn.op == 'pool' for cn in consumers[ta.id])
                             and len([cn for cn in consumers[ta.id] if cn.op != 'pool']) == 1 and ta.channels == ca):
                         ent = act_sums_for(ta)
+                    fold_buf = None
+                    if ent is not None and ctbf is not None and g[1] == 0 and skip_fold_ok(node):
+                        fold_buf = fold_src.get(tout.id) if pre is not None else self._z(STAT_ROWS, 2, ca, dtype=torch.float64)
+                    if fold_buf is not None:
+                        ent['parts'].add('skip')
+                        if pre is None:
+                            sec.update(fold_sums=_fp(fold_buf), fold_sums_ld=ca)
+                        r_, f_, a_ = bn_bwd_steps(gptr_, ctot, None, 0, 1, ra.srcs[0][0].data_ptr(), ca, aff, 0, sums, 0, ctot, ctot, hh, ww,
+                                                  None, ca, None, rt.gptr(bn + '/gamma'), rt.gptr(bn + '/beta'), frozen=False, second=sec)
+                        if r_ is not None and pre is None:
+                            r_.label += ' +foldsums'
+                        ctbf['coef'] = a_.coef
+                        self.bwd += [f_] if (pre is not None or r_ is None) else [r_, f_]
+                        gact[ta.id] = (None, 0, ca)
+                        skip_fold[ta.id] = dict(g=gptr_, ctot=ctot, aff=aff, coef=a_.coef, buf=fold_buf,
+                                                view=_FoldedSkipGrad(g[0], ra.srcs[0][0], aff, a_.coef, ca, ctot))
+                        self.dbg['du:' + bn] = du
+                        graw[tb.id] = ctbf
+                        continue
+                    dskip = self._z(n, hh, ww, ca)
                     if ent is not None:
                         sec.update(sk_sums=_fp(ent['buf']), sk_sums_ld=ca)
                         ent['parts'].add('skip')
@@ -1300,6 +1380,7 @@
                     self.dbg['du:' + bn] = du
                     graw[tb.id] = ctbf if ctbf is not None else du
                     continue
+                dskip = self._z(n, hh, ww, ca)
                 ra_, fa_, aa_ = bn_bwd_steps(gptr_, ctot, None, 0, 1, ra.srcs[0][0].data_ptr(), ca, aff, 0, sums, 0, ctot, ca, hh, ww,
                                              dskip.data_ptr(), ca, None, rt.gptr(bn + '/gamma'), rt.gptr(bn + '/beta'), frozen=bn in self.frozen)
                 rb_, fb_, ab_ = bn_bwd_steps(gptr_ + ca * es, ctot, None, 0, 1, rb.srcs[0][0].data_ptr(), cb, aff, ca, sums, ca, ctot, cb,
diff --git a/satellite_computervision_amd/ops.py b/satellite_computervision_amd/ops.py
--- a/satellite_computervision_amd/ops.py
+++ b/satellite_computervision_amd/ops.py
@@ -266,9 +266,10 @@
 
 def make_bnbwd_desc(*, yraw, ldy, scale, shift, mean, rstd, n, h, w_, c, dtype, da=None, ldda=0, dpool=None, lddp=0, f=1,
                     sums=None, sums_ld=0, coef=None, dy=None, lddy_out=0, dbias=None, linear=0, yraw1=None, ldy1=0, dy1=None, lddy1=0,
-                    c_split=0, sk_sums=None, sk_sums_ld=0):
+                    c_split=0, sk_sums=None, sk_sums_ld=0, fold_sums=None, fold_sums_ld=0):
     d = BnBwdDesc()
     d.sk_sums, d.sk_sums_ld = sk_sums, sk_sums_ld
+    d.fold_sums, d.fold_sums_ld = fold_sums, fold_sums_ld
     d.linear = linear
     d.yraw1, d.ldy1, d.dy1, d.lddy1, d.c_split = yraw1, ldy1, dy1, lddy1, c_split
     d.da, d.ldda, d.dpool, d.lddp, d.f = da, ldda, dpool, lddp, f
```

Measured after the change: 8381 tiles/s, median of 2. Within noise of the previous version (-0.1%).
